# lemma-osu/sknnr

Measured on AMD Instinct MI355X. Metric: Mqueries/sec + achieved HBM GB/s, 10M×50k×32 k=5, 1/2/4/8 MI355X, higher is better.
Workload: dtype f16 split MFMA (hi.hi swept, lo.hi + hi.lo corrections; f32 accumulate) pre-filter + f64 exact re-score

## Files before the change

include/sknnr_hip.h:

```cpp
#ifndef SKNNR_HIP_H
#define SKNNR_HIP_H

#include <stdint.h>

#ifdef __cplusplus
extern "C" {
#endif
#pragma GCC visibility push(default)

#define SKNNR_ABI_VERSION 5

typedef enum sknnr_status {
    SKNNR_OK = 0,
    SKNNR_ERR_INVALID = -1,
    SKNNR_ERR_K_TOO_LARGE = -2,
    SKNNR_ERR_NO_TARGETS = -3,
    SKNNR_ERR_UNSUPPORTED = -4,
    SKNNR_ERR_HIP = -5,
    SKNNR_ERR_NO_DEVICE = -6,
    SKNNR_ERR_NONFINITE = -7
} sknnr_status;

typedef enum sknnr_memspace {
    SKNNR_MEM_HOST = 0,
    SKNNR_MEM_DEVICE = 1
} sknnr_memspace;

typedef enum sknnr_formula {
    SKNNR_FORMULA_EXPANDED = 0,
    SKNNR_FORMULA_DIRECT = 1,
    SKNNR_FORMULA_HAMMING = 2
} sknnr_formula;

typedef enum sknnr_dtype {
    SKNNR_DTYPE_F64 = 0,
    SKNNR_DTYPE_F32 = 1,
    SKNNR_DTYPE_I16 = 2,
    SKNNR_DTYPE_U16 = 3,
    SKNNR_DTYPE_U8 = 4,
    SKNNR_DTYPE_I32 = 5
} sknnr_dtype;

typedef enum sknnr_weight_mode {
    SKNNR_WEIGHTS_UNIFORM = 0,
    SKNNR_WEIGHTS_DISTANCE = 1,
    SKNNR_WEIGHTS_EXPLICIT = 2,
    SKNNR_WEIGHTS_BASE_MASK = 0xff,
    SKNNR_WEIGHTS_F32_TARGETS = 0x100,
    SKNNR_WEIGHTS_F32_WEIGHTS = 0x200
} sknnr_weight_mode;

typedef struct sknnr_index sknnr_index;

typedef struct sknnr_query_opts {
    int32_t n_neighbors;
    int32_t exclude_self;
    int32_t deterministic;
    int32_t decimals;
    int32_t formula;
    int32_t apply_affine;
    int32_t weight_mode;
    int32_t check_finite;
    int32_t query_dtype;
    int32_t reserved_;
    int64_t row_offset;
} sknnr_query_opts;

typedef struct sknnr_stats {
    int64_t queries;
    int64_t coarse_queries;
    int64_t exact_fallbacks;
    int64_t exact_only_queries;
    double  last_kernel_ms;
    double  last_coarse_ms;
    double  total_kernel_ms;
    double  total_coarse_ms;
    int64_t timed_calls;
    int64_t coarse_rows_timed;
    double  mfma_executed_ratio;
} sknnr_stats;


int32_t sknnr_device_count(void);

int32_t sknnr_abi_version(void);

const char* sknnr_last_error(void);

int sknnr_index_create(const double* ref, int64_t n_ref, int32_t d, const double* y, int32_t t,
                       int32_t device, sknnr_index** out);

void sknnr_index_destroy(sknnr_index* index);

int sknnr_index_set_affine(sknnr_index* index, int32_t d_in, const double* center,
                           const double* scale, const double* proj);

int sknnr_index_set_hamming_weights(sknnr_index* index, const double* w, int32_t n);

int sknnr_index_set_forest(sknnr_index* index, int32_t d_in, int32_t n_trees, const int64_t* tree_offset,
                           const double* threshold, const int32_t* feature, const int32_t* left,
                           const int32_t* right);

int sknnr_forest_apply(sknnr_index* index, const void* q, int64_t nq, int32_t query_dtype, int32_t mem,
                       double* out_ids);

int sknnr_affine_transform(const double* x, int64_t n, int32_t d_in, const double* center,
                           const double* scale, const double* proj, int32_t d, double* out,
                           int32_t device);

int sknnr_index_shape(const sknnr_index* index, int64_t* n_ref, int32_t* d, int32_t* t,
                      int32_t* d_in, int32_t* device);

int sknnr_get_stats(const sknnr_index* index, sknnr_stats* out);
int sknnr_reset_stats(sknnr_index* index);

int sknnr_check_finite(sknnr_index* index, void* stream);


int sknnr_kneighbors(sknnr_index* index, const void* q, int64_t nq,
                     const sknnr_query_opts* opts, double* out_dist, int64_t* out_idx,
                     int32_t mem, void* stream);

int sknnr_predict(sknnr_index* index, const void* q, int64_t nq, const sknnr_query_opts* opts,
                  double* out_pred, double* out_dist, int64_t* out_idx, int32_t mem, void* stream);

int sknnr_predict_from_neighbors(sknnr_index* index, const double* dist, const int64_t* idx,
                                 const double* w, int64_t nq, int32_t k, int32_t weight_mode,
                                 double* out_pred, int32_t mem, void* stream);

int sknnr_hamming_distances(sknnr_index* index, const double* q, int64_t nq, const int64_t* rows, int64_t n_rows,
                            double* out, int32_t mem, void* stream);


int sknnr_shard_candidates(sknnr_index* index, const double* q, int64_t nq, const sknnr_query_opts* opts,
                           int64_t index_offset, double* out_val, int64_t* out_idx, int32_t mem, void* stream);
int sknnr_merge_shards(sknnr_index* index, const double* q, int64_t nq, const sknnr_query_opts* opts, int32_t n_shards,
                       const double* shard_val, const int64_t* shard_idx, double* out_dist, int64_t* out_idx,
                       int32_t mem, void* stream);


typedef struct sknnr_stream sknnr_stream;
int sknnr_stream_begin(sknnr_index* index, const sknnr_query_opts* opts, int32_t want_dist, int32_t want_pred,
                       sknnr_stream** out);
int sknnr_stream_push(sknnr_stream* stream, const void* q, int64_t nq, double* out_dist, int64_t* out_idx,
                      double* out_pred);
int sknnr_stream_flush(sknnr_stream* stream);
int sknnr_stream_end(sknnr_stream* stream, int64_t* rows_pushed);

int sknnr_crosswalk(const int64_t* table, int64_t n_table, const int64_t* idx, int64_t n,
                    int64_t* out, int32_t device, int32_t mem, void* stream);


int sknnr_debug_coarse_matrix(sknnr_index* index, const double* q, int64_t nq, float* out,
                              double* out_qnorm, double* out_scale, double* out_eps);

int sknnr_debug_last_prefilter(const sknnr_index* index, int64_t out[8]);

int sknnr_debug_last_hamming(const sknnr_index* index, int64_t out[8]);

int sknnr_debug_hamming_candidates(const sknnr_index* index, int32_t* cnt, int32_t* ids, int64_t n);

#pragma GCC visibility pop
#ifdef __cplusplus
}
#endif
#endif
```

sknnr_amd/_native.py:

```python

from __future__ import annotations

import ctypes
import os
from ctypes import POINTER, byref, c_char_p, c_double, c_float, c_int32, c_int64, c_void_p

import numpy as np

from . import _build

MEM_HOST = 0
MEM_DEVICE = 1
FORMULA_EXPANDED = 0
FORMULA_DIRECT = 1
FORMULA_HAMMING = 2
WEIGHTS_UNIFORM = 0
WEIGHTS_DISTANCE = 1
WEIGHTS_EXPLICIT = 2
WEIGHTS_F32_TARGETS = 0x100
WEIGHTS_F32_WEIGHTS = 0x200

ERR_INVALID = -1
ERR_K_TOO_LARGE = -2
ERR_NO_TARGETS = -3
ERR_UNSUPPORTED = -4
ERR_HIP = -5
ERR_NO_DEVICE = -6
ERR_NONFINITE = -7
ABI_VERSION = 5

DTYPE_CODES = {np.dtype(np.float64): 0, np.dtype(np.float32): 1, np.dtype(np.int16): 2, np.dtype(np.uint16): 3,
               np.dtype(np.uint8): 4, np.dtype(np.int32): 5}


def dtype_code(dt) -> int | None:
    try:
        return DTYPE_CODES.get(np.dtype(dt))
    except TypeError:
        name = str(dt).replace("torch.", "")
        try:
            return DTYPE_CODES.get(np.dtype(name))
        except TypeError:
            return None


EXPORTED_SYMBOLS = (
    "sknnr_device_count",
    "sknnr_abi_version",
    "sknnr_last_error",
    "sknnr_index_create",
    "sknnr_index_destroy",
    "sknnr_index_set_affine",
    "sknnr_index_set_hamming_weights",
    "sknnr_index_set_forest",
    "sknnr_forest_apply",
    "sknnr_affine_transform",
    "sknnr_index_shape",
    "sknnr_get_stats",
    "sknnr_reset_stats",
    "sknnr_check_finite",
    "sknnr_kneighbors",
    "sknnr_predict",
    "sknnr_predict_from_neighbors",
    "sknnr_hamming_distances",
    "sknnr_shard_candidates",
    "sknnr_merge_shards",
    "sknnr_stream_begin",
    "sknnr_stream_push",
    "sknnr_stream_flush",
    "sknnr_stream_end",
    "sknnr_crosswalk",
    "sknnr_debug_coarse_matrix",
    "sknnr_debug_last_prefilter",
    "sknnr_debug_last_hamming",
    "sknnr_debug_hamming_candidates",
)


class QueryOpts(ctypes.Structure):
    _fields_ = [
        ("n_neighbors", c_int32),
        ("exclude_self", c_int32),
        ("deterministic", c_int32),
        ("decimals", c_int32),
        ("formula", c_int32),
        ("apply_affine", c_int32),
        ("weight_mode", c_int32),
        ("check_finite", c_int32),
        ("query_dtype", c_int32),
        ("reserved_", c_int32),
        ("row_offset", c_int64),
    ]


class Stats(ctypes.Structure):
    _fields_ = [
        ("queries", c_int64),
        ("coarse_queries", c_int64),
        ("exact_fallbacks", c_int64),
        ("exact_only_queries", c_int64),
        ("last_kernel_ms", c_double),
        ("last_coarse_ms", c_double),
        ("total_kernel_ms", c_double),
        ("total_coarse_ms", c_double),
        ("timed_calls", c_int64),
        ("coarse_rows_timed", c_int64),
        ("mfma_executed_ratio", c_double),
    ]

    def as_dict(self) -> dict:
        return {name: getattr(self, name) for name, _ in self._fields_}


class HipBackendError(RuntimeError):

    def __init__(self, code: int, message: str):
        super().__init__(f"[sknnr_hip {code}] {message}")
        self.code = code
        self.message = message


_lib = None


def library_path() -> str:
    return os.environ.get("SKNNR_HIP_LIBRARY") or _build.LIB_PATH


def load(build_if_missing: bool = False):
    global _lib
    if _lib is not None:
        return _lib
    import torch

    path = library_path()
    if not os.path.exists(path):
        if build_if_missing:
            _build.build()
        else:
            raise ImportError(
                f"{path} is missing: the MI355X backend has not been built. "
                "Run `python -m sknnr_amd._build` (needs hipcc); there is no CPU fallback."
            )
    lib = ctypes.CDLL(path)
    if lib.sknnr_abi_version() != ABI_VERSION:
        raise ImportError(
            f"{path} has ABI version {lib.sknnr_abi_version()}, this package needs {ABI_VERSION}: "
            "rebuild it with `python -m sknnr_amd._build --force`")
    vp = c_void_p
    lib.sknnr_device_count.restype = c_int32
    lib.sknnr_abi_version.restype = c_int32
    lib.sknnr_last_error.restype = c_char_p
    lib.sknnr_index_create.argtypes = [vp, c_int64, c_int32, vp, c_int32, c_int32, POINTER(vp)]
    lib.sknnr_index_destroy.argtypes = [vp]
    lib.sknnr_index_destroy.restype = None
    lib.sknnr_index_set_affine.argtypes = [vp, c_int32, vp, vp, vp]
    lib.sknnr_index_set_hamming_weights.argtypes = [vp, vp, c_int32]
    lib.sknnr_index_set_forest.argtypes = [vp, c_int32, c_int32, vp, vp, vp, vp, vp]
    lib.sknnr_forest_apply.argtypes = [vp, vp, c_int64, c_int32, c_int32, vp]
    lib.sknnr_affine_transform.argtypes = [vp, c_int64, c_int32, vp, vp, vp, c_int32, vp, c_int32]
    lib.sknnr_index_shape.argtypes = [vp, POINTER(c_int64), POINTER(c_int32), POINTER(c_int32),
                                      POINTER(c_int32), POINTER(c_int32)]
    lib.sknnr_get_stats.argtypes = [vp, POINTER(Stats)]
    lib.sknnr_reset_stats.argtypes = [vp]
    lib.sknnr_check_finite.argtypes = [vp, vp]
    lib.sknnr_stream_begin.argtypes = [vp, POINTER(QueryOpts), c_int32, c_int32, POINTER(vp)]
    lib.sknnr_stream_push.argtypes = [vp, vp, c_int64, vp, vp, vp]
    lib.sknnr_stream_flush.argtypes = [vp]
    lib.sknnr_stream_end.argtypes = [vp, POINTER(c_int64)]
    lib.sknnr_kneighbors.argtypes = [vp, vp, c_int64, POINTER(QueryOpts), vp, vp, c_int32, vp]
    lib.sknnr_predict.argtypes = [vp, vp, c_int64, POINTER(QueryOpts), vp, vp, vp, c_int32, vp]
    lib.sknnr_predict_from_neighbors.argtypes = [vp, vp, vp, vp, c_int64, c_int32, c_int32, vp,
                                                 c_int32, vp]
    lib.sknnr_hamming_distances.argtypes = [vp, vp, c_int64, vp, c_int64, vp, c_int32, vp]
    lib.sknnr_shard_candidates.argtypes = [vp, vp, c_int64, POINTER(QueryOpts), c_int64, vp, vp, c_int32, vp]
    lib.sknnr_merge_shards.argtypes = [vp, vp, c_int64, POINTER(QueryOpts), c_int32, vp, vp, vp, vp, c_int32, vp]
    lib.sknnr_crosswalk.argtypes = [vp, c_int64, vp, c_int64, vp, c_int32, c_int32, vp]
    lib.sknnr_debug_coarse_matrix.argtypes = [vp, vp, c_int64, vp, vp, POINTER(c_double),
                                              POINTER(c_double)]
    lib.sknnr_debug_last_prefilter.argtypes = [vp, POINTER(c_int64)]
    lib.sknnr_debug_last_hamming.argtypes = [vp, POINTER(c_int64)]
    lib.sknnr_debug_hamming_candidates.argtypes = [vp, vp, vp, c_int64]
    _lib = lib
    return lib


def check(code: int) -> None:
    if code != 0:
        raise HipBackendError(code, load().sknnr_last_error().decode("utf-8", "replace"))


def device_count() -> int:
    return int(load().sknnr_device_count())


def _host_ptr(a):
    return None if a is None else a.ctypes.data_as(c_void_p)


def _c_f64(a):
    return None if a is None else np.ascontiguousarray(a, dtype=np.float64)


def _c_rows(a, opts):
    if a is None:
        return None
    for dt, code in DTYPE_CODES.items():
        if code == opts.query_dtype:
            return np.ascontiguousarray(a, dtype=dt)
    raise ValueError(f"unknown query_dtype {opts.query_dtype}")


class Index:

    def __init__(self, ref, y=None, device: int = 0):
        lib = load()
        ref = _c_f64(ref)
        if ref.ndim != 2:
            raise ValueError("ref must be 2-D")
        y2 = None
        if y is not None:
            y2 = _c_f64(y)
            if y2.ndim == 1:
                y2 = y2.reshape(-1, 1)
            if y2.shape[0] != ref.shape[0]:
                raise ValueError("y and ref row counts differ")
        self.n_ref, self.d = ref.shape
        self.t = 0 if y2 is None else y2.shape[1]
        self.device = device
        self.d_in = self.d
        self._h = c_void_p()
        check(lib.sknnr_index_create(_host_ptr(ref), self.n_ref, self.d, _host_ptr(y2), self.t,
                                     device, byref(self._h)))

    def close(self):
        if getattr(self, "_h", None) is not None and self._h:
            load().sknnr_index_destroy(self._h)
            self._h = None

    def __del__(self):
        try:
            self.close()
        except Exception:
            pass

    @property
    def handle(self):
        if not self._h:
            raise RuntimeError("index is closed")
        return self._h

    def set_affine(self, d_in: int, center=None, scale=None, proj=None):
        center, scale, proj = _c_f64(center), _c_f64(scale), _c_f64(proj)
        if proj is not None and proj.shape != (d_in, self.d):
            raise ValueError(f"proj must be ({d_in}, {self.d}), got {proj.shape}")
        check(load().sknnr_index_set_affine(self.handle, d_in, _host_ptr(center), _host_ptr(scale),
                                            _host_ptr(proj)))
        self.d_in = d_in

    def set_hamming_weights(self, w):
        w = _c_f64(w).reshape(-1)
        check(load().sknnr_index_set_hamming_weights(self.handle, _host_ptr(w), w.size))

    def set_forest(self, d_in, tree_offset, threshold, feature, left, right):
        off = np.ascontiguousarray(tree_offset, dtype=np.int64)
        thr = _c_f64(threshold)
        feat, lc, rc = (np.ascontiguousarray(a, dtype=np.int32) for a in (feature, left, right))
        n_nodes = int(off[-1]) if off.size else 0
        if off.ndim != 1 or off.size < 2 or any(a.shape != (n_nodes,) for a in (thr, feat, lc, rc)):
            raise ValueError("tree_offset must hold n_trees + 1 offsets and the node arrays tree_offset[-1] entries")
        check(load().sknnr_index_set_forest(self.handle, int(d_in), off.size - 1, _host_ptr(off), _host_ptr(thr),
                                            _host_ptr(feat), _host_ptr(lc), _host_ptr(rc)))
        self.d_in = int(d_in)

    def forest_apply_host(self, q, query_dtype=0):
        q = _c_rows(q, QueryOpts(query_dtype=int(query_dtype)))
        out = np.empty((q.shape[0], self.d), dtype=np.float64)
        check(load().sknnr_forest_apply(self.handle, _host_ptr(q), q.shape[0], int(query_dtype), MEM_HOST,
                                        _host_ptr(out)))
        return out

    def forest_apply_device(self, q_ptr, nq, query_dtype, out_ptr):
        check(load().sknnr_forest_apply(self.handle, c_void_p(q_ptr or None), nq, int(query_dtype), MEM_DEVICE,
                                        c_void_p(out_ptr or None)))

    def stats(self) -> dict:
        st = Stats()
        check(load().sknnr_get_stats(self.handle, byref(st)))
        return st.as_dict()

    def reset_stats(self):
        check(load().sknnr_reset_stats(self.handle))

    @staticmethod
    def make_opts(k, exclude_self=False, deterministic=True, decimals=10, formula=FORMULA_EXPANDED,
                  apply_affine=False, weight_mode=WEIGHTS_UNIFORM, row_offset=0,
                  check_finite=False, query_dtype=0) -> QueryOpts:
        return QueryOpts(int(k), int(bool(exclude_self)), int(bool(deterministic)), int(decimals),
                         int(formula), int(bool(apply_affine)), int(weight_mode), int(bool(check_finite)),
                         int(query_dtype), 0, int(row_offset))

    def check_finite(self, stream=0) -> None:
        check(load().sknnr_check_finite(self.handle, c_void_p(stream or None)))

    def open_stream(self, opts: QueryOpts, want_dist=True, want_pred=False) -> "QueryStream":
        return QueryStream(self, opts, want_dist, want_pred)

    def kneighbors_host(self, q, opts: QueryOpts, nq=None, return_distance=True):
        q = _c_rows(q, opts)
        if q is not None:
            nq = q.shape[0]
        k = opts.n_neighbors
        idx = np.empty((nq, k), dtype=np.int64)
        dist = np.empty((nq, k), dtype=np.float64) if return_distance else None
        check(load().sknnr_kneighbors(self.handle, _host_ptr(q), nq, byref(opts), _host_ptr(dist),
                                      _host_ptr(idx), MEM_HOST, None))
        return dist, idx

    def predict_host(self, q, opts: QueryOpts, nq=None, return_neighbors=False):
        q = _c_rows(q, opts)
        if q is not None:
            nq = q.shape[0]
        k = opts.n_neighbors
        pred = np.empty((nq, self.t), dtype=np.float64)
        dist = idx = None
        if return_neighbors:
            dist = np.empty((nq, k), dtype=np.float64)
            idx = np.empty((nq, k), dtype=np.int64)
        check(load().sknnr_predict(self.handle, _host_ptr(q), nq, byref(opts), _host_ptr(pred),
                                   _host_ptr(dist), _host_ptr(idx), MEM_HOST, None))
        return (pred, dist, idx) if return_neighbors else pred

    def predict_from_neighbors_host(self, dist, idx, w, weight_mode):
        idx = np.ascontiguousarray(idx, dtype=np.int64)
        dist, w = _c_f64(dist), _c_f64(w)
        nq, k = idx.shape
        pred = np.empty((nq, self.t), dtype=np.float64)
        check(load().sknnr_predict_from_neighbors(self.handle, _host_ptr(dist), _host_ptr(idx),
                                                  _host_ptr(w), nq, k, int(weight_mode),
                                                  _host_ptr(pred), MEM_HOST, None))
        return pred

    def kneighbors_device(self, q_ptr, nq, opts: QueryOpts, dist_ptr, idx_ptr, stream=0):
        check(load().sknnr_kneighbors(self.handle, c_void_p(q_ptr or None), nq, byref(opts),
                                      c_void_p(dist_ptr or None), c_void_p(idx_ptr), MEM_DEVICE,
                                      c_void_p(stream or None)))

    def predict_device(self, q_ptr, nq, opts: QueryOpts, pred_ptr, dist_ptr=0, idx_ptr=0, stream=0):
        check(load().sknnr_predict(self.handle, c_void_p(q_ptr or None), nq, byref(opts),
                                   c_void_p(pred_ptr), c_void_p(dist_ptr or None),
                                   c_void_p(idx_ptr or None), MEM_DEVICE, c_void_p(stream or None)))

    def predict_from_neighbors_device(self, dist_ptr, idx_ptr, w_ptr, nq, k, weight_mode, pred_ptr,
                                      stream=0):
        check(load().sknnr_predict_from_neighbors(
            self.handle, c_void_p(dist_ptr or None), c_void_p(idx_ptr), c_void_p(w_ptr or None), nq, k,
            int(weight_mode), c_void_p(pred_ptr), MEM_DEVICE, c_void_p(stream or None)))

    def hamming_distances_host(self, q, rows=None):
        q = _c_f64(q)
        nq = self.n_ref if q is None else q.shape[0]
        rows = None if rows is None else np.ascontiguousarray(rows, dtype=np.int64)
        n_rows = nq if rows is None else rows.size
        out = np.empty((n_rows, self.n_ref), dtype=np.float64)
        check(load().sknnr_hamming_distances(self.handle, _host_ptr(q), nq, _host_ptr(rows), n_rows, _host_ptr(out),
                                             MEM_HOST, None))
        return out

    def shard_candidates_host(self, q, opts: QueryOpts, index_offset=0):
        q = _c_f64(q)
        nq, k = q.shape[0], opts.n_neighbors
        val = np.empty((nq, k), dtype=np.float64)
        idx = np.empty((nq, k), dtype=np.int64)
        check(load().sknnr_shard_candidates(self.handle, _host_ptr(q), nq, byref(opts), int(index_offset),
                                            _host_ptr(val), _host_ptr(idx), MEM_HOST, None))
        return val, idx

    def shard_candidates_device(self, q_ptr, nq, opts: QueryOpts, index_offset, val_ptr, idx_ptr, stream=0):
        check(load().sknnr_shard_candidates(self.handle, c_void_p(q_ptr), nq, byref(opts), int(index_offset),
                                            c_void_p(val_ptr), c_void_p(idx_ptr), MEM_DEVICE, c_void_p(stream or None)))

    def merge_shards_host(self, q, opts: QueryOpts, shard_val, shard_idx, nq=None, return_distance=True):
        q = _c_f64(q)
        shard_val = _c_f64(shard_val)
        shard_idx = np.ascontiguousarray(shard_idx, dtype=np.int64)
        n_shards = shard_val.shape[0]
        if q is not None:
            nq = q.shape[0]
        k = opts.n_neighbors
        idx = np.empty((nq, k), dtype=np.int64)
        dist = np.empty((nq, k), dtype=np.float64) if return_distance else None
        check(load().sknnr_merge_shards(self.handle, _host_ptr(q), nq, byref(opts), n_shards, _host_ptr(shard_val),
                                        _host_ptr(shard_idx), _host_ptr(dist), _host_ptr(idx), MEM_HOST, None))
        return dist, idx

    def merge_shards_device(self, q_ptr, nq, opts: QueryOpts, n_shards, val_ptr, sidx_ptr, dist_ptr, idx_ptr, stream=0):
        check(load().sknnr_merge_shards(self.handle, c_void_p(q_ptr or None), nq, byref(opts), n_shards, c_void_p(val_ptr),
                                        c_void_p(sidx_ptr), c_void_p(dist_ptr or None), c_void_p(idx_ptr), MEM_DEVICE,
                                        c_void_p(stream or None)))

    def debug_coarse_matrix(self, q):
        q = _c_f64(q)
        nq = q.shape[0]
        out = np.empty((nq, self.n_ref), dtype=np.float32)
        qn = np.empty(nq, dtype=np.float64)
        s, eps = c_double(), c_double()
        check(load().sknnr_debug_coarse_matrix(self.handle, _host_ptr(q), nq, _host_ptr(out),
                                               _host_ptr(qn), byref(s), byref(eps)))
        return out, qn, s.value, eps.value

    PREFILTER_FIELDS = ("generation", "ks", "m_list", "rank_extra", "bulk_waves", "bulk_rows", "thin_rows", "cell_depth")

    def debug_last_prefilter(self) -> dict:
        out = (c_int64 * 8)()
        check(load().sknnr_debug_last_prefilter(self.handle, out))
        return dict(zip(self.PREFILTER_FIELDS, (int(v) for v in out)))

    HAMMING_FIELDS = ("ran", "kk", "compacts", "seed_rows", "band", "tree_pairs", "chunks", "handed_to_scan")

    def debug_last_hamming(self) -> dict:
        out = (c_int64 * 8)()
        check(load().sknnr_debug_last_hamming(self.handle, out))
        return dict(zip(self.HAMMING_FIELDS, (int(v) for v in out)))

    def debug_hamming_candidates(self, n: int):
        cnt = np.empty(n, dtype=np.int32)
        ids = np.empty((n, 192), dtype=np.int32)
        check(load().sknnr_debug_hamming_candidates(self.handle, _host_ptr(cnt), _host_ptr(ids), int(n)))
        return cnt, ids


class QueryStream:

    def __init__(self, index: Index, opts: QueryOpts, want_dist=True, want_pred=False):
        self._index = index
        self._h = c_void_p()
        self._keep = []
        self.k = opts.n_neighbors
        self._opts = opts
        self.want_dist, self.want_pred = bool(want_dist), bool(want_pred)
        check(load().sknnr_stream_begin(index.handle, byref(opts), int(self.want_dist), int(self.want_pred),
                                        byref(self._h)))

    def push(self, q, out_idx=None, out_dist=None, out_pred=None, need_idx=True):
        q = _c_rows(q, self._opts)
        nq = q.shape[0]
        if out_idx is None and (need_idx or not self.want_pred):
            out_idx = np.empty((nq, self.k), dtype=np.int64)
        if out_dist is None and self.want_dist:
            out_dist = np.empty((nq, self.k), dtype=np.float64)
        if out_pred is None and self.want_pred:
            out_pred = np.empty((nq, self._index.t), dtype=np.float64)
        for a, dt, cols in ((out_idx, np.int64, self.k), (out_dist, np.float64, self.k),
                            (out_pred, np.float64, self._index.t)):
            if a is not None and (a.dtype != dt or not a.flags.c_contiguous or a.shape != (nq, cols)):
                raise ValueError(f"output arrays must be C-contiguous ({nq}, {cols}) {np.dtype(dt)}")
        check(load().sknnr_stream_push(self._h, _host_ptr(q), nq, _host_ptr(out_dist), _host_ptr(out_idx),
                                       _host_ptr(out_pred)))
        self._keep.append((out_idx, out_dist, out_pred))
        if len(self._keep) > 8:
            del self._keep[:-8]
        return out_idx, out_dist, out_pred

    def flush(self):
        check(load().sknnr_stream_flush(self._h))
        self._keep.clear()

    def close(self) -> int:
        if not self._h:
            return 0
        n = c_int64(0)
        h, self._h = self._h, c_void_p()
        code = load().sknnr_stream_end(h, byref(n))
        self._keep.clear()
        check(code)
        return int(n.value)

    def __enter__(self):
        return self

    def __exit__(self, *exc):
        if exc[0] is None:
            self.close()
        else:
            try:
                self.close()
            except HipBackendError:
                pass

    def __del__(self):
        try:
            if self._h:
                load().sknnr_stream_end(self._h, None)
                self._h = c_void_p()
        except Exception:
            pass


def affine_transform_host(x, center=None, scale=None, proj=None, device: int = 0) -> np.ndarray:
    x = _c_f64(x)
    center, scale, proj = _c_f64(center), _c_f64(scale), _c_f64(proj)
    n, d_in = x.shape
    d = d_in if proj is None else proj.shape[1]
    out = np.empty((n, d), dtype=np.float64)
    check(load().sknnr_affine_transform(_host_ptr(x), n, d_in, _host_ptr(center), _host_ptr(scale),
                                        _host_ptr(proj), d, _host_ptr(out), device))
    return out


def crosswalk_host(table, idx, device: int = 0):
    table = np.ascontiguousarray(table, dtype=np.int64)
    idx = np.ascontiguousarray(idx, dtype=np.int64)
    out = np.empty(idx.shape, dtype=np.int64)
    check(load().sknnr_crosswalk(_host_ptr(table), table.size, _host_ptr(idx), idx.size,
                                 _host_ptr(out), device, MEM_HOST, None))
    return out


def crosswalk_device(table_ptr, n_table, idx_ptr, n, out_ptr, device=0, stream=0):
    check(load().sknnr_crosswalk(c_void_p(table_ptr), n_table, c_void_p(idx_ptr), n, c_void_p(out_ptr),
                                 device, MEM_DEVICE, c_void_p(stream or None)))
```

sknnr_amd/csrc/bucket.hip.h:

```cpp
#pragma once
#include <hip/hip_runtime.h>
#include <stdint.h>

namespace sknnr {

constexpr int kCellMaxDepth = 6;
constexpr int kCellMax = 1 << kCellMaxDepth;
constexpr int kBucketBlock = 1024;
#ifndef SKNNR_BUCKET_CHUNKS
#define SKNNR_BUCKET_CHUNKS 32
#endif
constexpr int kBucketChunks = SKNNR_BUCKET_CHUNKS;

struct CellTreeDev {
    const float* axes;
    const float* centre;
    const float* thr;
    int depth;
};

__device__ __forceinline__ int cell_of(const float (&z)[kCellMaxDepth], const CellTreeDev& t) {
    int node = 0;
#pragma unroll
    for (int l = 0; l < kCellMaxDepth; ++l)
        if (l < t.depth) node = 2 * node + (z[l] >= t.thr[(1 << l) - 1 + node] ? 1 : 0);
    return node;
}

struct CellArgs {
    const double* xq;
    long nq;
    long n_pad;
    int d;
    int depth;
    const float* axes;
    const float* centre;
    const float* thr;
    unsigned char* cell;
    int* hist;
    int* perm;
};

#ifdef SKNNR_KERNELS_EXACT
__global__ void __launch_bounds__(256) cell_assign_kernel(CellArgs a) {
    const long q = (long)blockIdx.x * 256 + threadIdx.x;
    if (q < a.nq) {
        const double* row = a.xq + q * a.d;
        float z[kCellMaxDepth];
#pragma unroll
        for (int l = 0; l < kCellMaxDepth; ++l) z[l] = 0.f;
        auto feed = [&](int k, double x) {
            const float v = (float)x - a.centre[k];
#pragma unroll
            for (int l = 0; l < kCellMaxDepth; ++l)
                if (l < a.depth) z[l] = fmaf(v, a.axes[l * a.d + k], z[l]);
        };
        int k = 0;
        if ((a.d & 3) == 0) {
            const double2* r2 = (const double2*)row;
            for (; k + 8 <= a.d; k += 8) {
                const double2 v0 = r2[k / 2], v1 = r2[k / 2 + 1], v2 = r2[k / 2 + 2], v3 = r2[k / 2 + 3];
                feed(k, v0.x); feed(k + 1, v0.y); feed(k + 2, v1.x); feed(k + 3, v1.y);
                feed(k + 4, v2.x); feed(k + 5, v2.y); feed(k + 6, v3.x); feed(k + 7, v3.y);
            }
        }
        for (; k < a.d; ++k) feed(k, row[k]);
        const CellTreeDev t{a.axes, a.centre, a.thr, a.depth};
        a.cell[q] = (unsigned char)cell_of(z, t);
    }
}
#endif

#ifdef SKNNR_KERNELS_EXACT
__global__ void __launch_bounds__(kBucketBlock) cell_count_kernel(CellArgs a) {
    __shared__ int h[kCellMax];
    if (threadIdx.x < kCellMax) h[threadIdx.x] = 0;
    __syncthreads();
#pragma unroll
    for (int r = 0; r < kBucketChunks; ++r) {
        const long q = ((long)blockIdx.x * kBucketChunks + r) * kBucketBlock + threadIdx.x;
        if (q < a.nq) atomicAdd(&h[a.cell[q]], 1);
    }
    __syncthreads();
    if (threadIdx.x < kCellMax && h[threadIdx.x] != 0) atomicAdd(&a.hist[threadIdx.x], h[threadIdx.x]);
}
#endif


#ifdef SKNNR_KERNELS_EXACT
__global__ void __launch_bounds__(kBucketBlock) cell_scatter_kernel(CellArgs a) {
    __shared__ int cnt[kCellMax], base[kCellMax], first[kCellMax];
    const int n_cells = 1 << a.depth;
    if (threadIdx.x < kCellMax) cnt[threadIdx.x] = 0;
    if (threadIdx.x == 0) {
        int acc = 0;
        for (int c = 0; c < kCellMax; ++c) {
            first[c] = acc;
            acc += c < n_cells ? a.hist[c] : 0;
        }
    }
    __syncthreads();
    int c[kBucketChunks], ticket[kBucketChunks];
#pragma unroll
    for (int r = 0; r < kBucketChunks; ++r) {
        const long q = ((long)blockIdx.x * kBucketChunks + r) * kBucketBlock + threadIdx.x;
        c[r] = 0;
        ticket[r] = 0;
        if (q < a.nq) {
            c[r] = a.cell[q];
            ticket[r] = atomicAdd(&cnt[c[r]], 1);
        } else if (q < a.n_pad) {
            a.perm[q] = (int)q;
            a.cell[q] = (unsigned char)(n_cells - 1);
        }
    }
    __syncthreads();
    if (threadIdx.x < kCellMax && cnt[threadIdx.x] != 0) base[threadIdx.x] = atomicAdd(&a.hist[kCellMax + threadIdx.x], cnt[threadIdx.x]);
    __syncthreads();
#pragma unroll
    for (int r = 0; r < kBucketChunks; ++r) {
        const long q = ((long)blockIdx.x * kBucketChunks + r) * kBucketBlock + threadIdx.x;
        if (q < a.nq) a.perm[first[c[r]] + base[c[r]] + ticket[r]] = (int)q;
    }
}
#endif

}
```

sknnr_amd/csrc/coarse.hip.h:

```cpp
#pragma once
#include <hip/hip_runtime.h>
#include <float.h>
#include <stdint.h>

namespace sknnr {

#if !defined(SKNNR_EXPERIMENTS) && defined(SKNNR_ABLATE_NO_CORR)
#error "SKNNR_ABLATE_NO_CORR is a timing experiment with wrong results: add -DSKNNR_EXPERIMENTS"
#endif

constexpr long kRowQuantum = 6144;

typedef _Float16 half8 __attribute__((ext_vector_type(8)));
typedef float floatx16 __attribute__((ext_vector_type(16)));
typedef float floatx4 __attribute__((ext_vector_type(4)));

__host__ __device__ constexpr int tile_frag_bytes(int ks) { return 2 * ks * 1024; }
__host__ __device__ constexpr int tile_bytes(int ks) { return 2 * ks * 1024 + 128; }
__host__ __device__ constexpr int tiles_per_stage(int ks) { return ks <= 2 ? 8 : (ks <= 4 ? 4 : 2); }
__host__ __device__ constexpr size_t qimg_index(long row, int part, int ks, int s, int kh) {
    return ((size_t)(row * 2 + part) * ks + s) * 2 + kh;
}
__host__ __device__ constexpr int acc_row(int r, int h) { return (r & 3) + 8 * (r >> 2) + 4 * h; }

// ... 32 lines not shown
__device__ __forceinline__ float min2f(float a, float b, float dep) {
    float r;
    asm("v_min_f32 %0, %1, %2" : "=v"(r) : "v"(a), "v"(b), "v"(dep));
    return r;
}
__device__ __forceinline__ float min2f(float a, float b) { return min2f(a, b, a); }

#ifndef SKNNR_SHIFT_INSERT_FROM
#define SKNNR_SHIFT_INSERT_FROM 32
#endif
template <int M>
__device__ __forceinline__ void list_insert(float (&vals)[M], int (&idxs)[M], float v, int id) {
    if constexpr (M >= SKNNR_SHIFT_INSERT_FROM) {
#pragma unroll
        for (int i = M - 1; i >= 0; --i) {
            const bool here = v < vals[i];
            const bool lower_left = i > 0 ? (v < vals[i - 1]) : false;
            const float nv = lower_left ? vals[i > 0 ? i - 1 : 0] : v;
            const int ni = lower_left ? idxs[i > 0 ? i - 1 : 0] : id;
            vals[i] = here ? nv : vals[i];
            idxs[i] = here ? ni : idxs[i];
        }
    } else {
        vals[M - 1] = v;
        idxs[M - 1] = id;
#pragma unroll
        for (int i = M - 1; i > 0; --i) {
            const bool sw = vals[i] < vals[i - 1];
            const float lo = sw ? vals[i] : vals[i - 1];
            const float hi = sw ? vals[i - 1] : vals[i];
            const int ilo = sw ? idxs[i] : idxs[i - 1];
            const int ihi = sw ? idxs[i - 1] : idxs[i];
            vals[i - 1] = lo;
            vals[i] = hi;
            idxs[i - 1] = ilo;
            idxs[i] = ihi;
        }
    }
}

#ifdef SKNNR_COARSE_TIMERS
static __device__ unsigned long long coarse_timers[8];
#define TICK()                                  \
    do {                                        \
        asm volatile("" ::: "memory");          \
        tk = __builtin_readcyclecounter();      \
        asm volatile("" ::: "memory");          \
    } while (0)
#define TSTAMP(i)            \
    do {                     \
        tk0 = tk;            \
        TICK();              \
        tm[i] += tk - tk0;   \
    } while (0)
#else
#define TICK() ((void)0)
#define TSTAMP(i) ((void)0)
#endif
#ifdef SKNNR_COARSE_COUNTERS
static __device__ unsigned long long coarse_counters[16];
#define CTR_ARG , unsigned (&ctr)[16]
#define CTR_PASS , ctr
#define CTR(i, n) ctr[i] += (unsigned)(n)
#else
#define CTR_ARG
#define CTR_PASS
#define CTR(i, n) ((void)0)
#endif


#ifndef SKNNR_PRIO_CORR
#define SKNNR_PRIO_CORR 2
#define SKNNR_PRIO_SCAN 2
#endif
#ifndef SKNNR_PRIO_MAIN
#define SKNNR_PRIO_MAIN 1
#define SKNNR_PRIO_TEST 0
#endif

__host__ __device__ constexpr int queue_cap(int m) { return m == 2 ? 2 : 4; }
__host__ __device__ constexpr int queue_flush_at(int m) { return m == 2 ? 2 : 3; }
__host__ __device__ constexpr int queue_bytes_per_wave(int nqb, int m) { return nqb * queue_cap(m) * 64 * 8; }

template <int KS>
__device__ __forceinline__ floatx16 contract_main(const half8 (&ah)[KS], const half8 (&bh)[KS], floatx16 c0) {
    floatx16 acc = __builtin_amdgcn_mfma_f32_32x32x16_f16(ah[0], bh[0], c0, 0, 0, 0);
#pragma unroll
    for (int s = 1; s < KS; ++s) acc = __builtin_amdgcn_mfma_f32_32x32x16_f16(ah[s], bh[s], acc, 0, 0, 0);
    return acc;
}
template <int KS>
__device__ __forceinline__ floatx16 contract_correct(const half8 (&ah)[KS], const half8 (&al)[KS],
                                                     const half8 (&bh)[KS], const half8 (&bl)[KS],
                                                     floatx16 acc) {
#pragma unroll
    for (int s = 0; s < KS; ++s) acc = __builtin_amdgcn_mfma_f32_32x32x16_f16(al[s], bh[s], acc, 0, 0, 0);
#pragma unroll
    for (int s = 0; s < KS; ++s) acc = __builtin_amdgcn_mfma_f32_32x32x16_f16(ah[s], bl[s], acc, 0, 0, 0);
    return acc;
}
template <int KS>
__device__ __forceinline__ floatx16 split_contract(const half8 (&ah)[KS], const half8 (&al)[KS],
                                                   const half8 (&bh)[KS], const half8 (&bl)[KS],
                                                   floatx16 c0) {
    return contract_correct<KS>(ah, al, bh, bl, contract_main<KS>(ah, bh, c0));
}

__device__ __forceinline__ void stage_copy(const char* __restrict__ gsrc, char* lds_dst, int bytes,
                                           int wave, int lane, int n_waves) {
    const int n_chunks = (bytes + 1023) >> 10;
    for (int c = wave; c < n_chunks; c += n_waves) {
        const int off = (c << 10) + (lane << 4);
        if (off < bytes) {
            __builtin_amdgcn_global_load_lds(
                (const __attribute__((address_space(1))) void*)(gsrc + off),
                (__attribute__((address_space(3))) void*)(lds_dst + (c << 10)), 16, 0, 0);
        }
    }
}

__device__ __forceinline__ unsigned lds_addr_of(const void* p) {
    return (unsigned)(unsigned long)(const __attribute__((address_space(3))) char*)p;
}
__device__ __forceinline__ void queue_store(unsigned addr, float v, int id) {
    const unsigned long long pr = ((unsigned long long)(unsigned)id << 32) | (unsigned long long)__float_as_uint(v);
    asm volatile("ds_write_b64 %0, %1" ::"v"(addr), "v"(pr) : "memory");
}
__device__ __forceinline__ unsigned long long queue_load(unsigned addr) {
    unsigned long long pr;
    asm volatile("ds_read_b64 %0, %1\n\ts_waitcnt lgkmcnt(0)" : "=&v"(pr) : "v"(addr) : "memory");
    return pr;
}

template <int M>
__device__ __forceinline__ void take_hit(float v, int id, float (&vals)[M], int (&idxs)[M], float& thr,
                                         int& cnt, unsigned qlane CTR_ARG) {
    const bool hit = v < thr;
    if (__builtin_amdgcn_ballot_w64(hit) == 0) return;
    CTR(3, 1);
    CTR(4, __builtin_popcountll(__builtin_amdgcn_ballot_w64(hit)));
    const bool room = cnt < queue_cap(M);
    if (hit && room) {
        queue_store(qlane + cnt * 512, v, id);
        cnt += 1;
    }
    if (__builtin_amdgcn_ballot_w64(hit && !room) != 0) {
        CTR(5, 1);
        if (hit && !room) {
            list_insert<M>(vals, idxs, v, id);
            thr = min2f(thr, vals[M - 1]);
        }
    }
}

template <int M>
__device__ __forceinline__ float pair_union_rank_m(const float (&vals)[M]) {
    float u = fminf(vals[0], __shfl_xor(vals[M - 1], 32, 64));
#pragma unroll
    for (int i = 1; i < M; ++i) u = fmaxf(u, fminf(vals[i], __shfl_xor(vals[M - 1 - i], 32, 64)));
    return u;
}

template <int M>
__device__ __forceinline__ void flush_queue(float (&vals)[M], int (&idxs)[M], float& thr, int& cnt,
                                            unsigned qlane CTR_ARG) {
    for (int i = 0; __builtin_amdgcn_ballot_w64(i < cnt) != 0; ++i) {
        CTR(7, 1);
        CTR(8, __builtin_popcountll(__builtin_amdgcn_ballot_w64(i < cnt)));
        if (i < cnt) {
            const unsigned long long e = queue_load(qlane + i * 512);
            const float ev = __uint_as_float((unsigned)e);
            CTR(9, __builtin_amdgcn_ballot_w64(ev < vals[M - 1]) != 0);
            CTR(10, __builtin_popcountll(__builtin_amdgcn_ballot_w64(ev < vals[M - 1])));
            if (ev < vals[M - 1]) list_insert<M>(vals, idxs, ev, (int)(e >> 32));
        }
    }
    cnt = 0;
    thr = pair_union_rank_m<M>(vals);
}

template <int KS, int M>
__global__ void __launch_bounds__(coarse_waves(KS, M) * 64, coarse_wps(KS, M))
coarse_kernel(const char* __restrict__ rimg,
              int n_stages,
              const uint4* __restrict__ qimg,
              const double* __restrict__ qnc,
              float skip_scale,
              int n_sentinel,
              float* __restrict__ cand_val,
              int* __restrict__ cand_idx) {
    constexpr int TPS = tiles_per_stage(KS);
    constexpr int TB = tile_bytes(KS);
    constexpr int STAGE = TPS * TB;
    extern __shared__ __attribute__((aligned(16))) char smem[];

    const int lane = threadIdx.x & 63;
    const int wave = __builtin_amdgcn_readfirstlane(threadIdx.x >> 6);
    const int half = lane >> 5;
    constexpr int WAVES = coarse_waves(KS, M);
    constexpr int NQB = coarse_nqb(KS, M);
    constexpr bool LO_ON_DEMAND = coarse_lo_on_demand(KS, M);
    const int qb0 = (blockIdx.x * WAVES + wave) * NQB;
    const unsigned qwave = lds_addr_of(smem + 2 * STAGE + wave * queue_bytes_per_wave(NQB, M) + lane * 8);

    half8 bh[NQB][KS], bl[NQB][KS];
#pragma unroll
    for (int qb = 0; qb < NQB; ++qb) {
#pragma unroll
        for (int s = 0; s < KS; ++s) {
            const long row = (long)(qb0 + qb) * 32 + (lane & 31);
            const uint4 uh = qimg[qimg_index(row, 0, KS, s, lane >> 5)];
            const uint4 ul = qimg[qimg_index(row, 1, KS, s, lane >> 5)];
            bh[qb][s] = __builtin_bit_cast(half8, uh);
            bl[qb][s] = __builtin_bit_cast(half8, ul);
        }
    }

    float vals[NQB][M];
    int idxs[NQB][M];
    float thr[NQB];
    float margin[NQB];
    int cnt[NQB];
#pragma unroll
    for (int qb = 0; qb < NQB; ++qb) {
        thr[qb] = FLT_MAX;
        cnt[qb] = 0;
        margin[qb] = skip_scale * (float)sqrt(qnc[(size_t)(qb0 + qb) * 32 + (lane & 31)]) + 1e-30f;
#pragma unroll
        for (int i = 0; i < M; ++i) {
            vals[qb][i] = (half == 0 && i < n_sentinel) ? -FLT_MAX : FLT_MAX;
            idxs[qb][i] = -1;
        }
    }

#ifdef SKNNR_COARSE_COUNTERS
    unsigned ctr[16] = {};
#endif
#ifdef SKNNR_COARSE_TIMERS
    unsigned long long tm[8] = {};
    unsigned long long tk = 0, tk0 = 0;
    TICK();
    const unsigned long long t_begin = tk;
#endif
    stage_copy(rimg, smem, STAGE, wave, lane, WAVES);
    __syncthreads();

    for (int st = 0; st < n_stages; ++st) {
        char* cur = smem + (st & 1) * STAGE;
        if (st + 1 < n_stages)
            stage_copy(rimg + (size_t)(st + 1) * STAGE, smem + ((st + 1) & 1) * STAGE, STAGE, wave, lane, WAVES);

        auto tile_load = [&](const char* tb, half8 (&ah)[KS], half8 (&al)[KS], floatx16& c0, bool keep_lo) {
#pragma unroll
            for (int s = 0; s < KS; ++s) {
                ah[s] = *(const half8*)(tb + (0 * KS + s) * 1024 + lane * 16);
                if (keep_lo) al[s] = *(const half8*)(tb + (1 * KS + s) * 1024 + lane * 16);
            }
            const floatx4* cp = (const floatx4*)(tb + tile_frag_bytes(KS) + half * 64);
            const floatx4 c_0 = cp[0], c_1 = cp[1], c_2 = cp[2], c_3 = cp[3];
#pragma unroll
            for (int i = 0; i < 4; ++i) {
                c0[i] = c_0[i];
                c0[4 + i] = c_1[i];
                c0[8 + i] = c_2[i];
                c0[12 + i] = c_3[i];
            }
        };
        auto tile_process = [&](const char* tb, int tile_no, const floatx16& c0, half8 (&ah)[KS], half8 (&al)[KS],
                                bool have_lo) {
            const int id_base = tile_no * 32 + 4 * half;
#pragma unroll
            for (int qb = 0; qb < NQB; ++qb) {
                __builtin_amdgcn_s_setprio(SKNNR_PRIO_MAIN);
                floatx16 acc = contract_main<KS>(ah, bh[qb], c0);
                __builtin_amdgcn_s_setprio(SKNNR_PRIO_TEST);
                const float t0 = first_read(acc[0]);
                float g[5];
                g[0] = min3f(t0, acc[1], acc[2], t0);
                g[1] = min3f(acc[3], acc[4], acc[5], t0);
                g[2] = min3f(acc[6], acc[7], acc[8], t0);
                g[3] = min3f(acc[9], acc[10], acc[11], t0);
                g[4] = min2f(min3f(acc[12], acc[13], acc[14], t0), acc[15], t0);
                const float m1 = min3f(min3f(g[0], g[1], g[2], t0), g[3], g[4], t0);
                const float loose = thr[qb] + margin[qb];
                CTR(0, 1);
                if (__builtin_amdgcn_ballot_w64(m1 < loose) == 0) {
                    TSTAMP(1);
                    continue;
                }
                TSTAMP(2);
                CTR(1, 1);
                CTR(11, __builtin_popcountll(__builtin_amdgcn_ballot_w64(m1 < loose)));
                CTR(12, __builtin_amdgcn_ballot_w64(m1 < thr[qb]) != 0);
                if (!have_lo) {
#pragma unroll
                    for (int s = 0; s < KS; ++s) al[s] = *(const half8*)(tb + (1 * KS + s) * 1024 + lane * 16);
                    have_lo = true;
                }
                __builtin_amdgcn_s_setprio(SKNNR_PRIO_CORR);
#ifndef SKNNR_ABLATE_NO_CORR
                acc = contract_correct<KS>(ah, al, bh[qb], bl[qb], acc);
#endif
                __builtin_amdgcn_s_setprio(SKNNR_PRIO_SCAN);
                const unsigned qlane = qwave + qb * (queue_cap(M) * 512);
#pragma unroll
                for (int k = 0; k < 5; ++k) {
// ... 85 lines not shown
```

sknnr_amd/csrc/coarse2.hip.h:

```cpp
#pragma once
#include "coarse.hip.h"

#if !defined(SKNNR_EXPERIMENTS) && (defined(SKNNR_V2_SWEEP_ONLY) || defined(SKNNR_V2_NO_BARRIER) || defined(SKNNR_V2_NO_SEED))
#error "SKNNR_V2_SWEEP_ONLY / NO_BARRIER / NO_SEED are timing experiments with wrong results: add -DSKNNR_EXPERIMENTS"
#endif

namespace sknnr {

typedef _Float16 half2v __attribute__((ext_vector_type(2)));

__host__ __device__ constexpr int tile2_bytes(int ks) { return ks * 1024 + 128; }
#ifndef SKNNR_V2_WAVES
#define SKNNR_V2_WAVES 16
#endif
#ifndef SKNNR_V2_UNROLL
#define SKNNR_V2_UNROLL 1
#endif
#ifndef SKNNR_V2_TPS
#define SKNNR_V2_TPS (SKNNR_V2_WAVES == 16 ? 16 : 8)
#endif
__host__ __device__ constexpr int tiles_per_stage2(int ks) { return ks <= 2 ? SKNNR_V2_TPS : SKNNR_V2_TPS / 2; }
#ifndef SKNNR_SEED_TILES
#define SKNNR_SEED_TILES 64
#endif
constexpr int kSeedTiles = SKNNR_SEED_TILES;
__host__ __device__ constexpr int seed_tiles_for(long n_tiles, int tps) {
    const long want = n_tiles / 8 < kSeedTiles ? n_tiles / 8 : kSeedTiles;
    const long stages = want / tps < 1 ? 1 : want / tps;
    return (int)(stages * tps);
}
constexpr int kCoarse2Waves = SKNNR_V2_WAVES;
constexpr int kCoarse2Nqb = 2;
#ifndef SKNNR_V2_QCAP
#define SKNNR_V2_QCAP 5
#endif
constexpr int kQueueCap = SKNNR_V2_QCAP;
#ifndef SKNNR_V2_FLUSH_AT
#define SKNNR_V2_FLUSH_AT 3
#endif
constexpr int kQueueFlushAt = SKNNR_V2_FLUSH_AT;
__host__ __device__ constexpr int queue2_bytes_per_wave() { return kCoarse2Nqb * kQueueCap * 64 * 8 + kCoarse2Nqb * 64 * 4; }
#ifndef SKNNR_V2_M2
#define SKNNR_V2_M2 1
#endif
#ifndef SKNNR_V2_M12
#define SKNNR_V2_M12 1
#endif
#ifndef SKNNR_V2_M16
#define SKNNR_V2_M16 1
#endif
__host__ __device__ constexpr bool coarse2_supported(int ks, int m) {
    return (m == 6 && ks <= 4) || (m == 8 && ks <= 4) || (SKNNR_V2_M2 && m == 2 && ks <= 2) || (SKNNR_V2_M16 && m == 16 && ks <= 4) ||
           (SKNNR_V2_M12 && m == 12 && ks <= 4);
}
#ifndef SKNNR_V2_M16_WAVES
#define SKNNR_V2_M16_WAVES 12
#endif
__host__ __device__ constexpr int coarse2_waves(int ks, int m) {
    return (m == 16 || (m == 12 && ks >= 2) || (m == 8 && ks >= 4)) ? SKNNR_V2_M16_WAVES : kCoarse2Waves;
}

__device__ __forceinline__ float dot8(const half8& x, const half8& y, float acc) {
#pragma unroll
    for (int i = 0; i < 4; ++i) {
        const half2v p = {x[2 * i], x[2 * i + 1]}, q = {y[2 * i], y[2 * i + 1]};
        acc = __builtin_amdgcn_fdot2(p, q, acc, false);
    }
    return acc;
}

template <int M, int E>
__device__ __forceinline__ float pair_union_rank(const float (&vals)[M]) {
    if constexpr (E == 0) {
        return pair_union_rank_m<M>(vals);
    } else {
        static_assert(E >= 1 && E <= M, "rank between M + 1 and 2 M");
        float u = fmaxf(vals[E - 1], __shfl_xor(vals[E - 1], 32, 64));
#pragma unroll
        for (int i = E; i < M; ++i) u = fmaxf(u, fminf(vals[i], __shfl_xor(vals[M + E - 1 - i], 32, 64)));
        return u;
    }
}
__host__ __device__ constexpr int coarse2_rank_extra(int m_list, int kk) {
    if (kk + 1 <= m_list) return 0;
    if (m_list == 6) return 3;
    if (m_list == 8) return kk <= 10 ? 4 : (kk <= 13 ? 7 : 8);
    if (m_list == 12) return kk <= 20 ? 10 : 12;
    return kk <= 20 ? 6 : (kk <= 25 ? 11 : (kk <= 30 ? 15 : 16));
}
constexpr int kCoarse2MaxKK6 = 7, kCoarse2MaxKK8 = 15, kCoarse2MaxKK12 = 23;
constexpr int kCoarse2MaxKK16 = 31;

#define SKNNR_TREE_A                                   \
    "v_min3_f32 %[g0], %[x0], %[x1], %[x2]\n\t"        \
    "v_min3_f32 %[g1], %[x3], %[x4], %[x5]\n\t"        \
    "v_min3_f32 %[g2], %[x6], %[x7], %[x8]\n\t"        \
    "v_min3_f32 %[g3], %[x9], %[x10], %[x11]\n\t"
#define SKNNR_TREE_B                                   \
    "v_min3_f32 %[g4], %[x12], %[x13], %[x14]\n\t"     \
    "v_min3_f32 %[m], %[g0], %[g1], %[g2]\n\t"         \
    "v_min_f32 %[g4], %[g4], %[x15]\n\t"               \
    "s_nop 0\n\t"                                      \
    "v_min3_f32 %[m], %[m], %[g3], %[g4]\n\t"
#define SKNNR_TREE_OUT [g0] "=&v"(g[0]), [g1] "=&v"(g[1]), [g2] "=&v"(g[2]), [g3] "=&v"(g[3]), [g4] "=&v"(g[4]), [m] "=&v"(m)
#define SKNNR_TREE_IN                                                                                             \
    [x0] "v"(x[0]), [x1] "v"(x[1]), [x2] "v"(x[2]), [x3] "v"(x[3]), [x4] "v"(x[4]), [x5] "v"(x[5]), [x6] "v"(x[6]), \
        [x7] "v"(x[7]), [x8] "v"(x[8]), [x9] "v"(x[9]), [x10] "v"(x[10]), [x11] "v"(x[11]), [x12] "v"(x[12]),       \
        [x13] "v"(x[13]), [x14] "v"(x[14]), [x15] "v"(x[15])

__device__ __forceinline__ void step_test_only(const floatx16& x, float (&g)[5], float& m) {
    asm volatile("s_nop 7\n\ts_nop 7\n\t" SKNNR_TREE_A SKNNR_TREE_B : SKNNR_TREE_OUT : SKNNR_TREE_IN);
}
template <int KS>
__device__ __forceinline__ void tile_issue_and_test(floatx16& a, floatx16& c, const half8 (&ah)[KS], const half8 (&p)[KS],
                                                    const half8 (&q)[KS], float (&g)[5], float& m) {
    static_assert(KS >= 1 && KS <= 4, "hand-scheduled for one to four K-steps");
    asm volatile("v_mfma_f32_32x32x16_f16 %[a], %[h0], %[p0], %[c]\n\t" : [a] "=&v"(a) : [c] "v"(c), [h0] "v"(ah[0]), [p0] "v"(p[0]));
#pragma unroll
    for (int s = 1; s < KS; ++s)
        asm volatile("v_mfma_f32_32x32x16_f16 %[a], %[h], %[p], %[a]\n\t" : [a] "+v"(a) : [h] "v"(ah[s]), [p] "v"(p[s]));
    asm volatile("v_mfma_f32_32x32x16_f16 %[c], %[h0], %[q0], %[c]\n\t"
                 "s_nop 7\n\ts_nop 3\n\t"
                 : [c] "+v"(c)
                 : [h0] "v"(ah[0]), [q0] "v"(q[0]), "v"(a));
    const floatx16& x = a;
    asm volatile(SKNNR_TREE_A
                 : [g0] "=&v"(g[0]), [g1] "=&v"(g[1]), [g2] "=&v"(g[2]), [g3] "=&v"(g[3])
                 : [x0] "v"(x[0]), [x1] "v"(x[1]), [x2] "v"(x[2]), [x3] "v"(x[3]), [x4] "v"(x[4]), [x5] "v"(x[5]),
                   [x6] "v"(x[6]), [x7] "v"(x[7]), [x8] "v"(x[8]), [x9] "v"(x[9]), [x10] "v"(x[10]), [x11] "v"(x[11]));
    if constexpr (KS >= 2)
        asm volatile("v_mfma_f32_32x32x16_f16 %[c], %[h1], %[q1], %[c]\n\t" : [c] "+v"(c) : [h1] "v"(ah[1]), [q1] "v"(q[1]));
    asm volatile("v_min3_f32 %[g4], %[x12], %[x13], %[x14]\n\t"
                 "v_min3_f32 %[m], %[g0], %[g1], %[g2]\n\t"
                 "v_min_f32 %[g4], %[g4], %[x15]\n\t"
                 "s_nop 0\n\t"
                 "v_min3_f32 %[m], %[m], %[g3], %[g4]\n\t"
                 : [g4] "=&v"(g[4]), [m] "=&v"(m)
                 : [x12] "v"(x[12]), [x13] "v"(x[13]), [x14] "v"(x[14]), [x15] "v"(x[15]), [g0] "v"(g[0]), [g1] "v"(g[1]),
                   [g2] "v"(g[2]), [g3] "v"(g[3]));
#pragma unroll
    for (int s = 2; s < KS; ++s)
        asm volatile("v_mfma_f32_32x32x16_f16 %[c], %[h], %[q], %[c]\n\t" : [c] "+v"(c) : [h] "v"(ah[s]), [q] "v"(q[s]));
}

template <int KS, int M, int WAVES = kCoarse2Waves, int E = 0>
__global__ void __launch_bounds__(WAVES * 64, WAVES == 12 ? 3 : (WAVES == 8 || M > 8 ? 2 : 4))
coarse2_kernel(const char* __restrict__ rhi,
               const char* __restrict__ rlo,
               int n_stages,
               const uint4* __restrict__ qimg,
               const double* __restrict__ qnc,
               float skip_scale,
               int n_sentinel,
               float* __restrict__ cand_val,
               int* __restrict__ cand_idx,
               int pos0, const int* __restrict__ qperm, const unsigned char* __restrict__ qcell,
               const int* __restrict__ cell_stage) {
    constexpr int TPS = tiles_per_stage2(KS);
    constexpr int TB = tile2_bytes(KS);
    constexpr int STAGE = TPS * TB;
    constexpr int NQB = kCoarse2Nqb;
    extern __shared__ __attribute__((aligned(16))) char smem[];

    const int lane = threadIdx.x & 63;
    const int wave = __builtin_amdgcn_readfirstlane(threadIdx.x >> 6);
    const int half = lane >> 5;
    const int qb0 = (blockIdx.x * WAVES + wave) * NQB;
    const unsigned qwave = lds_addr_of(smem + 2 * STAGE + wave * queue2_bytes_per_wave() + lane * 8);
    const unsigned qrow_lds = lds_addr_of(smem + 2 * STAGE + wave * queue2_bytes_per_wave() + NQB * kQueueCap * 512 + lane * 4);
    int st0 = 0;
    if (qperm) {
        const int mid = qperm[pos0 + (blockIdx.x * WAVES + WAVES / 2) * NQB * 32];
        st0 = __builtin_amdgcn_readfirstlane(cell_stage[qcell[mid]]);
    }
    auto qfrag = [&](int r, int part, int s) {
        return __builtin_bit_cast(half8, qimg[qimg_index(r, part, KS, s, lane >> 5)]);
    };
    auto stage_of = [&](int st) {
        const int i = st0 + st;
        return i >= n_stages ? i - n_stages : i;
    };

    half8 bh[NQB][KS];
    float qnorm[NQB];
#pragma unroll
    for (int qb = 0; qb < NQB; ++qb) {
        const int pos = pos0 + (qb0 + qb) * 32 + (lane & 31);
        const int r = qperm ? qperm[pos] : pos;
        asm volatile("ds_write_b32 %0, %1" ::"v"(qrow_lds + qb * 256), "v"(r) : "memory");
#pragma unroll
        for (int s = 0; s < KS; ++s) bh[qb][s] = qfrag(r, 0, s);
        qnorm[qb] = (float)sqrt(qnc[r]);
    }

    float vals[NQB][M];
    int idxs[NQB][M];
#ifdef SKNNR_COARSE_COUNTERS
    unsigned ctr[16] = {};
#endif
#ifdef SKNNR_COARSE_TIMERS
    unsigned long long tm[8] = {};
    unsigned long long tk = 0, tk0 = 0;
    TICK();
    const unsigned long long t_begin = tk;
#endif
    float loose[NQB], margin[NQB];
    int cnt[NQB];
    auto reset_lists = [&](int qb) {
#pragma unroll
        for (int i = 0; i < M; ++i) {
            vals[qb][i] = (half == 0 && i < n_sentinel) ? -FLT_MAX : FLT_MAX;
            idxs[qb][i] = -1;
        }
    };
#pragma unroll
    for (int qb = 0; qb < NQB; ++qb) {
        cnt[qb] = 0;
        margin[qb] = skip_scale * qnorm[qb] + 1e-30f;
        loose[qb] = FLT_MAX;
        reset_lists(qb);
    }

    auto load_c0 = [&](const char* tb, floatx16& acc) {
        const floatx4* cp = (const floatx4*)(tb + KS * 1024 + half * 64);
        const floatx4 c_0 = cp[0], c_1 = cp[1], c_2 = cp[2], c_3 = cp[3];
#pragma unroll
        for (int i = 0; i < 4; ++i) {
            acc[i] = c_0[i];
            acc[4 + i] = c_1[i];
            acc[8 + i] = c_2[i];
            acc[12 + i] = c_3[i];
        }
    };
    auto load_hi = [&](const char* tb, half8 (&ah)[KS]) {
#pragma unroll
        for (int s = 0; s < KS; ++s) ah[s] = *(const half8*)(tb + s * 1024 + lane * 16);
    };
    auto issue_main = [&](const half8 (&ah)[KS], int qb, floatx16& acc) {
        __builtin_amdgcn_s_setprio(1);
#pragma unroll
        for (int s = 0; s < KS; ++s) acc = __builtin_amdgcn_mfma_f32_32x32x16_f16(ah[s], bh[qb][s], acc, 0, 0, 0);
        __builtin_amdgcn_s_setprio(0);
    };

    auto flush_wave = [&](int qb) {
        TSTAMP(1);
        CTR(6, 1);
        const unsigned qbase = qwave - (unsigned)lane * 8u + (unsigned)qb * (kQueueCap * 512u);
        const int c = cnt[qb];
        const unsigned long long b0 = __builtin_amdgcn_ballot_w64((c & 1) != 0), b1 = __builtin_amdgcn_ballot_w64((c & 2) != 0),
                                 b2 = __builtin_amdgcn_ballot_w64((c & 4) != 0);
        auto below = [&](unsigned long long m) { return (int)__builtin_amdgcn_mbcnt_hi((unsigned)(m >> 32), __builtin_amdgcn_mbcnt_lo((unsigned)m, 0u)); };
        const int off = below(b0) + 2 * below(b1) + 4 * below(b2);
        const int total = __builtin_popcountll(b0) + 2 * __builtin_popcountll(b1) + 4 * __builtin_popcountll(b2);
        static_assert(kQueueCap == 5 || kQueueCap == 4, "four or five entries per lane are read here");
        unsigned long long own[5];
        if constexpr (kQueueCap == 5) {
            asm volatile("ds_read_b64 %0, %5\n\tds_read_b64 %1, %5 offset:512\n\tds_read_b64 %2, %5 offset:1024\n\t"
                         "ds_read_b64 %3, %5 offset:1536\n\tds_read_b64 %4, %5 offset:2048\n\ts_waitcnt lgkmcnt(0)"
                         : "=&v"(own[0]), "=&v"(own[1]), "=&v"(own[2]), "=&v"(own[3]), "=&v"(own[4])
                         : "v"(qbase + (unsigned)lane * 8u)
                         : "memory");
        } else {
            asm volatile("ds_read_b64 %0, %4\n\tds_read_b64 %1, %4 offset:512\n\tds_read_b64 %2, %4 offset:1024\n\t"
                         "ds_read_b64 %3, %4 offset:1536\n\ts_waitcnt lgkmcnt(0)"
                         : "=&v"(own[0]), "=&v"(own[1]), "=&v"(own[2]), "=&v"(own[3])
                         : "v"(qbase + (unsigned)lane * 8u)
                         : "memory");
        }
#pragma unroll
        for (int j = 0; j < kQueueCap; ++j) {
            const unsigned long long e = own[j] | ((unsigned long long)(unsigned)(lane & 31) << 58);
            if (j < c) asm volatile("ds_write_b64 %0, %1" ::"v"(qbase + (unsigned)(off + j) * 8u), "v"(e) : "memory");
        }
        const unsigned qrow_base = qrow_lds - (unsigned)lane * 4u + (unsigned)qb * 256u;
        for (int t0 = 0; t0 < total; t0 += 32) {
            CTR(7, 1);
            const int gi = t0 + (lane & 31);
            const bool on = gi < total;
            unsigned long long e;
            asm volatile("ds_read_b64 %0, %1\n\ts_waitcnt lgkmcnt(0)" : "=&v"(e) : "v"(qbase + (unsigned)(on ? gi : 0) * 8u) : "memory");
            CTR(8, __builtin_popcountll(__builtin_amdgcn_ballot_w64(on)));
            const unsigned hi32 = (unsigned)(e >> 32);
            const int pos = (int)(hi32 & 0x03ffffffu), col = (int)(hi32 >> 26);
            int r;
            asm volatile("ds_read_b32 %0, %1\n\ts_waitcnt lgkmcnt(0)" : "=&v"(r) : "v"(qrow_base + (unsigned)col * 4u) : "memory");
            const unsigned row = (unsigned)(pos & 31) * 16u + (unsigned)(32 * half) * 16u;
            const unsigned oh = (unsigned)(pos >> 5) * (unsigned)TB + row;
            const unsigned ol = (unsigned)(pos >> 5) * (unsigned)(KS * 1024) + row;
            half8 fl[KS], fh[KS], qh[KS], ql[KS];
#pragma unroll
            for (int s2 = 0; s2 < KS; ++s2) {
                fl[s2] = *(const half8*)(rlo + ol + s2 * 1024);
                fh[s2] = *(const half8*)(rhi + oh + s2 * 1024);
                qh[s2] = qfrag(r, 0, s2);
                ql[s2] = qfrag(r, 1, s2);
            }
            float acc = 0.f;
#pragma unroll
            for (int s2 = 0; s2 < KS; ++s2) {
                acc = dot8(fl[s2], qh[s2], acc);
                acc = dot8(fh[s2], ql[s2], acc);
            }
            const float other = __shfl_xor(acc, 32, 64);
            const float cv = __uint_as_float((unsigned)e) + (half ? other + acc : acc + other);
            if (on && half == 0) asm volatile("ds_write_b32 %0, %1" ::"v"(qbase + (unsigned)gi * 8u), "v"(cv) : "memory");
        }
        for (int j = 0; __builtin_amdgcn_ballot_w64(j < c) != 0; ++j) {
            const bool on = j < c;
            unsigned long long e;
            asm volatile("ds_read_b64 %0, %1\n\ts_waitcnt lgkmcnt(0)" : "=&v"(e) : "v"(qbase + (unsigned)(on ? off + j : 0) * 8u) : "memory");
            const float cv = __uint_as_float((unsigned)e);
            const int pos = (int)((unsigned)(e >> 32) & 0x03ffffffu);
            if constexpr (E == 0) {
                if (on && cv < vals[qb][M - 1]) list_insert<M>(vals[qb], idxs[qb], cv, pos);
            } else {
                float out_v = FLT_MAX;
                int out_i = -1;
                if (on) {
                    if (cv < vals[qb][M - 1]) {
                        out_v = vals[qb][M - 1];
                        out_i = idxs[qb][M - 1];
                        list_insert<M>(vals[qb], idxs[qb], cv, pos);
                    } else {
                        out_v = cv;
                        out_i = pos;
                    }
                }
                const bool offer = out_v < loose[qb];
                if (__builtin_amdgcn_ballot_w64(offer) != 0) {
                    const float in_v = __shfl_xor(offer ? out_v : FLT_MAX, 32, 64);
                    const int in_i = __shfl_xor(out_i, 32, 64);
                    if (in_v < vals[qb][M - 1]) list_insert<M>(vals[qb], idxs[qb], in_v, in_i);
                }
            }
        }
        cnt[qb] = 0;
        const float tight = pair_union_rank<M, E>(vals[qb]) + margin[qb];
        loose[qb] = loose[qb] != loose[qb] ? loose[qb] : min2f(loose[qb], tight);
        TSTAMP(2);
    };

    auto process = [&](floatx16& acc, const float (&g)[5], float m1, int tile_no, int qb) {
        CTR(0, 1);
        if (__builtin_amdgcn_ballot_w64(m1 < loose[qb]) == 0) return;
        CTR(1, 1);
        TSTAMP(0);
#ifdef SKNNR_V2_SWEEP_ONLY
        margin[qb] += 1e-30f;
        return;
#endif
        const unsigned qlane = qwave + qb * (kQueueCap * 512);
        asm volatile("" : "+s"(tile_no));
        const int id_base = tile_no * 32 + 4 * half;
        int want = cnt[qb];
#pragma unroll
        for (int k = 0; k < 5; ++k) {
            if (__builtin_amdgcn_ballot_w64(g[k] < loose[qb]) == 0) continue;
#pragma unroll
            for (int r = 3 * k; r < (k == 4 ? 16 : 3 * k + 3); ++r) {
                const bool hit = acc[r] < loose[qb];
                if (__builtin_amdgcn_ballot_w64(hit) == 0) continue;
                CTR(3, 1);
                CTR(4, __builtin_popcountll(__builtin_amdgcn_ballot_w64(hit)));
                want += hit ? 1 : 0;
                if (hit && cnt[qb] < kQueueCap) {
                    queue_store(qlane + cnt[qb] * 512, acc[r], id_base + acc_row(r, 0));
                    cnt[qb] += 1;
                }
            }
        }
        if (want > kQueueCap) loose[qb] = __builtin_nanf("");
        if (__builtin_amdgcn_ballot_w64(cnt[qb] >= kQueueFlushAt) != 0) flush_wave(qb);
        else TSTAMP(1);
    };

    const int n_tiles = n_stages * TPS;
#ifdef SKNNR_V2_NO_SEED
    if (false) {
#else
    if (n_tiles >= 2 * kSeedTiles) {
#endif
        const int SEED_STAGES = seed_tiles_for(n_tiles, TPS) / TPS;
        stage_copy(rhi + (size_t)stage_of(0) * STAGE, smem, STAGE, wave, lane, WAVES);
        __syncthreads();
        for (int st = 0; st < SEED_STAGES; ++st) {
            const char* cur = smem + (st & 1) * STAGE;
            if (st + 1 < SEED_STAGES)
                stage_copy(rhi + (size_t)stage_of(st + 1) * STAGE, smem + ((st + 1) & 1) * STAGE, STAGE, wave, lane, WAVES);
#pragma unroll 1
            for (int t = 0; t < TPS; ++t) {
                const char* tb = cur + t * TB;
                half8 ah[KS];
                load_hi(tb, ah);
#pragma unroll
                for (int qb = 0; qb < NQB; ++qb) {
                    floatx16 acc;
                    load_c0(tb, acc);
                    issue_main(ah, qb, acc);
                    const float t0 = first_read(acc[0]);
                    const float a0 = min3f(t0, acc[1], acc[2], t0), a1 = min3f(acc[3], acc[4], acc[5], t0);
                    const float a2 = min3f(acc[6], acc[7], acc[8], t0), a3 = min3f(acc[9], acc[10], acc[11], t0);
                    const float a4 = min2f(min3f(acc[12], acc[13], acc[14], t0), acc[15], t0);
                    const float m1 = min3f(min3f(a0, a1, a2, t0), a3, a4, t0);
                    if (__builtin_amdgcn_ballot_w64(m1 < vals[qb][M - 1]) != 0) {
                        if (m1 < vals[qb][M - 1]) list_insert<M>(vals[qb], idxs[qb], m1, 0);
                    }
                }
            }
            __syncthreads();
        }
#pragma unroll
        for (int qb = 0; qb < NQB; ++qb) {
            const float seed = pair_union_rank<M, E>(vals[qb]);
            loose[qb] = seed < FLT_MAX ? seed + 2.0f * margin[qb] : FLT_MAX;
            reset_lists(qb);
        }
        TSTAMP(4);
    }

    stage_copy(rhi + (size_t)stage_of(0) * STAGE, smem, STAGE, wave, lane, WAVES);
    __syncthreads();
    for (int st = 0; st < n_stages; ++st) {
        const char* cur = smem + (st & 1) * STAGE;
        if (st + 1 < n_stages)
            stage_copy(rhi + (size_t)stage_of(st + 1) * STAGE, smem + ((st + 1) & 1) * STAGE, STAGE, wave, lane, WAVES);
        const int tile0 = stage_of(st) * TPS;
        float g[5], m1;
#pragma unroll SKNNR_V2_UNROLL
        for (int t = 0; t < TPS; ++t) {
            const char* tb = cur + t * TB;
            const int tile_no = tile0 + t;
            floatx16 acc0, acc1;
            half8 ah[KS];
            load_hi(tb, ah);
            load_c0(tb, acc1);
            tile_issue_and_test<KS>(acc0, acc1, ah, bh[0], bh[1], g, m1);
            process(acc0, g, m1, tile_no, 0);
            step_test_only(acc1, g, m1);
            process(acc1, g, m1, tile_no, 1);
        }
        TSTAMP(0);
#ifdef SKNNR_V2_NO_BARRIER
        asm volatile("s_waitcnt vmcnt(0)" ::: "memory");
#else
        __syncthreads();
#endif
        TSTAMP(3);
    }

#ifdef SKNNR_COARSE_COUNTERS
    if (lane == 0)
        for (int i = 0; i < 16; ++i) atomicAdd(&coarse_counters[i], (unsigned long long)ctr[i]);
#endif
    TSTAMP(0);
#pragma unroll
    for (int qb = 0; qb < NQB; ++qb) {
        flush_wave(qb);
        const size_t q = (size_t)(pos0 + (qb0 + qb) * 32 + (lane & 31));
        const size_t base = (q * 2 + half) * M;
        const int mine = loose[qb] != loose[qb] ? 1 : 0;
        const bool bad = (mine | __shfl_xor(mine, 32, 64)) != 0;
#pragma unroll
        for (int i = 0; i < M; ++i) {
            cand_val[base + i] = bad ? __builtin_nanf("") : vals[qb][i];
            cand_idx[base + i] = idxs[qb][i];
        }
    }
#ifdef SKNNR_COARSE_TIMERS
    TICK();
    tm[7] = tk - t_begin;
    if (lane == 0)
        for (int i = 0; i < 8; ++i) atomicAdd(&coarse_timers[i], tm[i]);
#endif
}

}
```

sknnr_amd/csrc/exact.hip.h:

```cpp
#pragma once
#include <type_traits>
#include <hip/hip_runtime.h>
#include <float.h>
#include <math.h>
#include <stdint.h>

#include "bucket.hip.h"
#include "coarse.hip.h"

namespace sknnr {

enum : int { kDtypeF64 = 0, kDtypeF32 = 1, kDtypeI16 = 2, kDtypeU16 = 3, kDtypeU8 = 4, kDtypeI32 = 5, kDtypeCount = 6 };
__host__ __device__ constexpr int dtype_bytes(int dt) {
    return dt == kDtypeF64 ? 8 : (dt == kDtypeF32 || dt == kDtypeI32 ? 4 : (dt == kDtypeU8 ? 1 : 2));
}
__device__ __forceinline__ double load_as_f64(const void* __restrict__ x, int dt, long i) {
    switch (dt) {
        case kDtypeF32: return (double)((const float*)x)[i];
        case kDtypeI16: return (double)((const short*)x)[i];
        case kDtypeU16: return (double)((const unsigned short*)x)[i];
        case kDtypeU8: return (double)((const unsigned char*)x)[i];
        case kDtypeI32: return (double)((const int*)x)[i];
        default: return ((const double*)x)[i];
    }
// ... 214 lines not shown
    bool overflow = false;
#pragma unroll
    for (int jc = 0; jc < 2 * KS; ++jc) {
        half8 hi, lo;
#pragma unroll
        for (int jj = 0; jj < 8; ++jj) {
            const int k = jc * 8 + jj;
            const double b = (live && k < a.d) ? a.s * (acc[k] - a.mu[k]) : 0.0;
            overflow |= !(fabs(b) < kImageLimit);
            qn = fma(b, b, qn);
            const _Float16 h = (_Float16)(float)b;
            hi[jj] = h;
            lo[jj] = (_Float16)(float)(b - (double)h);
        }
        {
            const int step = jc >> 1, hh = jc & 1;
            char* irow = wtile + (size_t)lane_ * (64 * KS + 16);
            *(uint4*)(irow + 16 * (int)qimg_index(0, 0, KS, step, hh)) = __builtin_bit_cast(uint4, hi);
            *(uint4*)(irow + 16 * (int)qimg_index(0, 1, KS, step, hh)) = __builtin_bit_cast(uint4, lo);
        }
    }
    {
        __builtin_amdgcn_fence(__ATOMIC_RELEASE, "wavefront");
        __builtin_amdgcn_wave_barrier();
        __builtin_amdgcn_fence(__ATOMIC_ACQUIRE, "wavefront");
        constexpr int PPR = 4 * KS;
        const long q0w = q - lane_;
        uint4* dst = a.qimg + (size_t)q0w * PPR;
#pragma unroll
        for (int i = 0; i < PPR; ++i) {
            const int p = 64 * i + lane_;
            const int r = p / PPR, o = p % PPR;
            dst[p] = *(const uint4*)(wtile + (size_t)r * (64 * KS + 16) + 16 * o);
        }
    }
    if (a.qnc && q < a.nq_pad) a.qnc[q] = live ? (overflow ? INFINITY : qn) : 0.0;
}

#ifdef SKNNR_KERNELS_EXACT
__global__ void __launch_bounds__(256) check_finite_kernel(const double* __restrict__ x, long n, int* status) {
    bool has_nan = false, has_inf = false;
    const long stride = (long)gridDim.x * 256;
    for (long i = (long)blockIdx.x * 256 + threadIdx.x; i < n; i += stride) classify(x[i], has_nan, has_inf);
    report_nonfinite(status, has_nan, has_inf);
}
#endif

template <int FORMULA>
__device__ __forceinline__ double pair_d2_f(const double* __restrict__ x, const double* __restrict__ r,
                                            int d, double rn) {
    double qn = 0.0, acc = 0.0;
    int c = 0;
    auto step = [&](double xv, double rv) {
        if (FORMULA == 0) {
            qn = fma(xv, xv, qn);
            acc = fma(xv, rv, acc);
        } else {
            const double t = xv - rv;
            acc = acc + t * t;
        }
    };
    if ((d & 1) == 0) {
        const double2* x2 = (const double2*)x;
        const double2* r2 = (const double2*)r;
        for (; c + 16 <= d; c += 16) {
            double2 rv[8];
#pragma unroll
            for (int i = 0; i < 8; ++i) rv[i] = r2[(c >> 1) + i];
#pragma unroll
            for (int i = 0; i < 8; ++i) {
                const double2 xv = x2[(c >> 1) + i];
                step(xv.x, rv[i].x);
                step(xv.y, rv[i].y);
            }
        }
        for (; c + 8 <= d; c += 8) {
            double2 xv[4], rv[4];
#pragma unroll
            for (int i = 0; i < 4; ++i) {
                rv[i] = r2[(c >> 1) + i];
                xv[i] = x2[(c >> 1) + i];
            }
#pragma unroll
            for (int i = 0; i < 4; ++i) {
                step(xv[i].x, rv[i].x);
                step(xv[i].y, rv[i].y);
            }
        }
        for (; c < d; c += 2) {
            const double2 xv = x2[c >> 1], rv = r2[c >> 1];
            step(xv.x, rv.x);
            step(xv.y, rv.y);
        }
    }
    for (; c < d; ++c) step(x[c], r[c]);
    if (FORMULA == 0) {
        const double d2 = qn + (-2.0 * acc) + rn;
        return d2 > 0.0 ? d2 : 0.0;
    }
    return acc;
}
__device__ __forceinline__ double pair_d2(const double* __restrict__ x, const double* __restrict__ r,
                                          int d, double rn, int formula) {
    return formula == 0 ? pair_d2_f<0>(x, r, d, rn) : pair_d2_f<1>(x, r, d, rn);
}

struct SelectArgs {
    const double* xq;
    const double* ref;
    const double* rn;
    long nq;
    int d;
    int n_ref;
    int k;
    int kk;
    int exclude_self;
    int deterministic;
    int formula;
    int pow10_is_divisor;
    double pow10;
    long row_offset;
    const double* hw;
    double hw_sum;
    int raw;
    long id_offset;
    double* out_dist;
    long* out_idx;
};

__device__ __forceinline__ double round_key(double x, double p10, int divisor) {
    return divisor ? rint(x / p10) : rint(x * p10);
}

struct FinalizeArgs {
    SelectArgs s;
    const float* cand_val;
    const int* cand_idx;
    const int* perm;
    int m_list;
    int rank_extra;
    const double* qnc;
    double inv_s2;
    double s2;
    double inv_s;
    double eps_c;
    double ymax;
    double noise_a;
    double mu2;
    int* fail_list;
    int fail_base;
    int* fail_count;
    const int* qperm;
    long pos0;
};

template <int LPQ, int N>
__device__ __forceinline__ int peer_i(int v, int c) {
    constexpr int B = N / 16, R = N % 16;
    const int vb = B ? __shfl_xor(v, 16 * B, LPQ) : v;
    if constexpr (R != 0) {
        return __builtin_amdgcn_update_dpp(0, vb, 0x120 + R, 0xf, 0xf, false);
    } else {
        return vb;
    }
}
template <int LPQ, int N>
__device__ __forceinline__ float peer_f(float v, int c) {
    return __int_as_float(peer_i<LPQ, N>(__float_as_int(v), c));
}
template <int LPQ, int N>
__device__ __forceinline__ long peer_l(long v, int c) {
    const int lo = peer_i<LPQ, N>((int)(unsigned)(unsigned long)v, c);
    const int hi = peer_i<LPQ, N>((int)((unsigned long)v >> 32), c);
    return (long)(((unsigned long)(unsigned)hi << 32) | (unsigned long)(unsigned)lo);
}
template <int LPQ, int N>
__device__ __forceinline__ double peer_d(double v, int c) {
    return __longlong_as_double(peer_l<LPQ, N>(__double_as_longlong(v), c));
}
template <int LPQ>
struct PeersI {
    int blk[LPQ / 16];
    __device__ __forceinline__ explicit PeersI(int v) {
        blk[0] = v;
#pragma unroll
        for (int b = 1; b < LPQ / 16; ++b) blk[b] = __shfl_xor(v, 16 * b, LPQ);
    }
    template <int N>
    __device__ __forceinline__ int get() const {
        constexpr int B = N / 16, R = N % 16;
        if constexpr (R != 0) {
            return __builtin_amdgcn_update_dpp(0, blk[B], 0x120 + R, 0xf, 0xf, false);
        } else {
            return blk[B];
        }
    }
};
template <int LPQ>
struct PeersF {
    PeersI<LPQ> p;
    __device__ __forceinline__ explicit PeersF(float v) : p(__float_as_int(v)) {}
    template <int N>
    __device__ __forceinline__ float get() const { return __int_as_float(p.template get<N>()); }
};
template <int LPQ>
struct PeersL {
    PeersI<LPQ> lo, hi;
    __device__ __forceinline__ explicit PeersL(long v)
        : lo((int)(unsigned)(unsigned long)v), hi((int)((unsigned long)v >> 32)) {}
    template <int N>
    __device__ __forceinline__ long get() const {
        return (long)(((unsigned long)(unsigned)hi.template get<N>() << 32) | (unsigned long)(unsigned)lo.template get<N>());
    }
};
template <int LPQ>
struct PeersD {
    PeersL<LPQ> p;
    __device__ __forceinline__ explicit PeersD(double v) : p(__double_as_longlong(v)) {}
    template <int N>
    __device__ __forceinline__ double get() const { return __longlong_as_double(p.template get<N>()); }
};
template <int LPQ, int N = 1, typename F>
__device__ __forceinline__ void for_each_peer(F&& f) {
    if constexpr (N < LPQ) {
        f(std::integral_constant<int, N>{});
        for_each_peer<LPQ, N + 1>(f);
    }
}

template <int LPQ, int O = LPQ / 2>
__device__ __forceinline__ double group_min(double v, int c) {
    if constexpr (O > 0) {
        v = fmin(v, peer_d<LPQ, O>(v, c));
        return group_min<LPQ, O / 2>(v, c);
    } else {
        return v;
    }
}
template <int LPQ, int O = LPQ / 2>
__device__ __forceinline__ double group_max(double v, int c) {
    if constexpr (O > 0) {
        v = fmax(v, peer_d<LPQ, O>(v, c));
        return group_max<LPQ, O / 2>(v, c);
    } else {
        return v;
    }
}
template <int LPQ, int O = LPQ / 2>
__device__ __forceinline__ int group_min_i(int v, int c) {
    if constexpr (O > 0) {
        const int w = peer_i<LPQ, O>(v, c);
        return group_min_i<LPQ, O / 2>(w < v ? w : v, c);
    } else {
        return v;
    }
}

template <int LPQ>
__device__ __forceinline__ double scatter_d(double v, int dst_lane) {
    const long bits = __double_as_longlong(v);
    const int lo = __builtin_amdgcn_ds_permute(dst_lane << 2, (int)(unsigned)(unsigned long)bits);
    const int hi = __builtin_amdgcn_ds_permute(dst_lane << 2, (int)((unsigned long)bits >> 32));
    return __longlong_as_double((long)(((unsigned long)(unsigned)hi << 32) | (unsigned long)(unsigned)lo));
}
template <int LPQ>
__device__ __forceinline__ int group_count(bool flag, int gbase) {
    const unsigned long long b = __builtin_amdgcn_ballot_w64(flag);
    const unsigned long long mask = LPQ == 64 ? ~0ull : (((1ull << (LPQ & 63)) - 1ull) << gbase);
    return __builtin_popcountll(b & mask);
}
template <int LPQ>
__device__ __forceinline__ bool group_any(bool flag, int gbase) {
    const unsigned long long b = __builtin_amdgcn_ballot_w64(flag);
    const unsigned long long mask = LPQ == 64 ? ~0ull : (((1ull << (LPQ & 63)) - 1ull) << gbase);
    return (b & mask) != 0ull;
}

__host__ __device__ constexpr size_t finalize_row_bytes(int d) { return (size_t)d * 8 + 16; }
__host__ __device__ constexpr size_t finalize_lds_bytes(int m_tmpl, int d) { return (size_t)(256 / (2 * m_tmpl)) * finalize_row_bytes(d); }

template <int M>
__global__ void __launch_bounds__(256) finalize_kernel(FinalizeArgs a) {
    constexpr int LPQ = 2 * M;
    const SelectArgs& s = a.s;
    const long gt = (long)blockIdx.x * 256 + threadIdx.x;
    long q = gt / LPQ;
    const int c = (int)(gt % LPQ);
    const bool live = q < s.nq;
    if (!live) q = s.nq - 1;
    const long q_list = a.qperm ? a.pos0 + q : q;
    if (a.qperm) q = a.qperm[a.pos0 + q];

    extern __shared__ __attribute__((aligned(16))) char fin_lds[];
    double* xrow = (double*)(fin_lds + (size_t)(threadIdx.x / LPQ) * finalize_row_bytes(s.d));
    for (int e = c; e < s.d; e += LPQ) xrow[e] = s.xq[q * s.d + e];
    __builtin_amdgcn_fence(__ATOMIC_RELEASE, "wavefront");
    __builtin_amdgcn_wave_barrier();
    __builtin_amdgcn_fence(__ATOMIC_ACQUIRE, "wavefront");

    const int list = c / M, slot = c % M;
    const bool has_slot = slot < a.m_list;
    const long cpos = (q_list * 2 + list) * a.m_list + (has_slot ? slot : 0);
    const int pos_img = has_slot ? a.cand_idx[cpos] : -1;
    const float cv = has_slot ? a.cand_val[cpos] : INFINITY;
    const bool valid = pos_img >= 0 && pos_img < s.n_ref;
    const int id = valid ? a.perm[pos_img] : -1;

    const double qn = a.qnc[q];
    const double nrm = sqrt(qn) + a.ymax;
    const double eps = a.eps_c * nrm * nrm;
    const float cve = valid ? cv : INFINITY;
    int n_le = 1;
    const PeersF<LPQ> cve_of(cve);
    for_each_peer<LPQ>([&](auto n) { n_le += cve_of.template get<n.value>() <= cve; });
    const double tau_c = group_min<LPQ>(n_le >= s.kk ? (double)cve : INFINITY, c);
    const double nr = nrm * a.inv_s + a.mu2;
    const double noise = a.noise_a * nr * nr;
    const bool need = valid && ((double)cv <= tau_c + 2.0 * eps + 2.0 * noise * a.s2);

    double d2 = INFINITY;
    if (need) d2 = pair_d2(xrow, s.ref + (long)id * s.d, s.d, s.rn[id], s.formula);
    const bool usable = need && (d2 == d2) && d2 < INFINITY;
    if (!usable) d2 = INFINITY;
    const int key_id = usable ? id : (0x7fffff00 + c);

    int rank = 0;
    const PeersD<LPQ> d2_of(d2);
    const PeersI<LPQ> key_of(key_id);
    for_each_peer<LPQ>([&](auto n) {
        const double dj = d2_of.template get<n.value>();
        const int ij = key_of.template get<n.value>();
        rank += (dj < d2) || (dj == d2 && ij < key_id);
    });
    const int n_usable = group_count<LPQ>(usable, (int)(threadIdx.x & 63) & ~(LPQ - 1));

    const double tau = group_min<LPQ>(rank >= s.kk - 1 ? d2 : INFINITY, c);
    const int ex = a.rank_extra;
    const float cv_raw = has_slot ? cv : INFINITY;
    const bool paired = has_slot && slot >= ex;
    const int partner = M + (paired ? a.m_list + ex - 1 - slot : 0);
    const float cv_partner = __shfl(cv_raw, partner, LPQ);
    double t_pair = (list == 0 && paired) ? (double)fminf(cv_raw, cv_partner) : -INFINITY;
    if (ex > 0 && has_slot && slot == ex - 1) t_pair = (double)cv_raw;
    const double t_min = group_max<LPQ>(t_pair, c);
    const double bound = (qn + t_min - eps) * a.inv_s2 - noise;
    bool certified = (n_usable >= s.kk) && (tau < INFINITY) && (bound > tau);
    {
        const int gbase = (int)(threadIdx.x & 63) & ~(LPQ - 1);
        const double by_rank = scatter_d<LPQ>(d2, gbase + rank);
        const double next = __shfl_down(by_rank, 1, LPQ);
        const bool has_next = c + 1 < LPQ;
        const bool tied_here = has_next && by_rank == next && by_rank < INFINITY &&
                               (s.deterministic ? c == s.kk - 1 : c < s.kk);
        if (!s.raw && group_any<LPQ>(tied_here, gbase)) certified = false;
    }

    int sel = rank;
    const long self_id = s.row_offset + q;
    if (s.exclude_self) {
        const bool is_self = usable && (long)id == self_id && rank < s.kk;
        int drop = group_min_i<LPQ>(is_self ? rank : 0x7fffffff, c);
        if (drop == 0x7fffffff) drop = 0;
        sel = rank == drop ? -1 : (rank > drop ? rank - 1 : rank);
    }
    const bool chosen = usable && sel >= 0 && sel < s.k;
    const double dist = s.raw ? d2 : sqrt(d2 > 0.0 ? d2 : 0.0);

    int pos = sel;
    if (s.deterministic) {
        const double dmax = group_max<LPQ>(chosen ? dist : 0.0, c);
        const double row_scale = fmax(dmax, 1.0);
        const double k0 = chosen ? round_key(dist / row_scale, s.pow10, s.pow10_is_divisor) : INFINITY;
        const int gbase = (int)(threadIdx.x & 63) & ~(LPQ - 1);
        const double k0_by_sel = scatter_d<LPQ>(k0, gbase + (sel >= 0 ? sel : LPQ - 1));
        const double k0_next = __shfl_down(k0_by_sel, 1, LPQ);
        const bool equal_keys = c + 1 < s.k && c + 1 < LPQ && k0_by_sel == k0_next && k0_by_sel < INFINITY;
        if (__builtin_amdgcn_ballot_w64(equal_keys) != 0) {
            long k1 = (long)id - self_id;
            k1 = k1 < 0 ? -k1 : k1;
            const int tagged = key_id | (chosen ? (int)0x80000000u : 0);
            pos = 0;
            const PeersD<LPQ> k0_of(k0);
            const PeersL<LPQ> k1_of(k1);
            const PeersI<LPQ> tag_of(tagged);
            for_each_peer<LPQ>([&](auto n) {
                const double k0j = k0_of.template get<n.value>();
                const long k1j = k1_of.template get<n.value>();
                const int tj = tag_of.template get<n.value>();
                const int ij = tj & 0x7fffffff;
                const bool less = (k0j < k0) || (k0j == k0 && (k1j < k1 || (k1j == k1 && ij < key_id)));
                pos += (tj < 0) && less;
            });
        }
    }
    if (live && chosen) {
        if (s.out_dist) s.out_dist[q * s.k + pos] = dist;
        s.out_idx[q * s.k + pos] = id + s.id_offset;
    }
    if (live && c == 0 && !certified) {
        const int slot = atomicAdd(a.fail_count, 1);
        a.fail_list[slot] = a.fail_base + (int)q;
    }
}

struct ScanArgs {
    SelectArgs s;
    const double* refT;
    const int* list;
    const int* count;
    double* slice_v;
    int* slice_i;
    int* list2;
    int* count2;
};

constexpr int kScanSliceMaxKK = 32;
constexpr int kScanMaxSlices = 32;
__host__ __device__ inline int scan_slices(long n_items, int nq_pass, int n_ref, int kk, int grid_wg) {
    const long passes = (n_items + nq_pass - 1) / nq_pass;
    if (passes <= 0 || kk > kScanSliceMaxKK) return 1;
    const int n_steps = (n_ref + 511) / 512;
    long sl = grid_wg / passes;
    if (sl > kScanMaxSlices) sl = kScanMaxSlices;
    if (sl > n_steps) sl = n_steps;
    return sl < 2 ? 1 : (int)sl;
}

__device__ __forceinline__ void heap_push_ref(double* hv, int* hi, int k, double v, int id) {
    int cur = 0;
    for (;;) {
        const int l = 2 * cur + 1, r = l + 1;
        int nxt;
        if (l >= k) break;
        if (r >= k) {
            if (hv[l] > v) nxt = l; else break;
        } else if (hv[l] >= hv[r]) {
            if (v < hv[l]) nxt = l; else break;
        } else {
            if (v < hv[r]) nxt = r; else break;
        }
        hv[cur] = hv[nxt];
        hi[cur] = hi[nxt];
        cur = nxt;
    }
    hv[cur] = v;
    hi[cur] = id;
}

__device__ __forceinline__ void sorted_insert_ref(double* hv, int* hi, int k, double v, int id) {
    int pos = k - 1;
    while (pos > 0 && hv[pos - 1] > v) {
        hv[pos] = hv[pos - 1];
        hi[pos] = hi[pos - 1];
        --pos;
    }
    hv[pos] = v;
    hi[pos] = id;
}

__device__ __forceinline__ void swap_slots(double* v, int* x, int a, int b) {
    const double tv = v[a]; v[a] = v[b]; v[b] = tv;
    const int tx = x[a]; x[a] = x[b]; x[b] = tx;
}

__device__ void dual_quicksort_ref(double* v0, int* x0, int n0, int* stack) {
    int sp = 0;
    stack[sp++] = 0;
    stack[sp++] = n0;
    while (sp > 0) {
        const int n = stack[--sp];
        const int off = stack[--sp];
        double* v = v0 + off;
        int* x = x0 + off;
        if (n <= 1) continue;
        if (n == 2) {
            if (v[0] > v[1]) swap_slots(v, x, 0, 1);
            continue;
        }
        if (n == 3) {
            if (v[0] > v[1]) swap_slots(v, x, 0, 1);
            if (v[1] > v[2]) {
                swap_slots(v, x, 1, 2);
                if (v[0] > v[1]) swap_slots(v, x, 0, 1);
            }
            continue;
        }
        const int mid = n / 2;
        if (v[0] > v[n - 1]) swap_slots(v, x, 0, n - 1);
        if (v[n - 1] > v[mid]) {
            swap_slots(v, x, n - 1, mid);
            if (v[0] > v[n - 1]) swap_slots(v, x, 0, n - 1);
        }
        const double pivot = v[n - 1];
        int store = 0;
        for (int i = 0; i < n - 1; ++i) {
            if (v[i] < pivot) {
                swap_slots(v, x, i, store);
                ++store;
            }
        }
        swap_slots(v, x, store, n - 1);
        if (store > 1) { stack[sp++] = off; stack[sp++] = store; }
        if (store + 2 < n) { stack[sp++] = off + store + 1; stack[sp++] = n - store - 1; }
    }
}

template <int FORMULA>
__device__ void scan_finish_query(const SelectArgs& s, long q, double* hv, int* hi, int* stack) {
    const int KK = s.kk;
    if (s.raw) {
        for (int e = 1; e < KK; ++e) {
            const double dv = hv[e];
            const int iv = hi[e];
            int jj = e - 1;
            while (jj >= 0 && (hv[jj] > dv || (hv[jj] == dv && hi[jj] > iv))) {
                hv[jj + 1] = hv[jj];
                hi[jj + 1] = hi[jj];
                --jj;
            }
            hv[jj + 1] = dv;
            hi[jj + 1] = iv;
        }
        for (int e = 0; e < s.k; ++e) {
            if (s.out_dist) s.out_dist[q * s.k + e] = hv[e];
            s.out_idx[q * s.k + e] = (long)hi[e] + s.id_offset;
        }
        return;
    }
    if (FORMULA == 0) dual_quicksort_ref(hv, hi, KK, stack);
    const long self_id = s.row_offset + q;
    int drop = -1;
    if (s.exclude_self) {
        drop = 0;
        for (int e = 0; e < KK; ++e)
            if ((long)hi[e] == self_id) { drop = e; break; }
    }
    int n = 0;
    for (int e = 0; e < KK; ++e) {
        if (e == drop) continue;
        hv[n] = FORMULA == 2 ? hv[e] : sqrt(hv[e] > 0.0 ? hv[e] : 0.0);
        hi[n] = hi[e];
        ++n;
    }
    if (n > s.k) n = s.k;
    if (s.deterministic) {
        double dmax = 0.0;
        for (int e = 0; e < n; ++e) dmax = fmax(dmax, hv[e]);
        const double row_scale = fmax(dmax, 1.0);
        for (int e = 1; e < n; ++e) {
            const double dv = hv[e];
            const int iv = hi[e];
            const double k0 = round_key(dv / row_scale, s.pow10, s.pow10_is_divisor);
            long k1 = (long)iv - self_id;
            k1 = k1 < 0 ? -k1 : k1;
            int jj = e - 1;
            while (jj >= 0) {
// ... 514 lines not shown
```

sknnr_amd/csrc/k_coarse2.hip:

```cpp
#include <cstdio>
#include <cstring>

#include "launch.hip.h"

#ifndef SKNNR_C2_PART
#error "compile with -DSKNNR_C2_PART=0 or 1"
#endif

namespace sknnr {
namespace {

constexpr int kTailWaves = 4;

template <int KS, int M, int WAVES, int E>
hipError_t go(const launch::Coarse2Launch& L, hipStream_t st) {
    constexpr int QPB = WAVES * kCoarse2Nqb * 32;
    constexpr size_t sh = 2 * (size_t)tiles_per_stage2(KS) * tile2_bytes(KS) + (size_t)WAVES * queue2_bytes_per_wave();
    static_assert(kRowQuantum % QPB == 0, "query rows are padded to multiples of kRowQuantum");
    static_assert(sh <= 160 * 1024, "LDS budget");
    auto kern = coarse2_kernel<KS, M, WAVES, E>;
    hipError_t e = hipFuncSetAttribute((const void*)kern, hipFuncAttributeMaxDynamicSharedMemorySize, (int)sh);
    if (e != hipSuccess) return e;
    kern<<<dim3((unsigned)(L.rows / QPB)), dim3(WAVES * 64), sh, st>>>(L.rhi, L.rlo, L.n_stages, L.qimg, L.qnc, L.skip_scale, L.n_sentinel,
                                                                   L.cand_val, L.cand_idx, L.pos0, L.qperm, L.qcell, L.cell_stage);
    return hipGetLastError();
}

template <int KS, int M, int WAVES>
int by_rank(int extra, const launch::Coarse2Launch& L, hipStream_t st, hipError_t* err) {
    if (extra == 0) { *err = go<KS, M, WAVES, 0>(L, st); return 0; }
    if constexpr (M == 16) {
        if (extra == 6) { *err = go<KS, M, WAVES, 6>(L, st); return 0; }
        if (extra == 11) { *err = go<KS, M, WAVES, 11>(L, st); return 0; }
        if (extra == 15) { *err = go<KS, M, WAVES, 15>(L, st); return 0; }
        if (extra == 16) { *err = go<KS, M, WAVES, 16>(L, st); return 0; }
    } else if constexpr (M == 12) {
        if (extra == 10) { *err = go<KS, M, WAVES, 10>(L, st); return 0; }
        if (extra == 12) { *err = go<KS, M, WAVES, 12>(L, st); return 0; }
    } else if constexpr (M == 8) {
        if (extra == 4) { *err = go<KS, M, WAVES, 4>(L, st); return 0; }
        if (extra == 7) { *err = go<KS, M, WAVES, 7>(L, st); return 0; }
        if (extra == 8) { *err = go<KS, M, WAVES, 8>(L, st); return 0; }
    } else if constexpr (M == 6) {
        if (extra == 3) { *err = go<KS, M, WAVES, 3>(L, st); return 0; }
    }
    return launch::kNoInstance;
}

template <int KS, int M>
int by_waves(int waves, int extra, const launch::Coarse2Launch& L, hipStream_t st, hipError_t* err) {
    static_assert(coarse2_supported(KS, M), "no second-generation kernel for this shape");
    if (waves == coarse2_waves(KS, M)) return by_rank<KS, M, coarse2_waves(KS, M)>(extra, L, st, err);
    if (waves == kTailWaves) return by_rank<KS, M, kTailWaves>(extra, L, st, err);
    return launch::kNoInstance;
}

}

namespace launch {

#if SKNNR_C2_PART == 0
int coarse2_part1(int ks, int m, int waves, int extra, const Coarse2Launch& L, hipStream_t st, hipError_t* err);

static int coarse2_part0(int ks, int m, int waves, int extra, const Coarse2Launch& L, hipStream_t st, hipError_t* err) {
    if (ks == 2 && m == 6) return by_waves<2, 6>(waves, extra, L, st, err);
#ifndef SKNNR_DEV_ONLY_KS2_M6
    if (ks == 1 && m == 2) return by_waves<1, 2>(waves, extra, L, st, err);
    if (ks == 2 && m == 2) return by_waves<2, 2>(waves, extra, L, st, err);
    if (ks == 1 && m == 6) return by_waves<1, 6>(waves, extra, L, st, err);
    if (ks == 3 && m == 6) return by_waves<3, 6>(waves, extra, L, st, err);
    if (ks == 4 && m == 6) return by_waves<4, 6>(waves, extra, L, st, err);
#endif
    return kNoInstance;
}

int coarse2(int ks, int m_list, int waves, int rank_extra, const Coarse2Launch& L, hipStream_t st, hipError_t* err) {
    const int rc = coarse2_part0(ks, m_list, waves, rank_extra, L, st, err);
    return rc == kNoInstance ? coarse2_part1(ks, m_list, waves, rank_extra, L, st, err) : rc;
}

void coarse2_dev_report() {
#ifdef SKNNR_COARSE_TIMERS
    {
        unsigned long long c[8] = {};
        (void)hipMemcpyFromSymbol(c, HIP_SYMBOL(sknnr::coarse_timers), sizeof c);
        static const char* names[8] = {"sweep", "visit_scan", "flush", "stage_barrier", "seeding", "-", "-", "wave_total"};
        for (int i = 0; i < 8; ++i)
            std::fprintf(stderr, "[coarse-time] %-18s %14llu  %5.1f %%\n", names[i], c[i], 100.0 * (double)c[i] / (double)(c[7] ? c[7] : 1));
        std::memset(c, 0, sizeof c);
        (void)hipMemcpyToSymbol(HIP_SYMBOL(sknnr::coarse_timers), c, sizeof c);
    }
#endif
#ifdef SKNNR_COARSE_COUNTERS
    {
        unsigned long long c[16] = {};
        (void)hipMemcpyFromSymbol(c, HIP_SYMBOL(sknnr::coarse_counters), sizeof c);
        static const char* names[16] = {"tile_qblocks", "visits", "group_hits", "member_hits", "hit_lanes", "overflow_inserts",
                                        "flushes", "flush_iters", "flush_iter_lanes", "flush_insert_iters", "flush_insert_lanes",
                                        "visit_lanes", "visits_with_true_hit", "", "", ""};
        for (int i = 0; i < 13; ++i) std::fprintf(stderr, "[coarse] %-22s %llu\n", names[i], c[i]);
        std::memset(c, 0, sizeof c);
        (void)hipMemcpyToSymbol(HIP_SYMBOL(sknnr::coarse_counters), c, sizeof c);
    }
#endif
}
#else
int coarse2_part1(int ks, int m, int waves, int extra, const Coarse2Launch& L, hipStream_t st, hipError_t* err) {
#ifndef SKNNR_DEV_ONLY_KS2_M6
    if (ks == 1 && m == 8) return by_waves<1, 8>(waves, extra, L, st, err);
    if (ks == 2 && m == 8) return by_waves<2, 8>(waves, extra, L, st, err);
    if (ks == 3 && m == 8) return by_waves<3, 8>(waves, extra, L, st, err);
    if (ks == 4 && m == 8) return by_waves<4, 8>(waves, extra, L, st, err);
    if (ks == 3 && m == 12) return by_waves<3, 12>(waves, extra, L, st, err);
    if (ks == 3 && m == 16) return by_waves<3, 16>(waves, extra, L, st, err);
    if (ks == 4 && m == 12) return by_waves<4, 12>(waves, extra, L, st, err);
    if (ks == 4 && m == 16) return by_waves<4, 16>(waves, extra, L, st, err);
    if (ks == 1 && m == 12) return by_waves<1, 12>(waves, extra, L, st, err);
    if (ks == 2 && m == 12) return by_waves<2, 12>(waves, extra, L, st, err);
    if (ks == 1 && m == 16) return by_waves<1, 16>(waves, extra, L, st, err);
    if (ks == 2 && m == 16) return by_waves<2, 16>(waves, extra, L, st, err);
#endif
    return kNoInstance;
}
#endif

}
}
```

sknnr_amd/csrc/k_exact.hip:

```cpp
#define SKNNR_KERNELS_EXACT 1
#include <cstdint>
#include <cstdlib>

#include "launch.hip.h"

namespace sknnr {
namespace {
__global__ void add_counter_kernel(const int* __restrict__ cnt, long long* __restrict__ total) { *total += *cnt; }

template <int BT>
hipError_t prep_lds_bt(const PrepArgs& a, hipStream_t st) {
    const size_t sh = (size_t)BT * (a.d_in | 1) * 8;
    hipError_t e = hipFuncSetAttribute((const void*)prep_queries_kernel<BT>, hipFuncAttributeMaxDynamicSharedMemorySize, (int)sh);
    if (e != hipSuccess) return e;
    prep_queries_kernel<BT><<<dim3((unsigned)(a.nq_pad / BT)), dim3(BT), sh, st>>>(a);
    return hipGetLastError();
}

template <int FORMULA>
hipError_t exact_scan_f(bool chunked, const ScanArgs& a, long blocks, size_t sh, hipStream_t st) {
    auto kern = chunked ? exact_scan_kernel<FORMULA, true> : exact_scan_kernel<FORMULA, false>;
    hipError_t e = hipFuncSetAttribute((const void*)kern, hipFuncAttributeMaxDynamicSharedMemorySize, (int)sh);
    if (e != hipSuccess) return e;
    kern<<<dim3((unsigned)blocks), dim3(kScanWaves * 64), sh, st>>>(a);
    return hipGetLastError();
}
}

namespace launch {

hipError_t row_norms(const double* x, long n, int d, double* out, hipStream_t st) {
    row_norms_kernel<<<dim3((unsigned)((n + 255) / 256)), dim3(256), 0, st>>>(x, n, d, out);
    return hipGetLastError();
}

template <int KS>
hipError_t prep_direct_ks(PrepArgs a, hipStream_t st) {
    a.lds_wave_bytes = prep_direct_wave_lds(KS, a.xt != nullptr, a.qimg != nullptr);
    const size_t sh = (size_t)4 * a.lds_wave_bytes;
    hipError_t e = hipFuncSetAttribute((const void*)prep_queries_direct_kernel<KS>, hipFuncAttributeMaxDynamicSharedMemorySize, (int)sh);
    if (e != hipSuccess) return e;
    prep_queries_direct_kernel<KS><<<dim3((unsigned)(a.nq_pad / 256)), dim3(256), sh, st>>>(a);
    return hipGetLastError();
}

hipError_t prep_direct(const PrepArgs& a, hipStream_t st) {
    switch (a.ks) {
        case 1: return prep_direct_ks<1>(a, st);
        case 2: return prep_direct_ks<2>(a, st);
        case 3: return prep_direct_ks<3>(a, st);
        case 4: return prep_direct_ks<4>(a, st);
    }
    return hipErrorInvalidValue;
}

hipError_t prep_lds(int rows_per_block, const PrepArgs& a, hipStream_t st) {
    switch (rows_per_block) {
        case 256: return prep_lds_bt<256>(a, st);
        case 128: return prep_lds_bt<128>(a, st);
        case 64: return prep_lds_bt<64>(a, st);
    }
    return hipErrorInvalidValue;
}

hipError_t check_finite(const double* x, long n_el, int* status, hipStream_t st) {
    const long blocks = n_el + 255 < 256L * 256 * 16 ? (n_el + 255) / 256 : 256L * 16;
    check_finite_kernel<<<dim3((unsigned)(blocks < 1 ? 1 : blocks)), dim3(256), 0, st>>>(x, n_el, status);
    return hipGetLastError();
}

hipError_t cell_assign(const CellArgs& a, hipStream_t st) {
    cell_assign_kernel<<<dim3((unsigned)((a.nq + 255) / 256)), dim3(256), 0, st>>>(a);
    return hipGetLastError();
}
hipError_t cell_count(const CellArgs& a, hipStream_t st) {
    cell_count_kernel<<<dim3((unsigned)((a.nq + kBucketBlock * kBucketChunks - 1) / (kBucketBlock * kBucketChunks))), dim3(kBucketBlock), 0, st>>>(a);
    return hipGetLastError();
}
hipError_t cell_scatter(const CellArgs& a, hipStream_t st) {
    cell_scatter_kernel<<<dim3((unsigned)((a.n_pad + kBucketBlock * kBucketChunks - 1) / (kBucketBlock * kBucketChunks))), dim3(kBucketBlock), 0, st>>>(a);
    return hipGetLastError();
}

hipError_t finalize(const FinalizeArgs& f, long n, hipStream_t st) {
    if (f.m_list <= 8) {
        finalize_kernel<8><<<dim3((unsigned)((n * 16 + 255) / 256)), dim3(256), finalize_lds_bytes(8, f.s.d), st>>>(f);
    } else if (f.m_list <= 16) {
        finalize_kernel<16><<<dim3((unsigned)((n * 32 + 255) / 256)), dim3(256), finalize_lds_bytes(16, f.s.d), st>>>(f);
    } else {
        finalize_kernel<32><<<dim3((unsigned)((n * 64 + 255) / 256)), dim3(256), finalize_lds_bytes(32, f.s.d), st>>>(f);
    }
    return hipGetLastError();
}

hipError_t exact_scan(int formula, bool chunked, const ScanArgs& a, long blocks, size_t lds_bytes, hipStream_t st) {
    switch (formula) {
        case 0: return exact_scan_f<0>(chunked, a, blocks, lds_bytes, st);
        case 1: return exact_scan_f<1>(chunked, a, blocks, lds_bytes, st);
        default: return exact_scan_f<2>(chunked, a, blocks, lds_bytes, st);
    }
}

hipError_t scan_merge(int formula, const ScanArgs& a, long blocks, size_t lds_bytes, int grid_wg_of_scan, int forced_slices,
                      hipStream_t st) {
    const dim3 grid((unsigned)blocks), block(256);
    switch (formula) {
        case 0: scan_merge_kernel<0><<<grid, block, lds_bytes, st>>>(a, grid_wg_of_scan, forced_slices); break;
        case 1: scan_merge_kernel<1><<<grid, block, lds_bytes, st>>>(a, grid_wg_of_scan, forced_slices); break;
        default: scan_merge_kernel<2><<<grid, block, lds_bytes, st>>>(a, grid_wg_of_scan, forced_slices); break;
    }
    return hipGetLastError();
}

hipError_t pack_shards(const double* val, const long* idx, long nq, int n_shards, int kk, double* slice_v, int* slice_i,
                       hipStream_t st) {
    const long heaps = nq * n_shards * kk;
    const long blocks = (heaps + 255) / 256 < 256L * 32 ? (heaps + 255) / 256 : 256L * 32;
    pack_shards_kernel<<<dim3((unsigned)(blocks < 1 ? 1 : blocks)), dim3(256), 0, st>>>(val, idx, nq, n_shards, kk, slice_v, slice_i);
    return hipGetLastError();
}

hipError_t predict(const PredictArgs& a, hipStream_t st) {
    const long total = a.nq * a.t;
    if ((a.mode == 0 && a.y32) || (a.mode == 2 && a.w32))
        predict32_kernel<<<dim3((unsigned)((total + 255) / 256)), dim3(256), 0, st>>>(a);
    else if (a.k <= 8)
        predict_kernel<<<dim3((unsigned)((total + 255) / 256)), dim3(256), 0, st>>>(a);
    else
        predict_wide_kernel<<<dim3((unsigned)((total + 255) / 256)), dim3(256), 0, st>>>(a);
    return hipGetLastError();
}

hipError_t crosswalk(const long* table, const long* idx, long n, long* out, hipStream_t st) {
    const long want = (n + 255) / 256;
    const unsigned blocks = (unsigned)(want < 1 ? 1 : (want > 256L * 16 ? 256L * 16 : want));
    crosswalk_kernel<<<dim3(blocks), dim3(256), 0, st>>>(table, idx, n, out);
    return hipGetLastError();
}

hipError_t add_counter(const int* cnt, long long* total, hipStream_t st) {
    add_counter_kernel<<<dim3(1), dim3(1), 0, st>>>(cnt, total);
    return hipGetLastError();
}

}
}
```

sknnr_amd/csrc/launch.hip.h:

```cpp
#pragma once
#include <hip/hip_runtime.h>

#include "bucket.hip.h"
#include "coarse2.hip.h"
#include "exact.hip.h"
#include "forest.hip.h"
#include "hamming.hip.h"

namespace sknnr {
namespace launch {

hipError_t row_norms(const double* x, long n, int d, double* out, hipStream_t st);
hipError_t prep_direct(const PrepArgs& a, hipStream_t st);
hipError_t prep_lds(int rows_per_block, const PrepArgs& a, hipStream_t st);
hipError_t check_finite(const double* x, long n_el, int* status, hipStream_t st);
hipError_t cell_assign(const CellArgs& a, hipStream_t st);
hipError_t cell_count(const CellArgs& a, hipStream_t st);
hipError_t cell_scatter(const CellArgs& a, hipStream_t st);
hipError_t finalize(const FinalizeArgs& f, long n, hipStream_t st);
hipError_t exact_scan(int formula, bool chunked, const ScanArgs& a, long blocks, size_t lds_bytes, hipStream_t st);
hipError_t scan_merge(int formula, const ScanArgs& a, long blocks, size_t lds_bytes, int grid_wg_of_scan, int forced_slices,
                      hipStream_t st);
hipError_t pack_shards(const double* val, const long* idx, long nq, int n_shards, int kk, double* slice_v, int* slice_i,
                       hipStream_t st);
hipError_t predict(const PredictArgs& a, hipStream_t st);
hipError_t crosswalk(const long* table, const long* idx, long n, long* out, hipStream_t st);
hipError_t add_counter(const int* cnt, long long* total, hipStream_t st);

hipError_t hamming_pack(const double* xq, long nq, long nq_pad, int t, int tp, uint32_t* qimg, int* q_bad, hipStream_t st);
hipError_t hamming_rows(const double* x, long n, int t, int tpr, uint32_t* rows, hipStream_t st);
hipError_t hamming_coarse(const HammingArgs& a, hipStream_t st);
hipError_t hamming_rescore(const HammingRescoreArgs& a, hipStream_t st);
hipError_t hamming_distance_rows(const HammingRowsArgs& a, hipStream_t st);

hipError_t forest_apply(const ForestArgs& a, hipStream_t st);

struct Coarse1Launch {
    const char* rimg;
    int n_stages;
    const uint4* qimg;
    const double* qnc;
    float skip_scale;
    int n_sentinel;
    float* cand_val;
    int* cand_idx;
    long nq_pad;
};
struct Coarse2Launch {
    const char* rhi;
    const char* rlo;
    int n_stages;
    const uint4* qimg;
    const double* qnc;
    float skip_scale;
    int n_sentinel;
    float* cand_val;
    int* cand_idx;
    int pos0;
    const int* qperm;
    const unsigned char* qcell;
    const int* cell_stage;
    long rows;
};
constexpr int kNoInstance = -1;
int coarse1(int ks, int m_list, const Coarse1Launch& L, hipStream_t st, hipError_t* err);
int coarse2(int ks, int m_list, int waves, int rank_extra, const Coarse2Launch& L, hipStream_t st, hipError_t* err);
hipError_t coarse_matrix(int ks, const char* rimg, const int* perm, const uint4* qimg, int n_ref, long nq, long n_tiles,
                         long nqb, float* out);
void coarse1_dev_report();
void coarse2_dev_report();

}
}
```

sknnr_amd/csrc/sknnr_hip.hip:

```cpp
#include "../../include/sknnr_hip.h"

#include <hip/hip_runtime.h>
#include <sys/mman.h>

#include <algorithm>
#include <chrono>
#include <cmath>
#include <cstdarg>
#include <cstdio>
#include <cstdlib>
#include <condition_variable>
#include <cstring>
#include <deque>
#include <functional>
#include <future>
#include <limits>
#include <memory>
#include <mutex>
#include <new>
#include <string>
#include <thread>
#include <vector>

#include "launch.hip.h"
// ... 48 lines not shown
    if (rem > halfway || (rem == halfway && (q & 1u))) ++q;
    uint32_t out;
    if (hexp == 0) out = q;
    else out = ((hexp - 1) << 10) + q;
    return (uint16_t)(sign | out);
}

double f16_bits_to_f64(uint16_t h) {
    const int sign = (h >> 15) & 1;
    const int exp = (h >> 10) & 31;
    const int man = h & 1023;
    double v;
    if (exp == 0) v = std::ldexp((double)man, -24);
    else if (exp == 31) v = man ? std::numeric_limits<double>::quiet_NaN() : std::numeric_limits<double>::infinity();
    else v = std::ldexp((double)(man | 1024), exp - 25);
    return sign ? -v : v;
}

template <typename T>
struct DevBuf {
    T* p = nullptr;
    size_t n = 0;
    DevBuf() = default;
    DevBuf(const DevBuf&) = delete;
    DevBuf& operator=(const DevBuf&) = delete;
    ~DevBuf() { release(); }
    hipError_t ensure(size_t count) {
        if (count <= n && p) return hipSuccess;
        if (p) (void)hipFree(p);
        p = nullptr;
        n = 0;
        hipError_t e = hipMalloc((void**)&p, std::max<size_t>(count, 1) * sizeof(T));
        if (e == hipSuccess) n = count;
        return e;
    }
    void release() {
        if (p) (void)hipFree(p);
        p = nullptr;
        n = 0;
    }
};

constexpr int kMaxKs = 8;
constexpr long kChunkRows = 1L << 22;
long chunk_rows(int ks, int m_list) {
    static const long forced = [] {
        const char* e = std::getenv("SKNNR_CHUNK_ROWS");
        const long r = e ? std::atol(e) : 0;
        return r >= kRowQuantum ? std::min<long>(r, 1L << 26) : 0L;
    }();
    if (forced) return forced;
    const long per_row = 64L * std::max(ks, 1) + 8 + 16L * std::max(m_list, 2);
    const long rows = std::min<long>(1L << 24, (4L << 30) / per_row);
    return std::max<long>(kRowQuantum, rows / kRowQuantum * kRowQuantum);
}
constexpr int kScanMaxKK = 192;
constexpr double eps_units(int ks) { return 11.0 + 6.0 * ks; }
constexpr double eps_units2(int ks) { return 12.0 + 2.0 * ks; }

}

constexpr int kHostSlots = 4;

class HostWorker {
public:
    HostWorker() : th_([this] { run(); }) {}
    ~HostWorker() {
        {
            std::lock_guard<std::mutex> l(m_);
            stop_ = true;
        }
        cv_.notify_all();
        th_.join();
    }
    std::future<int> post(std::function<int()> fn) {
        std::packaged_task<int()> task(std::move(fn));
        std::future<int> f = task.get_future();
        {
            std::lock_guard<std::mutex> l(m_);
            q_.emplace_back(std::move(task));
        }
        cv_.notify_one();
        return f;
    }

private:
    void run() {
        for (;;) {
            std::packaged_task<int()> task;
            {
                std::unique_lock<std::mutex> l(m_);
                cv_.wait(l, [this] { return stop_ || !q_.empty(); });
                if (q_.empty()) return;
                task = std::move(q_.front());
                q_.pop_front();
            }
            task();
        }
    }
    std::mutex m_;
    std::condition_variable cv_;
    std::deque<std::packaged_task<int()>> q_;
    bool stop_ = false;
    std::thread th_;
};

struct sknnr_index {
    int device = 0;
    long n_ref = 0;
    int d = 0, t = 0;
    int ks = 0;
    int n_stages = 0;
    double s = 1.0;
    double ymax = 0.0;
    double mu_norm = 0.0;
    std::vector<double> mu;
    std::mutex mtx;

    int d_in = 0;
    bool has_affine = false;
    DevBuf<double> center, scale, proj;
    bool has_center = false, has_scale = false, has_proj = false;

    bool has_forest = false;
    int f_d_in = 0;
    DevBuf<int4> f_nodes;
    DevBuf<long> f_off;
    DevBuf<int> f_depth;
    DevBuf<double> f_ids;

    DevBuf<double> hw;
    double hw_sum = 0.0;
    bool has_hw = false;
    bool h16_ok = false;
    int h_tp = 0, h_ref_pad = 0;
    DevBuf<uint32_t> h_rimg, h_wq, h_qimg, h_rrow;
    DevBuf<int> h_bad, h_cand_cnt, h_cand_id;
    DevBuf<double> ref64, refT, rn64, y64, mu_dev;
    DevBuf<char> rimg;
    DevBuf<char> rhi2, rlo2;
    int n_stages2 = 0;
    DevBuf<int> perm;
    DevBuf<int> perm2;
    int cell_depth = 0;
    DevBuf<float> cell_axes, cell_centre, cell_thr;
    DevBuf<int> cell_stage;
    DevBuf<unsigned char> qcell;
    DevBuf<int> qperm, cell_hist;

    DevBuf<double> xt, qnc, xstage, dist_stage, pred_stage;
    DevBuf<uint4> qimg;
    DevBuf<float> cand_val;
    DevBuf<int> cand_idx, fail_list, fail_count, fail_list2, slice_i;
    DevBuf<double> slice_v;
    DevBuf<int> status;
    DevBuf<long long> fail_total;
    DevBuf<long> idx_stage;

    struct HostSlot {
        double* pin_x = nullptr;  size_t pin_x_n = 0;
        double* pin_d = nullptr;  size_t pin_d_n = 0;
        long* pin_i = nullptr;    size_t pin_i_n = 0;
        double* pin_p = nullptr;  size_t pin_p_n = 0;
        DevBuf<double> dev_x, dev_d, dev_p;
        DevBuf<long> dev_i;
        hipEvent_t ev_h2d = nullptr, ev_done = nullptr, ev_d2h = nullptr;
    } slot[kHostSlots];
    hipStream_t st_h2d = nullptr, st_run = nullptr, st_d2h = nullptr;
    std::unique_ptr<HostWorker> w_in, w_out;

    hipEvent_t ev_ws = nullptr;
    bool ws_busy = false;
    hipStream_t st_side = nullptr;
    hipEvent_t ev_fork = nullptr, ev_join = nullptr;
    long bulk_rows_done = 0;
    hipEvent_t ev_bulk_end = nullptr;
    int64_t last_prefilter[8] = {};
    int64_t last_hamming[8] = {};
    long last_hamming_rows = 0;
    bool stream_open = false;

    struct CallTiming {
        hipEvent_t e0 = nullptr, e1 = nullptr;
        std::vector<std::pair<hipEvent_t, hipEvent_t>> coarse;
        size_t coarse_used = 0;
        long coarse_rows = 0;
        bool pending = false;
    };
    static constexpr int kTimingRing = 64;
    CallTiming timing[kTimingRing];
    int timing_next = 0;
    sknnr_stats stats{};

    ~sknnr_index() {
        w_in.reset();
        w_out.reset();
        (void)hipSetDevice(device);
        for (auto* b : {&center, &scale, &proj, &ref64, &refT, &rn64, &y64, &mu_dev, &xt, &qnc, &xstage,
                        &dist_stage, &pred_stage, &f_ids})
            b->release();
        f_nodes.release(); f_off.release(); f_depth.release();
        rimg.release();
        perm.release();
        perm2.release();
        cell_axes.release(); cell_centre.release(); cell_thr.release(); cell_stage.release();
        qcell.release(); qperm.release(); cell_hist.release();
        h_rimg.release(); h_wq.release(); h_qimg.release(); h_rrow.release(); h_bad.release(); h_cand_cnt.release(); h_cand_id.release();
        qimg.release();
        cand_val.release();
        cand_idx.release();
        fail_list.release();
        fail_count.release();
        fail_total.release();
        status.release();
        idx_stage.release();
        for (auto& sl : slot) {
            for (void* hp : {(void*)sl.pin_x, (void*)sl.pin_d, (void*)sl.pin_i, (void*)sl.pin_p})
                if (hp) (void)hipHostFree(hp);
            sl.dev_x.release(); sl.dev_d.release(); sl.dev_p.release(); sl.dev_i.release();
            for (hipEvent_t e : {sl.ev_h2d, sl.ev_done, sl.ev_d2h})
                if (e) (void)hipEventDestroy(e);
        }
        for (hipStream_t h : {st_h2d, st_run, st_d2h})
            if (h) (void)hipStreamDestroy(h);
        if (ev_ws) (void)hipEventDestroy(ev_ws);
        if (st_side) (void)hipStreamDestroy(st_side);
        for (hipEvent_t e : {ev_fork, ev_join})
            if (e) (void)hipEventDestroy(e);
        for (auto& ct : timing) {
            for (hipEvent_t e : {ct.e0, ct.e1})
                if (e) (void)hipEventDestroy(e);
            for (auto& pr : ct.coarse) {
                (void)hipEventDestroy(pr.first);
                (void)hipEventDestroy(pr.second);
            }
        }
    }
};

extern "C" int32_t sknnr_device_count(void) {
    int n = 0;
    if (hipGetDeviceCount(&n) != hipSuccess) return 0;
    return n;
}

extern "C" int32_t sknnr_abi_version(void) { return SKNNR_ABI_VERSION; }

extern "C" const char* sknnr_last_error(void) { return g_last_error.c_str(); }

extern "C" int sknnr_index_shape(const sknnr_index* ix, int64_t* n_ref, int32_t* d, int32_t* t,
                                 int32_t* d_in, int32_t* device) {
    if (!ix) return fail(SKNNR_ERR_INVALID, "index is NULL");
    if (n_ref) *n_ref = ix->n_ref;
    if (d) *d = ix->d;
    if (t) *t = ix->t;
    if (d_in) *d_in = ix->has_affine ? ix->d_in : (ix->has_forest ? ix->f_d_in : ix->d);
    if (device) *device = ix->device;
    return SKNNR_OK;
}

static bool mahalanobis_norms(const double* ref, int64_t n_ref, int d, const std::vector<double>& mu,
                              std::vector<double>& out) {
    if ((double)n_ref * d * d > 8e9 || n_ref < 2 * (int64_t)d) return false;
    const int64_t n_cov = std::min<int64_t>(n_ref, 65536), stride = n_ref / n_cov;
    std::vector<double> cov((size_t)d * d, 0.0), v((size_t)d);
    for (int64_t i = 0; i < n_cov; ++i) {
        const double* r = ref + i * stride * d;
        for (int a = 0; a < d; ++a) v[(size_t)a] = r[a] - mu[(size_t)a];
        for (int a = 0; a < d; ++a)
            for (int b = 0; b <= a; ++b) cov[(size_t)a * d + b] += v[(size_t)a] * v[(size_t)b];
    }
    double tr = 0.0;
    for (int a = 0; a < d; ++a) {
        for (int b = 0; b <= a; ++b) cov[(size_t)a * d + b] /= (double)n_cov;
        tr += cov[(size_t)a * d + a];
    }
    if (!(tr > 0.0)) return false;
    for (int a = 0; a < d; ++a) cov[(size_t)a * d + a] += 1e-9 * tr / d;
    for (int a = 0; a < d; ++a) {
        for (int b = 0; b <= a; ++b) {
            double sum = cov[(size_t)a * d + b];
            for (int k = 0; k < b; ++k) sum -= cov[(size_t)a * d + k] * cov[(size_t)b * d + k];
            if (a == b) {
                if (!(sum > 0.0)) return false;
                cov[(size_t)a * d + a] = std::sqrt(sum);
            } else {
                cov[(size_t)a * d + b] = sum / cov[(size_t)b * d + b];
            }
        }
    }
    out.resize((size_t)n_ref);
    const unsigned n_thr = std::min<unsigned>(8, std::max(1u, std::thread::hardware_concurrency()));
    std::vector<std::thread> th;
    for (unsigned t = 0; t < n_thr; ++t)
        th.emplace_back([&, t] {
            std::vector<double> z((size_t)d);
            for (int64_t i = t; i < n_ref; i += n_thr) {
                const double* r = ref + i * d;
                double m2 = 0.0;
                for (int a = 0; a < d; ++a) {
                    double sum = r[a] - mu[(size_t)a];
                    for (int k = 0; k < a; ++k) sum -= cov[(size_t)a * d + k] * z[(size_t)k];
                    z[(size_t)a] = sum / cov[(size_t)a * d + a];
                    m2 += z[(size_t)a] * z[(size_t)a];
                }
                out[(size_t)i] = m2;
            }
        });
    for (auto& t : th) t.join();
    return true;
}

struct OrderSim {
    const double* ref;
    int64_t n_ref;
    int d, S, NQ = 64, J = 6;
    int64_t stride;
    std::vector<int> sample;
    std::vector<double> q;
    uint64_t rng = 0x9E3779B97F4A7C15ull;
    OrderSim(const double* ref_, int64_t n_ref_, int d_) : ref(ref_), n_ref(n_ref_), d(d_) {
        S = (int)std::min<int64_t>(n_ref, 8192);
        stride = n_ref / S;
        sample.resize(S);
        for (int i = 0; i < S; ++i) sample[i] = (int)(i * stride);
        q.resize((size_t)NQ * d);
        auto next = [&]() { rng ^= rng << 13; rng ^= rng >> 7; rng ^= rng << 17; return (int64_t)(rng % (uint64_t)n_ref); };
        for (int i = 0; i < NQ; ++i) {
            const int64_t a = next(), b = next(), c = next();
            for (int k = 0; k < d; ++k) q[(size_t)i * d + k] = ref[a * d + k] + 0.35 * (ref[b * d + k] - ref[c * d + k]);
        }
    }
    long visits(const std::vector<int>& order, const std::vector<int>* start = nullptr) const {
        std::vector<double> best((size_t)NQ * J, std::numeric_limits<double>::infinity());
        long n_vis = 0;
        for (int t0 = 0; t0 + 32 <= S; t0 += 32) {
            for (int qb = 0; qb < NQ / 32; ++qb) {
                bool any = false;
                for (int qi = qb * 32; qi < qb * 32 + 32; ++qi) {
                    double* bq = &best[(size_t)qi * J];
                    const double thr = bq[J - 1];
                    const int base = start ? (*start)[(size_t)qi] : 0;
                    for (int r = t0; r < t0 + 32; ++r) {
                        const double* rr = ref + (int64_t)order[(size_t)((base + r) % S)] * d;
                        double d2 = 0.0;
                        for (int k = 0; k < d; ++k) {
                            const double t = q[(size_t)qi * d + k] - rr[k];
                            d2 += t * t;
                        }
                        if (d2 < thr) {
                            any = true;
                            if (d2 < bq[J - 1]) {
                                int p = J - 1;
                                while (p > 0 && bq[p - 1] > d2) { bq[p] = bq[p - 1]; --p; }
                                bq[p] = d2;
                            }
                        }
                    }
                }
                n_vis += any;
            }
        }
        return n_vis;
// ... 586 lines not shown
    for (long c0 = 0; c0 < n; c0 += rows) {
        const long m = std::min<long>(rows, n - c0);
        AT_TRY(hipMemcpy(dx.p, x + c0 * d_in, (size_t)m * d_in * sizeof(double), hipMemcpyHostToDevice));
        PrepArgs a{};
        a.x = dx.p;
        a.nq = m;
        a.nq_pad = (m + 255) / 256 * 256;
        a.d_in = d_in;
        a.d = d;
        a.ks = ks;
        a.center = center ? dc.p : nullptr;
        a.scale = scale ? dsc.p : nullptr;
        a.proj = proj ? dpj.p : nullptr;
        a.xt = dout.p;
        const int ldx = d_in | 1;
        const int bt = (size_t)256 * ldx * 8 <= 150 * 1024 ? 256 : ((size_t)128 * ldx * 8 <= 150 * 1024 ? 128 : 64);
        AT_TRY(launch::prep_lds(bt, a, nullptr));
        AT_TRY(hipMemcpy(out + c0 * d, dout.p, (size_t)m * d * sizeof(double), hipMemcpyDeviceToHost));
    }
#undef AT_TRY
    cleanup();
    return rc;
}

static void resolve_call(sknnr_index* ix, sknnr_index::CallTiming& ct) {
    if (!ct.pending) return;
    ct.pending = false;
    if (hipEventSynchronize(ct.e1) != hipSuccess) return;
    float ms = 0.f;
    if (hipEventElapsedTime(&ms, ct.e0, ct.e1) != hipSuccess) return;
    double cms = 0.0;
    for (size_t i = 0; i < ct.coarse_used; ++i) {
        float m = 0.f;
        if (hipEventElapsedTime(&m, ct.coarse[i].first, ct.coarse[i].second) == hipSuccess) cms += m;
    }
    ix->stats.last_kernel_ms = ms;
    ix->stats.last_coarse_ms = cms;
    ix->stats.total_kernel_ms += ms;
    ix->stats.total_coarse_ms += cms;
    ix->stats.timed_calls += 1;
    ix->stats.coarse_rows_timed += ct.coarse_rows;
}
static void resolve_timing(sknnr_index* ix) {
    for (int i = 0; i < sknnr_index::kTimingRing; ++i)
        resolve_call(ix, ix->timing[(ix->timing_next + i) % sknnr_index::kTimingRing]);
}

extern "C" int sknnr_get_stats(const sknnr_index* cix, sknnr_stats* out) {
    if (!cix || !out) return fail(SKNNR_ERR_INVALID, "NULL argument");
    sknnr_index* ix = const_cast<sknnr_index*>(cix);
    std::lock_guard<std::mutex> lock(ix->mtx);
    (void)hipSetDevice(ix->device);
    resolve_timing(ix);
    long long total = 0;
    if (hipMemcpy(&total, ix->fail_total.p, sizeof total, hipMemcpyDeviceToHost) == hipSuccess)
        ix->stats.exact_fallbacks = total;
    *out = ix->stats;
    launch::coarse1_dev_report();
    launch::coarse2_dev_report();
    return SKNNR_OK;
}

extern "C" int sknnr_reset_stats(sknnr_index* ix) {
    if (!ix) return fail(SKNNR_ERR_INVALID, "index is NULL");
    std::lock_guard<std::mutex> lock(ix->mtx);
    HIP_TRY(hipSetDevice(ix->device));
    HIP_TRY(hipDeviceSynchronize());
    HIP_TRY(hipMemset(ix->fail_total.p, 0, 16));
    for (auto& ct : ix->timing) ct.pending = false;
    ix->stats = sknnr_stats{};
    return SKNNR_OK;
}

static int nonfinite_error(int bits) {
    if (bits & 1) return fail(SKNNR_ERR_NONFINITE, "Input X contains NaN.");
    if (bits & 2) return fail(SKNNR_ERR_NONFINITE, "Input X contains infinity or a value too large for dtype('float64').");
    return fail(SKNNR_ERR_NONFINITE, "Input X contains infinity or a value too large for dtype('float32').");
}

static int poll_status(sknnr_index* ix) {
    int bits = 0;
    HIP_TRY(hipMemcpy(&bits, ix->status.p, sizeof bits, hipMemcpyDeviceToHost));
    if (!bits) return SKNNR_OK;
    HIP_TRY(hipMemset(ix->status.p, 0, 16));
    return nonfinite_error(bits);
}

extern "C" int sknnr_check_finite(sknnr_index* ix, void* stream) {
    if (!ix) return fail(SKNNR_ERR_INVALID, "index is NULL");
    std::lock_guard<std::mutex> lock(ix->mtx);
    HIP_TRY(hipSetDevice(ix->device));
    HIP_TRY(hipStreamSynchronize((hipStream_t)stream));
    return poll_status(ix);
}

namespace {

int launch_prep(sknnr_index* ix, const void* x, long nq, long nq_pad, bool affine, double* xt,
                hipStream_t st, bool check_finite = false, bool cells = false, bool* cells_done = nullptr, int x_dtype = kDtypeF64) {
    PrepArgs a{};
    a.x_dtype = x_dtype;
    if (cells_done) *cells_done = false;
    a.status = check_finite ? ix->status.p : nullptr;
    a.x = x;
    a.nq = nq;
    a.nq_pad = nq_pad;
    a.d_in = affine ? ix->d_in : ix->d;
    a.d = ix->d;
    a.ks = ix->ks;
    a.center = (affine && ix->has_center) ? ix->center.p : nullptr;
    a.scale = (affine && ix->has_scale) ? ix->scale.p : nullptr;
    a.proj = (affine && ix->has_proj) ? ix->proj.p : nullptr;
    a.mu = ix->mu_dev.p;
    a.s = ix->s;
    a.xt = xt;
    a.qimg = ix->qimg.p;
    a.qnc = ix->qnc.p;
    const int ldx = a.d_in | 1;
    const size_t lim = 150 * 1024;
    if (ix->ks <= 4 && !std::getenv("SKNNR_PREP_LDS")) {
        if (cells && ix->cell_depth > 0) {
            a.tree = CellTreeDev{ix->cell_axes.p, ix->cell_centre.p, ix->cell_thr.p, ix->cell_depth};
            a.cell = ix->qcell.p;
            if (cells_done) *cells_done = true;
        }
        HIP_TRY(launch::prep_direct(a, st));
    } else if ((size_t)256 * ldx * 8 <= lim) {
        HIP_TRY(launch::prep_lds(256, a, st));
    } else if ((size_t)128 * ldx * 8 <= lim) {
        HIP_TRY(launch::prep_lds(128, a, st));
    } else if ((size_t)64 * ldx * 8 <= lim) {
        HIP_TRY(launch::prep_lds(64, a, st));
    } else {
        return fail(SKNNR_ERR_UNSUPPORTED, "d_in = %d is too wide for the query preparation kernel (max 299)", a.d_in);
    }
    return SKNNR_OK;
}

int launch_coarse(sknnr_index* ix, long nq_pad, int m_list, int kk, hipStream_t st) {
    launch::Coarse1Launch L{ix->rimg.p, ix->n_stages, ix->qimg.p, ix->qnc.p, (float)(std::ldexp(1.0, -9) * ix->ymax * 1.02),
                            m_list - (kk + 1), ix->cand_val.p, ix->cand_idx.p, nq_pad};
    hipError_t e = hipSuccess;
    if (launch::coarse1(ix->ks, m_list, L, st, &e) == launch::kNoInstance)
        return fail(SKNNR_ERR_UNSUPPORTED, "no coarse kernel for ks = %d, list length %d", ix->ks, m_list);
    HIP_TRY(e);
    int64_t* r = ix->last_prefilter;
    r[0] = 1, r[1] = ix->ks, r[2] = m_list, r[3] = 0, r[4] = coarse_waves(ix->ks, m_list), r[5] = nq_pad;
    return SKNNR_OK;
}

constexpr int kCoarse2TailWaves = 4;
constexpr int kCusPerDevice = 256;

int launch_coarse2_waves(sknnr_index* ix, int m_list, int waves, long row0, long rows, int kk, hipStream_t st) {
    const int extra = coarse2_rank_extra(m_list, kk);
    if (extra != 0 && !((m_list == 16 && kk <= kCoarse2MaxKK16) || (m_list == 12 && kk <= kCoarse2MaxKK12) || (m_list == 8 && kk <= kCoarse2MaxKK8) || (m_list == 6 && kk <= kCoarse2MaxKK6)))
        return fail(SKNNR_ERR_UNSUPPORTED, "lists of %d cannot serve %d neighbours", m_list, kk);
    const bool bucketed = ix->cell_depth > 0;
    launch::Coarse2Launch L{ix->rhi2.p, ix->rlo2.p, ix->n_stages2, ix->qimg.p, ix->qnc.p, (float)(std::ldexp(1.0, -9) * ix->ymax * 1.02),
                            extra != 0 ? 0 : m_list - (kk + 1), ix->cand_val.p, ix->cand_idx.p, (int)row0,
                            bucketed ? ix->qperm.p : nullptr, bucketed ? ix->qcell.p : nullptr,
                            bucketed ? ix->cell_stage.p : nullptr, rows};
    hipError_t e = hipSuccess;
    if (launch::coarse2(ix->ks, m_list, waves, extra, L, st, &e) == launch::kNoInstance)
        return fail(SKNNR_ERR_UNSUPPORTED, "no second-generation coarse kernel for ks = %d, list length %d, %d waves, rank + %d", ix->ks,
                    m_list, waves, extra);
    HIP_TRY(e);
    int64_t* r = ix->last_prefilter;
    r[0] = 2, r[1] = ix->ks, r[2] = m_list, r[3] = extra;
    if (waves == kCoarse2TailWaves) {
        r[6] += rows;
    } else {
        r[4] = waves;
        r[5] += rows;
    }
    return SKNNR_OK;
}

int launch_coarse2(sknnr_index* ix, long rows, int m_list, int kk, hipStream_t st) {
    if (!coarse2_supported(ix->ks, m_list))
        return fail(SKNNR_ERR_UNSUPPORTED, "no second-generation coarse kernel for ks = %d, list length %d", ix->ks, m_list);
    const int BULK_WAVES = coarse2_waves(ix->ks, m_list);
    const long QPB = BULK_WAVES * kCoarse2Nqb * 32;
    const long QPB_TAIL = kCoarse2TailWaves * kCoarse2Nqb * 32;
    static const bool split = [] {
        const char* e = std::getenv("SKNNR_COARSE_TAIL");
        return !(e && std::atoi(e) == 0);
    }();
    const long n_wg = (rows + QPB - 1) / QPB;
    long tail_wg = n_wg % kCusPerDevice;
    if (!split || tail_wg > kCusPerDevice / (BULK_WAVES / kCoarse2TailWaves)) tail_wg = 0;
    const long bulk_rows = (n_wg - tail_wg) * QPB;
    ix->bulk_rows_done = 0;
    if (bulk_rows > 0) {
        int rc = launch_coarse2_waves(ix, m_list, BULK_WAVES, 0, bulk_rows, kk, st);
        if (rc) return rc;
        if (tail_wg > 0 && ix->ev_fork) {
            if (ix->ev_bulk_end) {
                HIP_TRY(hipEventRecord(ix->ev_bulk_end, st));
                ix->ev_bulk_end = nullptr;
            }
            HIP_TRY(hipEventRecord(ix->ev_fork, st));
            ix->bulk_rows_done = bulk_rows;
        }
    }
    if (tail_wg > 0) {
        const long tail_rows = std::min(tail_wg * QPB, (rows - bulk_rows + QPB_TAIL - 1) / QPB_TAIL * QPB_TAIL);
        return launch_coarse2_waves(ix, m_list, kCoarse2TailWaves, bulk_rows, tail_rows, kk, st);
    }
    return SKNNR_OK;
}

bool use_coarse2(const sknnr_index* ix, int m_list) {
    static const bool enabled = [] {
        const char* e = std::getenv("SKNNR_COARSE_V2");
        return !(e && std::atoi(e) == 0);
    }();
    const long tiles2 = (long)ix->n_stages2 * tiles_per_stage2(ix->ks);
    return enabled && tiles2 >= 2 * kSeedTiles && tiles2 * tile2_bytes(ix->ks) < (1L << 32) && tiles2 * 32 < (1L << 26) &&
           coarse2_supported(ix->ks, m_list);
}

constexpr int kCoarseMaxKK = 31;
int coarse_list_len(int kk) { return kk <= 1 ? 2 : (kk <= 5 ? 6 : (kk <= 7 ? 8 : (kk <= 15 ? 16 : 32))); }
int coarse_list_len(const sknnr_index* ix, int kk) {
    static const int enabled = [] {
        const char* e = std::getenv("SKNNR_V2_BIG_K");
        return e ? std::atoi(e) : 4;
    }();
    if (enabled >= 3 && kk > 5 && kk <= kCoarse2MaxKK6 && !use_coarse2(ix, 8) && use_coarse2(ix, 6)) return 6;
    if (enabled >= 2 && kk > 7 && kk <= kCoarse2MaxKK8 && use_coarse2(ix, 8)) return 8;
    if (enabled >= 4 && kk > 15 && kk <= kCoarse2MaxKK12 && use_coarse2(ix, 12)) return 12;
    if (enabled >= 1 && kk > 15 && kk <= kCoarse2MaxKK16 && use_coarse2(ix, 16)) return 16;
    return coarse_list_len(kk);
}
int coarse_rank_extra(int m_list, int kk) { return coarse2_rank_extra(m_list, kk); }

void launch_finalize(const FinalizeArgs& f, long n, hipStream_t st) { (void)launch::finalize(f, n, st); }

constexpr int kScanGridWg = 256 * 4;

int launch_scan_formula(sknnr_index* ix, const ScanArgs& a0, long max_items, bool chunked, size_t sh, hipStream_t st) {
    const SelectArgs& s = a0.s;
    const int nq_pass = scan_nq(s.formula);
    ScanArgs a = a0;
    const bool may_slice = s.kk <= kScanSliceMaxKK && scan_slices(1, nq_pass, s.n_ref, s.kk, kScanGridWg) > 1;
    if (may_slice) {
        const size_t heaps = (size_t)kScanGridWg * nq_pass * s.kk;
        HIP_TRY(ix->slice_v.ensure(heaps));
        HIP_TRY(ix->slice_i.ensure(heaps));
        HIP_TRY(ix->fail_list2.ensure((size_t)kScanGridWg * nq_pass));
        HIP_TRY(hipMemsetAsync(ix->fail_count.p + 2, 0, sizeof(int), st));
        a.slice_v = ix->slice_v.p;
        a.slice_i = ix->slice_i.p;
        a.list2 = ix->fail_list2.p;
        a.count2 = ix->fail_count.p + 2;
    }
    const long passes = (max_items + nq_pass - 1) / nq_pass;
    const long blocks = may_slice ? kScanGridWg : std::max<long>(1, std::min<long>(passes, kScanGridWg));
    HIP_TRY(launch::exact_scan(s.formula, chunked, a, blocks, sh, st));
    if (!may_slice) return SKNNR_OK;
    const long sliced_max = std::min<long>(max_items, (long)kScanGridWg * nq_pass / 2);
    const int kkp = (s.kk + 2) & ~1, stk = (2 * s.kk + 4 + 1) & ~1;
    const size_t msh = 4 * ((size_t)12 * kkp + (size_t)4 * stk);
    HIP_TRY(launch::scan_merge(s.formula, a, (sliced_max + 3) / 4, msh, (int)blocks, 0, st));
    ScanArgs b = a0;
    b.list = ix->fail_list2.p;
    b.count = ix->fail_count.p + 2;
    b.slice_v = nullptr;
    b.slice_i = nullptr;
    const long blocks2 = std::max<long>(1, std::min<long>((sliced_max + nq_pass - 1) / nq_pass, kScanGridWg));
    HIP_TRY(launch::exact_scan(s.formula, chunked, b, blocks2, sh, st));
    return SKNNR_OK;
}

int launch_scan(sknnr_index* ix, const SelectArgs& s, const int* list, const int* count, long max_items,
                hipStream_t st) {
    const size_t sh = scan_block_bytes(s.d, s.kk, s.formula);
    if (sh > 150 * 1024)
        return fail(SKNNR_ERR_UNSUPPORTED, "n_neighbors = %d with d = %d does not fit the exact scan kernel", s.k, s.d);
    ScanArgs a{s, ix->refT.p, list, count, nullptr, nullptr, nullptr, nullptr};
    const bool chunked = s.d > kScanColChunk;
    return launch_scan_formula(ix, a, max_items, chunked, sh, st);
}

bool uses_forest(const sknnr_index* ix, const sknnr_query_opts* o) {
    return o->apply_affine && o->formula == SKNNR_FORMULA_HAMMING && ix->has_forest;
}
int query_cols(const sknnr_index* ix, const sknnr_query_opts* o) {
    if (!o->apply_affine) return ix->d;
    return uses_forest(ix, o) ? ix->f_d_in : ix->d_in;
}

struct CallCtx {
    sknnr_index* ix;
    const sknnr_query_opts* o;
    int kk;
    bool coarse;
};

int validate_call(sknnr_index* ix, const void* q, int64_t nq, const sknnr_query_opts* o, int64_t* out_idx) {
    if (!ix) return fail(SKNNR_ERR_INVALID, "index is NULL");
    if (!o) return fail(SKNNR_ERR_INVALID, "opts is NULL");
    if (o->query_dtype < 0 || o->query_dtype >= kDtypeCount) return fail(SKNNR_ERR_INVALID, "unknown query_dtype %d", o->query_dtype);
    const bool forest_map = uses_forest(ix, o);
    if (o->query_dtype != SKNNR_DTYPE_F64 && q && !forest_map) {
        if (ix->ks == 0) return fail(SKNNR_ERR_UNSUPPORTED, "query_dtype %d needs d <= 128 (d = %d): pass float64 rows", o->query_dtype, ix->d);
        if (o->formula == SKNNR_FORMULA_HAMMING) return fail(SKNNR_ERR_UNSUPPORTED, "node ids are float64: query_dtype must be 0 with formula = HAMMING");
    }
    if (nq < 0) return fail(SKNNR_ERR_INVALID, "nq must be >= 0");
    if (!out_idx && nq > 0) return fail(SKNNR_ERR_INVALID, "out_idx is NULL");
    if (o->n_neighbors <= 0) return fail(SKNNR_ERR_INVALID, "Expected n_neighbors > 0. Got %d", o->n_neighbors);
    if (!q && !o->exclude_self) return fail(SKNNR_ERR_INVALID, "q is NULL but exclude_self is not set");
    const long n_fit = ix->n_ref;
    if (o->exclude_self) {
        if (o->n_neighbors + 1 > n_fit)
            return fail(SKNNR_ERR_K_TOO_LARGE,
                        "Expected n_neighbors < n_samples_fit, but n_neighbors = %d, n_samples_fit = %ld, n_samples = %ld",
                        o->n_neighbors, n_fit, (long)nq);
        if (!q && (o->row_offset < 0 || o->row_offset + nq > n_fit))
            return fail(SKNNR_ERR_INVALID, "self query rows [%ld, %ld) outside the %ld reference rows",
                        (long)o->row_offset, (long)(o->row_offset + nq), n_fit);
    } else if (o->n_neighbors > n_fit) {
        return fail(SKNNR_ERR_K_TOO_LARGE,
                    "Expected n_neighbors <= n_samples_fit, but n_neighbors = %d, n_samples_fit = %ld, n_samples = %ld",
                    o->n_neighbors, n_fit, (long)nq);
    }
    if (o->apply_affine && !ix->has_affine && !forest_map)
        return fail(SKNNR_ERR_INVALID, "apply_affine is set but no affine map was installed");
    if (o->formula != SKNNR_FORMULA_EXPANDED && o->formula != SKNNR_FORMULA_DIRECT && o->formula != SKNNR_FORMULA_HAMMING)
        return fail(SKNNR_ERR_INVALID, "unknown formula %d", o->formula);
    if (o->formula == SKNNR_FORMULA_HAMMING) {
        if (!ix->has_hw) return fail(SKNNR_ERR_INVALID, "formula = HAMMING needs sknnr_index_set_hamming_weights first");
        if (o->apply_affine && !forest_map) return fail(SKNNR_ERR_INVALID, "node ids are not mapped by an affine transform");
    }
    if (o->n_neighbors + (o->exclude_self ? 1 : 0) > kScanMaxKK)
        return fail(SKNNR_ERR_UNSUPPORTED, "n_neighbors = %d exceeds the HIP backend's limit of %d%s", o->n_neighbors,
                    kScanMaxKK - (o->exclude_self ? 1 : 0),
                    o->exclude_self ? " with X=None (the query rows' own rows are searched too)" : "");
    if (std::abs(o->decimals) > 300) return fail(SKNNR_ERR_INVALID, "decimals out of range");
    return SKNNR_OK;
}

int run_forest(sknnr_index* ix, const void* xdev, long nq, const sknnr_query_opts* o, double* d_dist, long* d_idx,
               hipStream_t st);
int run_device(sknnr_index* ix, const void* xdev, long nq, const sknnr_query_opts* o, double* d_dist,
               long* d_idx, hipStream_t st, int raw = 0, long id_offset = 0) {
    std::fill(std::begin(ix->last_prefilter), std::end(ix->last_prefilter), 0);
    std::fill(std::begin(ix->last_hamming), std::end(ix->last_hamming), 0);
    ix->last_hamming_rows = 0;
    if (xdev && uses_forest(ix, o)) return run_forest(ix, xdev, nq, o, d_dist, d_idx, st);
    const int kk = o->n_neighbors + (o->exclude_self ? 1 : 0);
    const bool affine = o->apply_affine != 0 && xdev != nullptr;
    const bool self_rows = xdev == nullptr;
    const int x_dtype = self_rows ? kDtypeF64 : o->query_dtype;
    const bool to_xt = affine || x_dtype != kDtypeF64;
    static const bool scan_everything = std::getenv("SKNNR_EXACT_ONLY") != nullptr;
    const bool coarse = ix->ks > 0 && kk <= kCoarseMaxKK && o->formula != SKNNR_FORMULA_HAMMING && !scan_everything;
    const int d_x = affine ? ix->d_in : ix->d;
    if (nq > 0x7fffffffL) return fail(SKNNR_ERR_UNSUPPORTED, "more than 2^31 - 1 query rows in one call");
    if (affine && ix->ks == 0)
        return fail(SKNNR_ERR_UNSUPPORTED, "d = %d > 128 with an affine map is outside the HIP envelope", ix->d);
    if (ix->ws_busy) HIP_TRY(hipStreamWaitEvent(st, ix->ev_ws, 0));
    const bool check_finite = o->check_finite != 0 && xdev != nullptr;

    const double* xq_call = self_rows ? ix->ref64.p + o->row_offset * ix->d : (const double*)xdev;
    if (to_xt) {
        HIP_TRY(ix->xt.ensure((size_t)nq * ix->d));
        xq_call = ix->xt.p;
    }
    const long chunk = chunk_rows(ix->ks, coarse_list_len(ix, kk));
    const long cap = std::min(chunk, nq);
    const long cap_pad = (cap + kRowQuantum - 1) / kRowQuantum * kRowQuantum;
    if (coarse || to_xt) {
        HIP_TRY(ix->qimg.ensure((size_t)(cap_pad / 32) * 2 * ix->ks * 64));
        HIP_TRY(ix->qnc.ensure(cap_pad));
    }
    if (coarse && ix->cell_depth > 0) {
        HIP_TRY(ix->qcell.ensure((size_t)cap_pad));
        HIP_TRY(ix->qperm.ensure((size_t)cap_pad));
    }
    if (coarse) {
        HIP_TRY(ix->cand_val.ensure((size_t)cap_pad * 2 * coarse_list_len(ix, kk)));
        HIP_TRY(ix->cand_idx.ensure((size_t)cap_pad * 2 * coarse_list_len(ix, kk)));
        HIP_TRY(ix->fail_list.ensure(nq));
        HIP_TRY(hipMemsetAsync(ix->fail_count.p, 0, 16, st));
    }

    SelectArgs call{};
    call.xq = xq_call;
    call.ref = ix->ref64.p;
    call.rn = ix->rn64.p;
    call.nq = nq;
    call.d = ix->d;
    call.n_ref = (int)ix->n_ref;
    call.k = o->n_neighbors;
    call.kk = kk;
    call.exclude_self = o->exclude_self ? 1 : 0;
    call.deterministic = o->deterministic ? 1 : 0;
    call.formula = o->formula;
    call.pow10_is_divisor = o->decimals < 0;
    call.pow10 = std::pow(10.0, std::abs(o->decimals));
    call.row_offset = o->row_offset;
    call.hw = ix->hw.p;
    call.hw_sum = ix->hw_sum;
    call.raw = raw;
    call.id_offset = id_offset;
    if (raw) call.deterministic = 0;
    call.out_dist = d_dist;
    call.out_idx = d_idx;

    sknnr_index::CallTiming& ct = ix->timing[ix->timing_next];
    ix->timing_next = (ix->timing_next + 1) % sknnr_index::kTimingRing;
    resolve_call(ix, ct);
    if (!ct.e0) {
        HIP_TRY(hipEventCreate(&ct.e0));
        HIP_TRY(hipEventCreate(&ct.e1));
    }
    ct.coarse_used = 0;
    ct.coarse_rows = 0;
    HIP_TRY(hipEventRecord(ct.e0, st));
    if (check_finite && !(coarse || to_xt)) {
        const long n_el = nq * (long)d_x;
        HIP_TRY(launch::check_finite((const double*)xdev, n_el, ix->status.p, st));
    }
    for (long c0 = 0; c0 < nq; c0 += chunk) {
        const long n = std::min(chunk, nq - c0);
        const long n_pad = (n + kRowQuantum - 1) / kRowQuantum * kRowQuantum;
        const void* xin = self_rows ? (const void*)(xq_call + c0 * ix->d)
                                    : (const void*)((const char*)xdev + (size_t)c0 * d_x * dtype_bytes(x_dtype));
        const bool bucketed = coarse && ix->cell_depth > 0 && use_coarse2(ix, coarse_list_len(ix, kk));
        bool cells_done = false;
        if (coarse || to_xt) {
            int rc = launch_prep(ix, xin, n, n_pad, affine, to_xt ? ix->xt.p + c0 * ix->d : nullptr, st, check_finite, bucketed, &cells_done,
                                 x_dtype);
            if (rc) return rc;
        }
        if (!coarse) continue;

        if (ct.coarse_used == ct.coarse.size()) {
            hipEvent_t e0, e1;
            HIP_TRY(hipEventCreate(&e0));
            HIP_TRY(hipEventCreate(&e1));
            ct.coarse.emplace_back(e0, e1);
        }
        auto& ev = ct.coarse[ct.coarse_used++];
        const bool v2 = use_coarse2(ix, coarse_list_len(ix, kk));
        if (bucketed) {
            CellArgs ca{};
            ca.xq = xq_call + c0 * ix->d;
            ca.nq = n;
            ca.n_pad = n_pad;
            ca.d = ix->d;
            ca.depth = ix->cell_depth;
            ca.axes = ix->cell_axes.p;
            ca.centre = ix->cell_centre.p;
            ca.thr = ix->cell_thr.p;
            ca.cell = ix->qcell.p;
            ca.hist = ix->cell_hist.p;
            ca.perm = ix->qperm.p;
            HIP_TRY(hipMemsetAsync(ix->cell_hist.p, 0, 2 * kCellMax * sizeof(int), st));
            if (!cells_done) HIP_TRY(launch::cell_assign(ca, st));
            HIP_TRY(launch::cell_count(ca, st));
            HIP_TRY(launch::cell_scatter(ca, st));
        }
        HIP_TRY(hipEventRecord(ev.first, st));
        if (v2 && !ix->st_side && !std::getenv("SKNNR_NO_SIDE_STREAM")) {
            HIP_TRY(hipStreamCreateWithFlags(&ix->st_side, hipStreamNonBlocking));
            HIP_TRY(hipEventCreateWithFlags(&ix->ev_fork, hipEventDisableTiming));
            HIP_TRY(hipEventCreateWithFlags(&ix->ev_join, hipEventDisableTiming));
        }
        ix->bulk_rows_done = 0;
        ix->ev_bulk_end = ev.second;
        std::fill(std::begin(ix->last_prefilter), std::end(ix->last_prefilter), 0);
        ix->last_prefilter[7] = bucketed ? ix->cell_depth : 0;
        {
            const long tiles = v2 ? (long)ix->n_stages2 * tiles_per_stage2(ix->ks) +
                                        seed_tiles_for((long)ix->n_stages2 * tiles_per_stage2(ix->ks), tiles_per_stage2(ix->ks))
                                  : (long)ix->n_stages * tiles_per_stage(ix->ks);
            ix->stats.mfma_executed_ratio = (double)tiles * 32.0 * (16.0 * ix->ks) / ((double)ix->n_ref * ix->d);
        }
        int rc = v2 ? launch_coarse2(ix, n, coarse_list_len(ix, kk), kk, st)
                    : launch_coarse(ix, n_pad, coarse_list_len(ix, kk), kk, st);
        if (rc) return rc;
        if (ix->ev_bulk_end) HIP_TRY(hipEventRecord(ev.second, st));
        ix->ev_bulk_end = nullptr;
        ct.coarse_rows += ix->bulk_rows_done > 0 ? std::min<long>(ix->bulk_rows_done, n) : n;

        FinalizeArgs f{};
        f.s = call;
        f.s.xq = xq_call + c0 * ix->d;
        f.s.nq = n;
        f.s.row_offset = o->row_offset + c0;
        f.s.out_dist = d_dist ? d_dist + c0 * o->n_neighbors : nullptr;
        f.s.out_idx = d_idx + c0 * o->n_neighbors;
        f.cand_val = ix->cand_val.p;
        f.cand_idx = ix->cand_idx.p;
        f.perm = v2 ? ix->perm2.p : ix->perm.p;
        f.qnc = ix->qnc.p;
        f.qperm = bucketed ? ix->qperm.p : nullptr;
        f.m_list = coarse_list_len(ix, kk);
        f.rank_extra = coarse_rank_extra(f.m_list, kk);
        f.inv_s2 = 1.0 / (ix->s * ix->s);
        f.s2 = ix->s * ix->s;
        f.inv_s = 1.0 / ix->s;
        f.eps_c = (v2 ? eps_units2(ix->ks) : eps_units(ix->ks)) * std::ldexp(1.0, -24);
        f.ymax = ix->ymax;
        f.noise_a = (ix->d + 4) * std::ldexp(1.0, -53);
        f.mu2 = o->formula == SKNNR_FORMULA_EXPANDED ? 2.0 * ix->mu_norm : 0.0;
        f.fail_list = ix->fail_list.p;
        f.fail_count = ix->fail_count.p;
        f.fail_base = (int)c0;
        auto finalize_rows = [&](long r0, long rows, hipStream_t s_) {
            FinalizeArgs g = f;
            if (bucketed) {
                g.pos0 = r0;
                g.s.nq = rows;
                launch_finalize(g, rows, s_);
                return;
            }
            g.s.xq = f.s.xq + r0 * ix->d;
            g.s.nq = rows;
            g.s.row_offset = f.s.row_offset + r0;
            g.s.out_dist = f.s.out_dist ? f.s.out_dist + r0 * o->n_neighbors : nullptr;
            g.s.out_idx = f.s.out_idx + r0 * o->n_neighbors;
            g.cand_val = f.cand_val + (size_t)r0 * 2 * f.m_list;
            g.cand_idx = f.cand_idx + (size_t)r0 * 2 * f.m_list;
            g.qnc = f.qnc + r0;
            g.fail_base = f.fail_base + (int)r0;
            launch_finalize(g, rows, s_);
        };
        const long done = v2 ? std::min<long>(ix->bulk_rows_done, n) : 0;
        if (done > 0) {
            HIP_TRY(hipStreamWaitEvent(ix->st_side, ix->ev_fork, 0));
            finalize_rows(0, done, ix->st_side);
            HIP_TRY(hipGetLastError());
            HIP_TRY(hipEventRecord(ix->ev_join, ix->st_side));
            if (n > done) finalize_rows(done, n - done, st);
            HIP_TRY(hipGetLastError());
            HIP_TRY(hipStreamWaitEvent(st, ix->ev_join, 0));
        } else {
            finalize_rows(0, n, st);
            HIP_TRY(hipGetLastError());
        }
    }
    const bool ham_int = !coarse && o->formula == SKNNR_FORMULA_HAMMING && ix->h16_ok && kk <= kHamMaxKK;
    if (ham_int) {
        const long chunk_q = 1L << 18;
        const long cap_q = std::min(chunk_q, nq);
        const long cap_pad = (cap_q + 255) / 256 * 256;
        HIP_TRY(ix->h_qimg.ensure((size_t)ix->h_tp * cap_pad));
        HIP_TRY(ix->h_bad.ensure((size_t)cap_pad));
        HIP_TRY(ix->h_cand_cnt.ensure((size_t)cap_q));
        HIP_TRY(ix->h_cand_id.ensure((size_t)cap_q * kHamCand));
        HIP_TRY(ix->fail_list.ensure(nq));
        HIP_TRY(hipMemsetAsync(ix->fail_count.p, 0, 16, st));
        const int64_t rec[7] = {1, kk, ham_compacts(kk) ? 1 : 0, ham_seed_rows((int)ix->n_ref, kk), (int64_t)ix->d + 2,
                                ix->h_tp, (nq + chunk_q - 1) / chunk_q};
        std::copy(std::begin(rec), std::end(rec), ix->last_hamming);
        for (long c0 = 0; c0 < nq; c0 += chunk_q) {
            const long n = std::min(chunk_q, nq - c0);
            ix->last_hamming_rows = n;
            const long n_pad = (n + 255) / 256 * 256;
            HIP_TRY(launch::hamming_pack(xq_call + c0 * ix->d, n, n_pad, ix->d, ix->h_tp, ix->h_qimg.p, ix->h_bad.p, st));
            HammingArgs ha{};
            ha.rimg = ix->h_rimg.p;
            ha.wq = ix->h_wq.p;
            ha.qimg = ix->h_qimg.p;
            ha.q_bad = ix->h_bad.p;
            ha.n_ref = (int)ix->n_ref;
            ha.n_ref_pad = ix->h_ref_pad;
            ha.tp = ix->h_tp;
            ha.nq = n;
            ha.nq_pad = n_pad;
            ha.kk = kk;
            ha.band = (unsigned)ix->d + 2u;
            ha.cand_cnt = ix->h_cand_cnt.p;
            ha.cand_id = ix->h_cand_id.p;
            HIP_TRY(launch::hamming_coarse(ha, st));
            HammingRescoreArgs hr{};
            hr.s = call;
            hr.s.xq = xq_call + c0 * ix->d;
            hr.s.nq = n;
            hr.s.row_offset = o->row_offset + c0;
            hr.s.out_dist = d_dist ? d_dist + c0 * o->n_neighbors : nullptr;
            hr.s.out_idx = d_idx + c0 * o->n_neighbors;
            hr.cand_cnt = ix->h_cand_cnt.p;
            hr.cand_id = ix->h_cand_id.p;
            hr.fail_list = ix->fail_list.p;
            hr.fail_count = ix->fail_count.p;
            hr.fail_base = (int)c0;
            hr.rrow = ix->h_rrow.p;
            hr.tpr = ham_row_dwords(ix->d);
            HIP_TRY(launch::hamming_rescore(hr, st));
        }
    }
    int rc = (coarse || ham_int) ? launch_scan(ix, call, ix->fail_list.p, ix->fail_count.p, nq, st)
                                 : launch_scan(ix, call, nullptr, nullptr, nq, st);
    if (rc) return rc;
    if (coarse) {
        HIP_TRY(launch::add_counter(ix->fail_count.p, ix->fail_total.p, st));
        ix->stats.coarse_queries += nq;
    } else {
        if (ham_int) HIP_TRY(launch::add_counter(ix->fail_count.p, ix->fail_total.p, st));
        ix->stats.exact_only_queries += nq;
    }
    HIP_TRY(hipEventRecord(ct.e1, st));
    ct.pending = true;
    HIP_TRY(hipEventRecord(ix->ev_ws, st));
    ix->ws_busy = true;
    ix->stats.queries += nq;
    return SKNNR_OK;
}

long forest_chunk_rows(int n_trees) {
    const long by_bytes = (4L << 30) / (8L * std::max(n_trees, 1));
    return std::max<long>(kFtRows, std::min<long>(1L << 18, by_bytes) / kFtRows * kFtRows);
}

ForestArgs forest_args(const sknnr_index* ix, const void* x, long n, int x_dtype, double* out, int* status) {
    ForestArgs a{};
    a.x = x;
    a.x_dtype = x_dtype;
    a.nq = n;
    a.d_in = ix->f_d_in;
    a.nodes = ix->f_nodes.p;
    a.tree_off = ix->f_off.p;
    a.tree_depth = ix->f_depth.p;
    a.n_trees = ix->d;
    a.out = out;
    a.status = status;
    return a;
}

int run_forest(sknnr_index* ix, const void* xdev, long nq, const sknnr_query_opts* o, double* d_dist, long* d_idx,
               hipStream_t st) {
    if (ix->ws_busy) HIP_TRY(hipStreamWaitEvent(st, ix->ev_ws, 0));
    const long chunk = forest_chunk_rows(ix->d);
    HIP_TRY(ix->f_ids.ensure((size_t)std::min(chunk, nq) * ix->d));
    const size_t row_bytes = (size_t)ix->f_d_in * dtype_bytes(o->query_dtype);
    const int k = o->n_neighbors;
    for (long c0 = 0; c0 < nq; c0 += chunk) {
        const long n = std::min(chunk, nq - c0);
        const ForestArgs fa = forest_args(ix, (const char*)xdev + (size_t)c0 * row_bytes, n, o->query_dtype, ix->f_ids.p,
                                          o->check_finite ? ix->status.p : nullptr);
        HIP_TRY(launch::forest_apply(fa, st));
        sknnr_query_opts oc = *o;
        oc.apply_affine = 0;
        oc.query_dtype = SKNNR_DTYPE_F64;
        oc.check_finite = 0;
        oc.row_offset = o->row_offset + c0;
        int rc = run_device(ix, ix->f_ids.p, n, &oc, d_dist ? d_dist + c0 * k : nullptr, d_idx + c0 * k, st);
        if (rc) return rc;
    }
    return SKNNR_OK;
}

}

static int launch_predict(sknnr_index* ix, const double* dist, const long* idx, const double* w, long nq, int k,
                          int mode, double* out, hipStream_t st);

namespace {

constexpr long kHostChunkRows = 1L << 20;

long host_chunk_rows() {
    static const long v = [] {
        const char* e = std::getenv("SKNNR_HOST_CHUNK_ROWS");
        const long r = e ? std::atol(e) : 0;
        return r >= 1024 ? r : kHostChunkRows;
    }();
    return v;
}

void parallel_copy(void* dst, const void* src, size_t bytes) {
    const size_t kMin = 8u << 20;
    unsigned n = std::min<unsigned>(8, std::max(1u, std::thread::hardware_concurrency()));
    if (bytes < 2 * kMin) n = 1;
    if (n == 1) {
        std::memcpy(dst, src, bytes);
        return;
    }
    std::vector<std::thread> th;
// ... 706 lines not shown
            if (ix->ws_busy) HIP_TRY(hipStreamWaitEvent(st, ix->ev_ws, 0));
        }
        if (!dd) {
            HIP_TRY(ix->dist_stage.ensure((size_t)nq * k));
            dd = ix->dist_stage.p;
        }
        if (!di) {
            HIP_TRY(ix->idx_stage.ensure((size_t)nq * k));
            di = ix->idx_stage.p;
        }
        rc = run_device(ix, q, nq, o, dd, di, st);
        if (rc) return rc;
        return launch_predict(ix, dd, di, nullptr, nq, k, o->weight_mode, out_pred, st);
    }
    if (q) return run_host_pipeline(ix, q, nq, o, out_dist, (long*)out_idx, out_pred);
    return run_self_rows(ix, nq, o, out_dist, (long*)out_idx, out_pred);
}

struct sknnr_stream {
    HostPipe pipe;
    int64_t rows_pushed = 0;
};

extern "C" int sknnr_stream_begin(sknnr_index* ix, const sknnr_query_opts* o, int32_t want_dist, int32_t want_pred,
                                  sknnr_stream** out) {
    if (!out) return fail(SKNNR_ERR_INVALID, "out is NULL");
    *out = nullptr;
    static int64_t dummy_idx;
    static const double dummy_q = 0.0;
    int rc = validate_call(ix, &dummy_q, 0, o, &dummy_idx);
    if (rc) return rc;
    if (o->exclude_self) return fail(SKNNR_ERR_INVALID, "a stream answers pushed rows: exclude_self is not available");
    if (want_pred) {
        if (ix->t < 1) return fail(SKNNR_ERR_NO_TARGETS, "the index was created without targets");
        if (!weight_mode_ok(o->weight_mode, false))
            return fail(SKNNR_ERR_INVALID, "a stream predicts with uniform or distance weights only");
    }
    std::lock_guard<std::mutex> lock(ix->mtx);
    if (ix->stream_open) return fail(SKNNR_ERR_INVALID, "a query stream is already open on this handle");
    HIP_TRY(hipSetDevice(ix->device));
    sknnr_stream* s = new (std::nothrow) sknnr_stream();
    if (!s) return fail(SKNNR_ERR_INVALID, "out of host memory");
    rc = pipe_open(s->pipe, ix, o, want_dist != 0, true, want_pred != 0);
    if (rc) {
        delete s;
        return rc;
    }
    ix->stream_open = true;
    *out = s;
    return SKNNR_OK;
}

extern "C" int sknnr_stream_push(sknnr_stream* s, const void* q, int64_t nq, double* out_dist, int64_t* out_idx,
                                 double* out_pred) {
    if (!s) return fail(SKNNR_ERR_INVALID, "stream is NULL");
    if (nq < 0) return fail(SKNNR_ERR_INVALID, "nq must be >= 0");
    if (nq == 0) return SKNNR_OK;
    if (!q) return fail(SKNNR_ERR_INVALID, "q is NULL");
    HostPipe& p = s->pipe;
    if (!out_idx && !out_pred) return fail(SKNNR_ERR_INVALID, "a push needs out_idx or out_pred");
    if (out_dist && !p.want_dist) return fail(SKNNR_ERR_INVALID, "the stream was opened without distances");
    if (out_pred && !p.want_pred) return fail(SKNNR_ERR_INVALID, "the stream was opened without predictions");
    std::lock_guard<std::mutex> lock(p.ix->mtx);
    HIP_TRY(hipSetDevice(p.ix->device));
    int rc = pipe_submit_rows(p, q, nq, out_dist, (long*)out_idx, out_pred);
    if (rc) {
        const std::string msg = g_last_error;
        pipe_abort(p);
        (void)hipDeviceSynchronize();
        g_last_error = msg;
        return rc;
    }
    s->rows_pushed += nq;
    return SKNNR_OK;
}

extern "C" int sknnr_stream_flush(sknnr_stream* s) {
    if (!s) return fail(SKNNR_ERR_INVALID, "stream is NULL");
    std::lock_guard<std::mutex> lock(s->pipe.ix->mtx);
    HIP_TRY(hipSetDevice(s->pipe.ix->device));
    return pipe_flush(s->pipe);
}

extern "C" int sknnr_stream_end(sknnr_stream* s, int64_t* rows_pushed) {
    if (!s) return SKNNR_OK;
    int rc;
    {
        std::lock_guard<std::mutex> lock(s->pipe.ix->mtx);
        rc = hipSetDevice(s->pipe.ix->device) == hipSuccess ? pipe_flush(s->pipe) : fail(SKNNR_ERR_HIP, "hipSetDevice failed");
        s->pipe.ix->stream_open = false;
    }
    if (rows_pushed) *rows_pushed = s->rows_pushed;
    delete s;
    return rc;
}

extern "C" int sknnr_crosswalk(const int64_t* table, int64_t n_table, const int64_t* idx, int64_t n, int64_t* out,
                               int32_t device, int32_t mem, void* stream) {
    if (!table || !idx || !out || n < 0 || n_table < 1) return fail(SKNNR_ERR_INVALID, "bad argument");
    if (mem != SKNNR_MEM_DEVICE && mem != SKNNR_MEM_HOST) return fail(SKNNR_ERR_INVALID, "unknown memspace %d", mem);
    if (n == 0) return SKNNR_OK;
    HIP_TRY(hipSetDevice(device));
    if (mem == SKNNR_MEM_DEVICE) {
        HIP_TRY(launch::crosswalk((const long*)table, (const long*)idx, n, (long*)out, (hipStream_t)stream));
        return SKNNR_OK;
    }
    DevBuf<long> dt, di, dout;
    HIP_TRY(dt.ensure(n_table));
    HIP_TRY(di.ensure(n));
    HIP_TRY(dout.ensure(n));
    HIP_TRY(hipMemcpy(dt.p, table, n_table * sizeof(long), hipMemcpyHostToDevice));
    HIP_TRY(hipMemcpy(di.p, idx, n * sizeof(long), hipMemcpyHostToDevice));
    HIP_TRY(launch::crosswalk(dt.p, di.p, n, dout.p, nullptr));
    HIP_TRY(hipMemcpy(out, dout.p, n * sizeof(long), hipMemcpyDeviceToHost));
    return SKNNR_OK;
}

extern "C" int sknnr_debug_coarse_matrix(sknnr_index* ix, const double* q, int64_t nq, float* out, double* out_qnorm,
                                         double* out_scale, double* out_eps) {
    if (!ix || !q || !out || nq < 1) return fail(SKNNR_ERR_INVALID, "bad argument");
    if (ix->ks == 0) return fail(SKNNR_ERR_UNSUPPORTED, "no coarse image (d > 128)");
    if ((double)nq * (double)ix->n_ref > 16777216.0) return fail(SKNNR_ERR_INVALID, "nq * n_ref must be <= 2^24");
    std::lock_guard<std::mutex> lock(ix->mtx);
    HIP_TRY(hipSetDevice(ix->device));
    HIP_TRY(hipDeviceSynchronize());
    const long n_pad = (nq + kRowQuantum - 1) / kRowQuantum * kRowQuantum;
    HIP_TRY(ix->xstage.ensure((size_t)nq * ix->d));
    HIP_TRY(hipMemcpy(ix->xstage.p, q, (size_t)nq * ix->d * sizeof(double), hipMemcpyHostToDevice));
    HIP_TRY(ix->qimg.ensure((size_t)(n_pad / 32) * 2 * ix->ks * 64));
    HIP_TRY(ix->qnc.ensure(n_pad));
    int rc = launch_prep(ix, ix->xstage.p, nq, n_pad, false, nullptr, nullptr);
    if (rc) return rc;
    DevBuf<float> dout;
    HIP_TRY(dout.ensure((size_t)nq * ix->n_ref));
    const long n_tiles = (ix->n_ref + 31) / 32, nqb = (nq + 31) / 32;
    hipError_t e = launch::coarse_matrix(ix->ks, ix->rimg.p, ix->perm.p, ix->qimg.p, (int)ix->n_ref, nq, n_tiles, nqb, dout.p);
    if (e == hipSuccess) e = hipMemcpy(out, dout.p, (size_t)nq * ix->n_ref * sizeof(float), hipMemcpyDeviceToHost);
    if (e == hipSuccess && out_qnorm) e = hipMemcpy(out_qnorm, ix->qnc.p, nq * sizeof(double), hipMemcpyDeviceToHost);
    dout.release();
    if (e != hipSuccess) return fail(SKNNR_ERR_HIP, "debug matrix failed: %s", hipGetErrorString(e));
    if (out_scale) *out_scale = ix->s;
    if (out_eps) *out_eps = eps_units(ix->ks) * std::ldexp(1.0, -24);
    return SKNNR_OK;
}

extern "C" int sknnr_debug_last_prefilter(const sknnr_index* cix, int64_t out[8]) {
    if (!cix || !out) return fail(SKNNR_ERR_INVALID, "NULL argument");
    sknnr_index* ix = const_cast<sknnr_index*>(cix);
    std::lock_guard<std::mutex> lock(ix->mtx);
    std::copy(std::begin(ix->last_prefilter), std::end(ix->last_prefilter), out);
    return SKNNR_OK;
}

extern "C" int sknnr_debug_last_hamming(const sknnr_index* cix, int64_t out[8]) {
    if (!cix || !out) return fail(SKNNR_ERR_INVALID, "NULL argument");
    sknnr_index* ix = const_cast<sknnr_index*>(cix);
    std::lock_guard<std::mutex> lock(ix->mtx);
    std::copy(std::begin(ix->last_hamming), std::end(ix->last_hamming), out);
    out[7] = 0;
    if (ix->last_hamming[0]) {
        int n_fail = 0;
        HIP_TRY(hipSetDevice(ix->device));
        HIP_TRY(hipDeviceSynchronize());
        HIP_TRY(hipMemcpy(&n_fail, ix->fail_count.p, sizeof n_fail, hipMemcpyDeviceToHost));
        out[7] = n_fail;
    }
    return SKNNR_OK;
}

extern "C" int sknnr_debug_hamming_candidates(const sknnr_index* cix, int32_t* cnt, int32_t* ids, int64_t n) {
    if (!cix || !cnt || !ids) return fail(SKNNR_ERR_INVALID, "NULL argument");
    sknnr_index* ix = const_cast<sknnr_index*>(cix);
    std::lock_guard<std::mutex> lock(ix->mtx);
    if (!ix->last_hamming[0]) return fail(SKNNR_ERR_INVALID, "the last call did not run the integer Hamming pre-filter");
    if (n < 0 || n > ix->last_hamming_rows)
        return fail(SKNNR_ERR_INVALID, "n = %ld rows, the last device chunk has %ld", (long)n, ix->last_hamming_rows);
    HIP_TRY(hipSetDevice(ix->device));
    HIP_TRY(hipDeviceSynchronize());
    HIP_TRY(hipMemcpy(cnt, ix->h_cand_cnt.p, (size_t)n * sizeof(int32_t), hipMemcpyDeviceToHost));
    HIP_TRY(hipMemcpy(ids, ix->h_cand_id.p, (size_t)n * kHamCand * sizeof(int32_t), hipMemcpyDeviceToHost));
    return SKNNR_OK;
}
```

Before: 222.5.

## Emit compact sorted candidate record from coarse kernel for 8-lane finalize

When list length is at most 6 and ks is at most 2, the coarse MFMA kernel now merges both half-lists in registers and writes a rank-ordered 8-entry (value,row) record per query, plus a precomputed pair bound. It no longer writes the full per-half candidate arrays. A new finalize_record_kernel reads this record with 8 lanes per query, using DPP peers and per-position query norms gathered during bucketing. This cuts the candidate traffic between stages and the finalize lane count. Queries whose needed candidates may spill past the 8-entry record are marked truncated and sent to the exact fallback, which adds fallback risk; an env var can disable the path.

```diff
diff --git a/include/sknnr_hip.h b/include/sknnr_hip.h
--- a/include/sknnr_hip.h
+++ b/include/sknnr_hip.h
@@ -156,6 +156,8 @@
 
 int sknnr_debug_last_prefilter(const sknnr_index* index, int64_t out[8]);
 
+int sknnr_debug_last_finalize(const sknnr_index* index, int64_t out[4]);
+
 int sknnr_debug_last_hamming(const sknnr_index* index, int64_t out[8]);
 
 int sknnr_debug_hamming_candidates(const sknnr_index* index, int32_t* cnt, int32_t* ids, int64_t n);
diff --git a/sknnr_amd/_native.py b/sknnr_amd/_native.py
--- a/sknnr_amd/_native.py
+++ b/sknnr_amd/_native.py
@@ -72,6 +72,7 @@
     "sknnr_crosswalk",
     "sknnr_debug_coarse_matrix",
     "sknnr_debug_last_prefilter",
+    "sknnr_debug_last_finalize",
     "sknnr_debug_last_hamming",
     "sknnr_debug_hamming_candidates",
 )
@@ -179,6 +180,8 @@
     lib.sknnr_debug_coarse_matrix.argtypes = [vp, vp, c_int64, vp, vp, POINTER(c_double),
                                               POINTER(c_double)]
     lib.sknnr_debug_last_prefilter.argtypes = [vp, POINTER(c_int64)]
+    if hasattr(lib, "sknnr_debug_last_finalize"):
+        lib.sknnr_debug_last_finalize.argtypes = [vp, POINTER(c_int64)]
     lib.sknnr_debug_last_hamming.argtypes = [vp, POINTER(c_int64)]
     lib.sknnr_debug_hamming_candidates.argtypes = [vp, vp, vp, c_int64]
     _lib = lib
@@ -416,6 +419,13 @@
         check(load().sknnr_debug_last_prefilter(self.handle, out))
         return dict(zip(self.PREFILTER_FIELDS, (int(v) for v in out)))
 
+    FINALIZE_FIELDS = ("lanes_per_query", "record", "truncated_rows", "reserved")
+
+    def debug_last_finalize(self) -> dict:
+        out = (c_int64 * 4)()
+        check(load().sknnr_debug_last_finalize(self.handle, out))
+        return dict(zip(self.FINALIZE_FIELDS, (int(v) for v in out)))
+
     HAMMING_FIELDS = ("ran", "kk", "compacts", "seed_rows", "band", "tree_pairs", "chunks", "handed_to_scan")
 
     def debug_last_hamming(self) -> dict:
diff --git a/sknnr_amd/csrc/bucket.hip.h b/sknnr_amd/csrc/bucket.hip.h
--- a/sknnr_amd/csrc/bucket.hip.h
+++ b/sknnr_amd/csrc/bucket.hip.h
@@ -39,6 +39,8 @@
     unsigned char* cell;
     int* hist;
     int* perm;
+    const double* qnc;
+    double* qnc_pos;
 };
 
 #ifdef SKNNR_KERNELS_EXACT
@@ -111,6 +113,7 @@
             ticket[r] = atomicAdd(&cnt[c[r]], 1);
         } else if (q < a.n_pad) {
             a.perm[q] = (int)q;
+            if (a.qnc_pos) a.qnc_pos[q] = a.qnc[q];
             a.cell[q] = (unsigned char)(n_cells - 1);
         }
     }
@@ -120,7 +123,11 @@
 #pragma unroll
     for (int r = 0; r < kBucketChunks; ++r) {
         const long q = ((long)blockIdx.x * kBucketChunks + r) * kBucketBlock + threadIdx.x;
-        if (q < a.nq) a.perm[first[c[r]] + base[c[r]] + ticket[r]] = (int)q;
+        if (q < a.nq) {
+            const int p = first[c[r]] + base[c[r]] + ticket[r];
+            a.perm[p] = (int)q;
+            if (a.qnc_pos) a.qnc_pos[p] = a.qnc[q];
+        }
     }
 }
 #endif
diff --git a/sknnr_amd/csrc/coarse.hip.h b/sknnr_amd/csrc/coarse.hip.h
--- a/sknnr_amd/csrc/coarse.hip.h
+++ b/sknnr_amd/csrc/coarse.hip.h
@@ -208,6 +208,8 @@
         }
     }
 }
+
+constexpr int kRecordLen = 8;
 
 template <int M>
 __device__ __forceinline__ float pair_union_rank_m(const float (&vals)[M]) {
diff --git a/sknnr_amd/csrc/coarse2.hip.h b/sknnr_amd/csrc/coarse2.hip.h
--- a/sknnr_amd/csrc/coarse2.hip.h
+++ b/sknnr_amd/csrc/coarse2.hip.h
@@ -143,6 +143,17 @@
         asm volatile("v_mfma_f32_32x32x16_f16 %[c], %[h], %[q], %[c]\n\t" : [c] "+v"(c) : [h] "v"(ah[s]), [q] "v"(q[s]));
 }
 
+struct Coarse2Record {
+    unsigned long long* entry;
+    float* bound;
+    const int* perm;
+    int n_ref;
+};
+constexpr int kRecordMaxList = 6;
+__host__ __device__ constexpr bool coarse2_record_supported(int ks, int m, int rank_extra) {
+    return ks <= 2 && m <= kRecordMaxList && rank_extra == 0;
+}
+
 template <int KS, int M, int WAVES = kCoarse2Waves, int E = 0>
 __global__ void __launch_bounds__(WAVES * 64, WAVES == 12 ? 3 : (WAVES == 8 || M > 8 ? 2 : 4))
 coarse2_kernel(const char* __restrict__ rhi,
@@ -155,7 +166,8 @@
                float* __restrict__ cand_val,
                int* __restrict__ cand_idx,
                int pos0, const int* __restrict__ qperm, const unsigned char* __restrict__ qcell,
-               const int* __restrict__ cell_stage) {
+               const int* __restrict__ cell_stage,
+               Coarse2Record rec) {
     constexpr int TPS = tiles_per_stage2(KS);
     constexpr int TB = tile2_bytes(KS);
     constexpr int STAGE = TPS * TB;
@@ -454,8 +466,60 @@
         for (int i = 0; i < 16; ++i) atomicAdd(&coarse_counters[i], (unsigned long long)ctr[i]);
 #endif
     TSTAMP(0);
-#pragma unroll
-    for (int qb = 0; qb < NQB; ++qb) {
+    bool filed = false;
+    if constexpr (coarse2_record_supported(KS, M, E)) {
+        if (rec.entry) {
+            filed = true;
+            static_assert(kQueueCap * 512 >= 32 * kRecordLen * 8, "the record image fits the queue region");
+#pragma unroll
+            for (int qb = 0; qb < NQB; ++qb) flush_wave(qb);
+            int slot_of[NQB][M], row_of[NQB][M];
+#pragma unroll
+            for (int qb = 0; qb < NQB; ++qb) {
+                bool ok[M];
+                float pv[M];
+#pragma unroll
+                for (int i = 0; i < M; ++i) {
+                    ok[i] = idxs[qb][i] >= 0 && idxs[qb][i] < rec.n_ref;
+                    pv[i] = __shfl_xor(ok[i] ? vals[qb][i] : __builtin_nanf(""), 32, 64);
+                }
+                int ahead = 0;
+#pragma unroll
+                for (int i = 0; i < M; ++i) {
+                    const float v = vals[qb][i];
+                    int r = ahead;
+#pragma unroll
+                    for (int j = 0; j < M; ++j) r += (half == 0 ? pv[j] < v : pv[j] <= v) ? 1 : 0;
+                    const bool file = ok[i] && r < kRecordLen;
+                    slot_of[qb][i] = file ? r : kRecordLen;
+                    row_of[qb][i] = file ? rec.perm[idxs[qb][i]] : -1;
+                    ahead += ok[i] ? 1 : 0;
+                }
+            }
+#pragma unroll
+            for (int qb = 0; qb < NQB; ++qb) {
+                const unsigned rimg = qwave + (unsigned)qb * (kQueueCap * 512u);
+                const unsigned rcol = rimg - (unsigned)lane * 8u + (unsigned)(lane & 31) * (kRecordLen * 8u);
+                const unsigned long long none = 0xffffffff7f800000ull;
+#pragma unroll
+                for (int j = 0; j < kRecordLen / 2; ++j)
+                    asm volatile("ds_write_b64 %0, %1" ::"v"(rcol + (unsigned)(half * (kRecordLen / 2) + j) * 8u), "v"(none) : "memory");
+#pragma unroll
+                for (int i = 0; i < M; ++i)
+                    if (slot_of[qb][i] < kRecordLen) queue_store(rcol + (unsigned)slot_of[qb][i] * 8u, vals[qb][i], row_of[qb][i]);
+                const size_t q0 = (size_t)(pos0 + (qb0 + qb) * 32);
+                unsigned long long* out = rec.entry + q0 * kRecordLen + lane;
+#pragma unroll
+                for (int t = 0; t < 32 * kRecordLen / 64; ++t) out[t * 64] = queue_load(rimg + (unsigned)t * 512u);
+                const float u = pair_union_rank<M, E>(vals[qb]);
+                const int mine = loose[qb] != loose[qb] ? 1 : 0;
+                const bool bad = (mine | __shfl_xor(mine, 32, 64)) != 0;
+                if (half == 0) rec.bound[q0 + lane] = bad ? __builtin_nanf("") : u;
+            }
+        }
+    }
+#pragma unroll
+    for (int qb = 0; qb < NQB && !filed; ++qb) {
         flush_wave(qb);
         const size_t q = (size_t)(pos0 + (qb0 + qb) * 32 + (lane & 31));
         const size_t base = (q * 2 + half) * M;
diff --git a/sknnr_amd/csrc/exact.hip.h b/sknnr_amd/csrc/exact.hip.h
--- a/sknnr_amd/csrc/exact.hip.h
+++ b/sknnr_amd/csrc/exact.hip.h
@@ -390,10 +390,29 @@
     int* fail_count;
     const int* qperm;
     long pos0;
+    const unsigned long long* rec;
+    const float* rec_bound;
+    const double* qnc_pos;
+    int* trunc_count;
 };
 
+constexpr int kDppQuadXor[4] = {0xE4, 0xB1, 0x4E, 0x1B};
+constexpr int kDppRowHalfMirror = 0x141;
+__device__ __forceinline__ int half_mirror8(int v) { return __builtin_amdgcn_update_dpp(0, v, kDppRowHalfMirror, 0xf, 0xf, false); }
+template <int N>
+__device__ __forceinline__ int peer8_i(int v, int mirror) {
+    static_assert(N >= 1 && N < 8, "a peer of an 8-lane group");
+    if constexpr (N < 4) {
+        return __builtin_amdgcn_update_dpp(0, v, kDppQuadXor[N], 0xf, 0xf, false);
+    } else if constexpr (N < 7) {
+        return __builtin_amdgcn_update_dpp(0, mirror, kDppQuadXor[7 - N], 0xf, 0xf, false);
+    } else {
+        return mirror;
+    }
+}
 template <int LPQ, int N>
 __device__ __forceinline__ int peer_i(int v, int c) {
+    if constexpr (LPQ == 8) return peer8_i<N>(v, half_mirror8(v));
     constexpr int B = N / 16, R = N % 16;
     const int vb = B ? __shfl_xor(v, 16 * B, LPQ) : v;
     if constexpr (R != 0) {
@@ -418,14 +437,16 @@
 }
 template <int LPQ>
 struct PeersI {
-    int blk[LPQ / 16];
+    int blk[LPQ == 8 ? 2 : LPQ / 16];
     __device__ __forceinline__ explicit PeersI(int v) {
         blk[0] = v;
+        if constexpr (LPQ == 8) blk[1] = half_mirror8(v);
 #pragma unroll
         for (int b = 1; b < LPQ / 16; ++b) blk[b] = __shfl_xor(v, 16 * b, LPQ);
     }
     template <int N>
     __device__ __forceinline__ int get() const {
+        if constexpr (LPQ == 8) return peer8_i<N>(blk[0], blk[1]);
         constexpr int B = N / 16, R = N % 16;
         if constexpr (R != 0) {
             return __builtin_amdgcn_update_dpp(0, blk[B], 0x120 + R, 0xf, 0xf, false);
@@ -517,6 +538,10 @@
 __host__ __device__ constexpr size_t finalize_row_bytes(int d) { return (size_t)d * 8 + 16; }
 __host__ __device__ constexpr size_t finalize_lds_bytes(int m_tmpl, int d) { return (size_t)(256 / (2 * m_tmpl)) * finalize_row_bytes(d); }
 
+template <int LPQ, bool RECORD>
+__device__ __forceinline__ void finalize_core(const FinalizeArgs& a, long q, int c, bool live, const double* xrow, int id, bool valid,
+                                              float cv, double qn, double tau_c, double t_min);
+
 template <int M>
 __global__ void __launch_bounds__(256) finalize_kernel(FinalizeArgs a) {
     constexpr int LPQ = 2 * M;
@@ -545,13 +570,28 @@
     const int id = valid ? a.perm[pos_img] : -1;
 
     const double qn = a.qnc[q];
-    const double nrm = sqrt(qn) + a.ymax;
-    const double eps = a.eps_c * nrm * nrm;
     const float cve = valid ? cv : INFINITY;
     int n_le = 1;
     const PeersF<LPQ> cve_of(cve);
     for_each_peer<LPQ>([&](auto n) { n_le += cve_of.template get<n.value>() <= cve; });
     const double tau_c = group_min<LPQ>(n_le >= s.kk ? (double)cve : INFINITY, c);
+    const int ex = a.rank_extra;
+    const float cv_raw = has_slot ? cv : INFINITY;
+    const bool paired = has_slot && slot >= ex;
+    const int partner = M + (paired ? a.m_list + ex - 1 - slot : 0);
+    const float cv_partner = __shfl(cv_raw, partner, LPQ);
+    double t_pair = (list == 0 && paired) ? (double)fminf(cv_raw, cv_partner) : -INFINITY;
+    if (ex > 0 && has_slot && slot == ex - 1) t_pair = (double)cv_raw;
+    const double t_min = group_max<LPQ>(t_pair, c);
+    finalize_core<LPQ, false>(a, q, c, live, xrow, id, valid, cv, qn, tau_c, t_min);
+}
+
+template <int LPQ, bool RECORD>
+__device__ __forceinline__ void finalize_core(const FinalizeArgs& a, long q, int c, bool live, const double* xrow, int id, bool valid,
+                                              float cv, double qn, double tau_c, double t_min) {
+    const SelectArgs& s = a.s;
+    const double nrm = sqrt(qn) + a.ymax;
+    const double eps = a.eps_c * nrm * nrm;
     const double nr = nrm * a.inv_s + a.mu2;
     const double noise = a.noise_a * nr * nr;
     const bool need = valid && ((double)cv <= tau_c + 2.0 * eps + 2.0 * noise * a.s2);
@@ -573,16 +613,13 @@
     const int n_usable = group_count<LPQ>(usable, (int)(threadIdx.x & 63) & ~(LPQ - 1));
 
     const double tau = group_min<LPQ>(rank >= s.kk - 1 ? d2 : INFINITY, c);
-    const int ex = a.rank_extra;
-    const float cv_raw = has_slot ? cv : INFINITY;
-    const bool paired = has_slot && slot >= ex;
-    const int partner = M + (paired ? a.m_list + ex - 1 - slot : 0);
-    const float cv_partner = __shfl(cv_raw, partner, LPQ);
-    double t_pair = (list == 0 && paired) ? (double)fminf(cv_raw, cv_partner) : -INFINITY;
-    if (ex > 0 && has_slot && slot == ex - 1) t_pair = (double)cv_raw;
-    const double t_min = group_max<LPQ>(t_pair, c);
     const double bound = (qn + t_min - eps) * a.inv_s2 - noise;
     bool certified = (n_usable >= s.kk) && (tau < INFINITY) && (bound > tau);
+    bool truncated = false;
+    if constexpr (RECORD) {
+        truncated = group_any<LPQ>(c == LPQ - 1 && need, (int)(threadIdx.x & 63) & ~(LPQ - 1));
+        if (truncated) certified = false;
+    }
     {
         const int gbase = (int)(threadIdx.x & 63) & ~(LPQ - 1);
         const double by_rank = scatter_d<LPQ>(d2, gbase + rank);
@@ -638,8 +675,39 @@
     if (live && c == 0 && !certified) {
         const int slot = atomicAdd(a.fail_count, 1);
         a.fail_list[slot] = a.fail_base + (int)q;
-    }
-}
+        if (RECORD && truncated) atomicAdd(a.trunc_count, 1);
+    }
+}
+
+#ifdef SKNNR_KERNELS_EXACT
+__global__ void __launch_bounds__(256) finalize_record_kernel(FinalizeArgs a) {
+    constexpr int LPQ = kRecordLen;
+    const SelectArgs& s = a.s;
+    const long gt = (long)blockIdx.x * 256 + threadIdx.x;
+    long q = gt / LPQ;
+    const int c = (int)(gt % LPQ);
+    const bool live = q < s.nq;
+    if (!live) q = s.nq - 1;
+    const long q_list = a.qperm ? a.pos0 + q : q;
+    const unsigned long long e = a.rec[q_list * LPQ + c];
+    const float t_min = a.rec_bound[q_list];
+    const double qn = a.qnc_pos[q_list];
+    if (a.qperm) q = a.qperm[q_list];
+
+    extern __shared__ __attribute__((aligned(16))) char fin_lds[];
+    double* xrow = (double*)(fin_lds + (size_t)(threadIdx.x / LPQ) * finalize_row_bytes(s.d));
+    for (int i = c; i < s.d; i += LPQ) xrow[i] = s.xq[q * s.d + i];
+    __builtin_amdgcn_fence(__ATOMIC_RELEASE, "wavefront");
+    __builtin_amdgcn_wave_barrier();
+    __builtin_amdgcn_fence(__ATOMIC_ACQUIRE, "wavefront");
+
+    const int id = (int)(unsigned)(e >> 32);
+    const float cv = __uint_as_float((unsigned)e);
+    const bool valid = id >= 0 && id < s.n_ref;
+    const double tau_c = (double)__shfl(valid ? cv : INFINITY, s.kk - 1, LPQ);
+    finalize_core<LPQ, true>(a, q, c, live, xrow, id, valid, cv, qn, tau_c, (double)t_min);
+}
+#endif
 
 struct ScanArgs {
     SelectArgs s;
diff --git a/sknnr_amd/csrc/k_coarse2.hip b/sknnr_amd/csrc/k_coarse2.hip
--- a/sknnr_amd/csrc/k_coarse2.hip
+++ b/sknnr_amd/csrc/k_coarse2.hip
@@ -18,11 +18,12 @@
     constexpr size_t sh = 2 * (size_t)tiles_per_stage2(KS) * tile2_bytes(KS) + (size_t)WAVES * queue2_bytes_per_wave();
     static_assert(kRowQuantum % QPB == 0, "query rows are padded to multiples of kRowQuantum");
     static_assert(sh <= 160 * 1024, "LDS budget");
+    if (L.rec.entry && !coarse2_record_supported(KS, M, E)) return hipErrorInvalidValue;
     auto kern = coarse2_kernel<KS, M, WAVES, E>;
     hipError_t e = hipFuncSetAttribute((const void*)kern, hipFuncAttributeMaxDynamicSharedMemorySize, (int)sh);
     if (e != hipSuccess) return e;
     kern<<<dim3((unsigned)(L.rows / QPB)), dim3(WAVES * 64), sh, st>>>(L.rhi, L.rlo, L.n_stages, L.qimg, L.qnc, L.skip_scale, L.n_sentinel,
-                                                                   L.cand_val, L.cand_idx, L.pos0, L.qperm, L.qcell, L.cell_stage);
+                                                                   L.cand_val, L.cand_idx, L.pos0, L.qperm, L.qcell, L.cell_stage, L.rec);
     return hipGetLastError();
 }
 
diff --git a/sknnr_amd/csrc/k_exact.hip b/sknnr_amd/csrc/k_exact.hip
--- a/sknnr_amd/csrc/k_exact.hip
+++ b/sknnr_amd/csrc/k_exact.hip
@@ -82,8 +82,12 @@
     return hipGetLastError();
 }
 
+int finalize_lanes(const FinalizeArgs& f) { return f.rec ? kRecordLen : (f.m_list <= 8 ? 16 : (f.m_list <= 16 ? 32 : 64)); }
+
 hipError_t finalize(const FinalizeArgs& f, long n, hipStream_t st) {
-    if (f.m_list <= 8) {
+    if (f.rec) {
+        finalize_record_kernel<<<dim3((unsigned)((n * kRecordLen + 255) / 256)), dim3(256), finalize_lds_bytes(kRecordLen / 2, f.s.d), st>>>(f);
+    } else if (f.m_list <= 8) {
         finalize_kernel<8><<<dim3((unsigned)((n * 16 + 255) / 256)), dim3(256), finalize_lds_bytes(8, f.s.d), st>>>(f);
     } else if (f.m_list <= 16) {
         finalize_kernel<16><<<dim3((unsigned)((n * 32 + 255) / 256)), dim3(256), finalize_lds_bytes(16, f.s.d), st>>>(f);
diff --git a/sknnr_amd/csrc/launch.hip.h b/sknnr_amd/csrc/launch.hip.h
--- a/sknnr_amd/csrc/launch.hip.h
+++ b/sknnr_amd/csrc/launch.hip.h
@@ -18,6 +18,7 @@
 hipError_t cell_count(const CellArgs& a, hipStream_t st);
 hipError_t cell_scatter(const CellArgs& a, hipStream_t st);
 hipError_t finalize(const FinalizeArgs& f, long n, hipStream_t st);
+int finalize_lanes(const FinalizeArgs& f);
 hipError_t exact_scan(int formula, bool chunked, const ScanArgs& a, long blocks, size_t lds_bytes, hipStream_t st);
 hipError_t scan_merge(int formula, const ScanArgs& a, long blocks, size_t lds_bytes, int grid_wg_of_scan, int forced_slices,
                       hipStream_t st);
@@ -61,6 +62,7 @@
     const unsigned char* qcell;
     const int* cell_stage;
     long rows;
+    Coarse2Record rec;
 };
 constexpr int kNoInstance = -1;
 int coarse1(int ks, int m_list, const Coarse1Launch& L, hipStream_t st, hipError_t* err);
diff --git a/sknnr_amd/csrc/sknnr_hip.hip b/sknnr_amd/csrc/sknnr_hip.hip
--- a/sknnr_amd/csrc/sknnr_hip.hip
+++ b/sknnr_amd/csrc/sknnr_hip.hip
@@ -224,6 +224,9 @@
     DevBuf<uint4> qimg;
     DevBuf<float> cand_val;
     DevBuf<int> cand_idx, fail_list, fail_count, fail_list2, slice_i;
+    DevBuf<unsigned long long> rec;
+    DevBuf<float> rec_bound;
+    DevBuf<double> qnc_pos;
     DevBuf<double> slice_v;
     DevBuf<int> status;
     DevBuf<long long> fail_total;
@@ -248,6 +251,7 @@
     long bulk_rows_done = 0;
     hipEvent_t ev_bulk_end = nullptr;
     int64_t last_prefilter[8] = {};
+    int64_t last_finalize[2] = {};
     int64_t last_hamming[8] = {};
     long last_hamming_rows = 0;
     bool stream_open = false;
@@ -281,6 +285,7 @@
         qimg.release();
         cand_val.release();
         cand_idx.release();
+        rec.release(); rec_bound.release(); qnc_pos.release();
         fail_list.release();
         fail_count.release();
         fail_total.release();
@@ -1173,7 +1178,15 @@
 constexpr int kCoarse2TailWaves = 4;
 constexpr int kCusPerDevice = 256;
 
-int launch_coarse2_waves(sknnr_index* ix, int m_list, int waves, long row0, long rows, int kk, hipStream_t st) {
+bool use_record(int ks, int m_list, int kk, bool v2, int raw) {
+    static const bool enabled = [] {
+        const char* e = std::getenv("SKNNR_FINALIZE_RECORD");
+        return !(e && std::atoi(e) == 0);
+    }();
+    return enabled && v2 && !raw && coarse2_record_supported(ks, m_list, coarse2_rank_extra(m_list, kk));
+}
+
+int launch_coarse2_waves(sknnr_index* ix, int m_list, int waves, long row0, long rows, int kk, bool record, hipStream_t st) {
     const int extra = coarse2_rank_extra(m_list, kk);
     if (extra != 0 && !((m_list == 16 && kk <= kCoarse2MaxKK16) || (m_list == 12 && kk <= kCoarse2MaxKK12) || (m_list == 8 && kk <= kCoarse2MaxKK8) || (m_list == 6 && kk <= kCoarse2MaxKK6)))
         return fail(SKNNR_ERR_UNSUPPORTED, "lists of %d cannot serve %d neighbours", m_list, kk);
@@ -1181,7 +1194,8 @@
     launch::Coarse2Launch L{ix->rhi2.p, ix->rlo2.p, ix->n_stages2, ix->qimg.p, ix->qnc.p, (float)(std::ldexp(1.0, -9) * ix->ymax * 1.02),
                             extra != 0 ? 0 : m_list - (kk + 1), ix->cand_val.p, ix->cand_idx.p, (int)row0,
                             bucketed ? ix->qperm.p : nullptr, bucketed ? ix->qcell.p : nullptr,
-                            bucketed ? ix->cell_stage.p : nullptr, rows};
+                            bucketed ? ix->cell_stage.p : nullptr, rows,
+                            Coarse2Record{record ? ix->rec.p : nullptr, ix->rec_bound.p, ix->perm2.p, (int)ix->n_ref}};
     hipError_t e = hipSuccess;
     if (launch::coarse2(ix->ks, m_list, waves, extra, L, st, &e) == launch::kNoInstance)
         return fail(SKNNR_ERR_UNSUPPORTED, "no second-generation coarse kernel for ks = %d, list length %d, %d waves, rank + %d", ix->ks,
@@ -1198,7 +1212,7 @@
     return SKNNR_OK;
 }
 
-int launch_coarse2(sknnr_index* ix, long rows, int m_list, int kk, hipStream_t st) {
+int launch_coarse2(sknnr_index* ix, long rows, int m_list, int kk, bool record, hipStream_t st) {
     if (!coarse2_supported(ix->ks, m_list))
         return fail(SKNNR_ERR_UNSUPPORTED, "no second-generation coarse kernel for ks = %d, list length %d", ix->ks, m_list);
     const int BULK_WAVES = coarse2_waves(ix->ks, m_list);
@@ -1214,7 +1228,7 @@
     const long bulk_rows = (n_wg - tail_wg) * QPB;
     ix->bulk_rows_done = 0;
     if (bulk_rows > 0) {
-        int rc = launch_coarse2_waves(ix, m_list, BULK_WAVES, 0, bulk_rows, kk, st);
+        int rc = launch_coarse2_waves(ix, m_list, BULK_WAVES, 0, bulk_rows, kk, record, st);
         if (rc) return rc;
         if (tail_wg > 0 && ix->ev_fork) {
             if (ix->ev_bulk_end) {
@@ -1227,7 +1241,7 @@
     }
     if (tail_wg > 0) {
         const long tail_rows = std::min(tail_wg * QPB, (rows - bulk_rows + QPB_TAIL - 1) / QPB_TAIL * QPB_TAIL);
-        return launch_coarse2_waves(ix, m_list, kCoarse2TailWaves, bulk_rows, tail_rows, kk, st);
+        return launch_coarse2_waves(ix, m_list, kCoarse2TailWaves, bulk_rows, tail_rows, kk, record, st);
     }
     return SKNNR_OK;
 }
@@ -1369,6 +1383,7 @@
                long* d_idx, hipStream_t st, int raw = 0, long id_offset = 0) {
     std::fill(std::begin(ix->last_prefilter), std::end(ix->last_prefilter), 0);
     std::fill(std::begin(ix->last_hamming), std::end(ix->last_hamming), 0);
+    std::fill(std::begin(ix->last_finalize), std::end(ix->last_finalize), 0);
     ix->last_hamming_rows = 0;
     if (xdev && uses_forest(ix, o)) return run_forest(ix, xdev, nq, o, d_dist, d_idx, st);
     const int kk = o->n_neighbors + (o->exclude_self ? 1 : 0);
@@ -1401,9 +1416,16 @@
         HIP_TRY(ix->qcell.ensure((size_t)cap_pad));
         HIP_TRY(ix->qperm.ensure((size_t)cap_pad));
     }
-    if (coarse) {
+    const bool record = coarse && use_record(ix->ks, coarse_list_len(ix, kk), kk, use_coarse2(ix, coarse_list_len(ix, kk)), raw);
+    if (record) {
+        HIP_TRY(ix->rec.ensure((size_t)cap_pad * kRecordLen));
+        HIP_TRY(ix->rec_bound.ensure((size_t)cap_pad));
+        if (ix->cell_depth > 0) HIP_TRY(ix->qnc_pos.ensure((size_t)cap_pad));
+    } else if (coarse) {
         HIP_TRY(ix->cand_val.ensure((size_t)cap_pad * 2 * coarse_list_len(ix, kk)));
         HIP_TRY(ix->cand_idx.ensure((size_t)cap_pad * 2 * coarse_list_len(ix, kk)));
+    }
+    if (coarse) {
         HIP_TRY(ix->fail_list.ensure(nq));
         HIP_TRY(hipMemsetAsync(ix->fail_count.p, 0, 16, st));
     }
@@ -1480,6 +1502,8 @@
             ca.cell = ix->qcell.p;
             ca.hist = ix->cell_hist.p;
             ca.perm = ix->qperm.p;
+            ca.qnc = ix->qnc.p;
+            ca.qnc_pos = record ? ix->qnc_pos.p : nullptr;
             HIP_TRY(hipMemsetAsync(ix->cell_hist.p, 0, 2 * kCellMax * sizeof(int), st));
             if (!cells_done) HIP_TRY(launch::cell_assign(ca, st));
             HIP_TRY(launch::cell_count(ca, st));
@@ -1501,7 +1525,7 @@
                                   : (long)ix->n_stages * tiles_per_stage(ix->ks);
             ix->stats.mfma_executed_ratio = (double)tiles * 32.0 * (16.0 * ix->ks) / ((double)ix->n_ref * ix->d);
         }
-        int rc = v2 ? launch_coarse2(ix, n, coarse_list_len(ix, kk), kk, st)
+        int rc = v2 ? launch_coarse2(ix, n, coarse_list_len(ix, kk), kk, record, st)
                     : launch_coarse(ix, n_pad, coarse_list_len(ix, kk), kk, st);
         if (rc) return rc;
         if (ix->ev_bulk_end) HIP_TRY(hipEventRecord(ev.second, st));
@@ -1520,6 +1544,12 @@
         f.perm = v2 ? ix->perm2.p : ix->perm.p;
         f.qnc = ix->qnc.p;
         f.qperm = bucketed ? ix->qperm.p : nullptr;
+        if (record) {
+            f.rec = ix->rec.p;
+            f.rec_bound = ix->rec_bound.p;
+            f.qnc_pos = bucketed ? ix->qnc_pos.p : ix->qnc.p;
+            f.trunc_count = ix->fail_count.p + 3;
+        }
         f.m_list = coarse_list_len(ix, kk);
         f.rank_extra = coarse_rank_extra(f.m_list, kk);
         f.inv_s2 = 1.0 / (ix->s * ix->s);
@@ -1545,12 +1575,20 @@
             g.s.row_offset = f.s.row_offset + r0;
             g.s.out_dist = f.s.out_dist ? f.s.out_dist + r0 * o->n_neighbors : nullptr;
             g.s.out_idx = f.s.out_idx + r0 * o->n_neighbors;
-            g.cand_val = f.cand_val + (size_t)r0 * 2 * f.m_list;
-            g.cand_idx = f.cand_idx + (size_t)r0 * 2 * f.m_list;
+            if (record) {
+                g.rec = f.rec + (size_t)r0 * kRecordLen;
+                g.rec_bound = f.rec_bound + r0;
+                g.qnc_pos = f.qnc_pos + r0;
+            } else {
+                g.cand_val = f.cand_val + (size_t)r0 * 2 * f.m_list;
+                g.cand_idx = f.cand_idx + (size_t)r0 * 2 * f.m_list;
+            }
             g.qnc = f.qnc + r0;
             g.fail_base = f.fail_base + (int)r0;
             launch_finalize(g, rows, s_);
         };
+        ix->last_finalize[0] = launch::finalize_lanes(f);
+        ix->last_finalize[1] = record ? 1 : 0;
         const long done = v2 ? std::min<long>(ix->bulk_rows_done, n) : 0;
         if (done > 0) {
             HIP_TRY(hipStreamWaitEvent(ix->st_side, ix->ev_fork, 0));
@@ -2563,6 +2601,23 @@
     return SKNNR_OK;
 }
 
+extern "C" int sknnr_debug_last_finalize(const sknnr_index* cix, int64_t out[4]) {
+    if (!cix || !out) return fail(SKNNR_ERR_INVALID, "NULL argument");
+    sknnr_index* ix = const_cast<sknnr_index*>(cix);
+    std::lock_guard<std::mutex> lock(ix->mtx);
+    out[0] = ix->last_finalize[0];
+    out[1] = ix->last_finalize[1];
+    out[2] = out[3] = 0;
+    if (ix->last_finalize[1]) {
+        int n_trunc = 0;
+        HIP_TRY(hipSetDevice(ix->device));
+        HIP_TRY(hipDeviceSynchronize());
+        HIP_TRY(hipMemcpy(&n_trunc, ix->fail_count.p + 3, sizeof n_trunc, hipMemcpyDeviceToHost));
+        out[2] = n_trunc;
+    }
+    return SKNNR_OK;
+}
+
 extern "C" int sknnr_debug_last_hamming(const sknnr_index* cix, int64_t out[8]) {
     if (!cix || !out) return fail(SKNNR_ERR_INVALID, "NULL argument");
     sknnr_index* ix = const_cast<sknnr_index*>(cix);
```

Measured after the change: 225.0 (median of 6 runs). +1.1%, better.
